# Krual-T/OutfitX

Hardware: AMD Instinct MI355X
Metric: outfits/sec CP forward (8-item sets, 224^2, bf16) (higher is better)
Workload: dtype f16

## Files before the change

include/ofx.h:

```cpp
#ifndef OFX_H
#define OFX_H
#include <stddef.h>
#include <stdint.h>

#ifdef __cplusplus
extern "C" {
#endif

#define OFX_ABI_VERSION 6

enum { OFX_OK = 0, OFX_EINVAL = -1, OFX_ESHAPE = -2, OFX_EHIP = -3, OFX_EWORKSPACE = -4, OFX_ESTATE = -5 };
enum ofx_dtype { OFX_F32 = 0, OFX_BF16 = 1, OFX_F16 = 2 };
enum ofx_act { OFX_ACT_NONE = 0, OFX_ACT_QUICK_GELU = 1, OFX_ACT_GELU = 2, OFX_ACT_MISH = 3, OFX_ACT_MISH_GRAD = 4 };
enum ofx_precision { OFX_PREC_BF16 = 0, OFX_PREC_F16 = 1, OFX_PREC_BF16X3 = 2, OFX_PREC_F16W2 = 3 };
enum ofx_out_kind { OFX_OUT_F32 = 0, OFX_OUT_OP = 1, OFX_OUT_SPLIT3 = 2 };

typedef struct ofx_handle ofx_handle;
typedef void* ofx_stream;

const char* ofx_last_error(void);
int ofx_abi_version(void);

typedef struct ofx_model_desc {
    int d_model, n_head, d_ffn, n_layers, max_items;
    int outfit_act;
    int outfit_precision;
    int vit_width, vit_layers, vit_heads, vit_mlp, vit_patch, vit_image, vit_act;
    int txt_width, txt_layers, txt_heads, txt_mlp, txt_vocab, txt_max_pos, txt_act, txt_eos_id;
    int proj_dim;
    int tower_precision;
    float ln_eps;
    int vit_w2_mask, txt_x3, proj_x3, vit_x3;
    int txt_w2_mask, vit_w2_qkv_layers, vit_w2_fc1_layers, vit_w2_out_layers, vit_w2_fc2_layers;
} ofx_model_desc;
enum { OFX_W2_PATCH = 1, OFX_W2_QKV = 2, OFX_W2_OUT = 4, OFX_W2_FC1 = 8, OFX_W2_FC2 = 16 };

void ofx_default_desc(ofx_model_desc* d);

ofx_handle* ofx_create(int device, const ofx_model_desc* desc);
void ofx_destroy(ofx_handle* h);

int ofx_pack_outfit_weights(ofx_handle* h, const void* const* fp32_params, int n_params, ofx_stream stream);
int ofx_pack_vision_weights(ofx_handle* h, const void* const* fp32_params, int n_params, ofx_stream stream);
int ofx_pack_text_weights(ofx_handle* h, const void* const* fp32_params, int n_params, ofx_stream stream);

enum ofx_op { OFX_OP_SET_ENCODER = 0, OFX_OP_VIT = 1, OFX_OP_TEXT = 2, OFX_OP_TOPK = 3 };
size_t ofx_workspace_bytes(ofx_handle* h, int op, int n, int len);

int ofx_set_encoder_fwd(ofx_handle* h, const float* x, const uint8_t* pad_mask, const float* prefix,
                        int prefix_stride, int B, int L, float* out_row0, void* ws, size_t ws_bytes,
                        ofx_stream stream);
int ofx_cp_head(ofx_handle* h, const float* row0, int B, float* logits, ofx_stream stream);
int ofx_cir_head(ofx_handle* h, const float* row0, int B, float* emb, void* ws, size_t ws_bytes, ofx_stream stream);
int ofx_cir_prefix(ofx_handle* h, const float* target_text_emb, int B, float* prefix_out, ofx_stream stream);

int ofx_vit_b32_fwd(ofx_handle* h, const float* pixels, int N, float* emb, int emb_ld, int emb_col,
                    int normalize, void* ws, size_t ws_bytes, ofx_stream stream);
int ofx_clip_text_fwd(ofx_handle* h, const int64_t* ids, const int64_t* attn_mask, const int* lengths_host,
                      int N, int T, float* emb, int emb_ld, int emb_col, int normalize, void* ws,
                      size_t ws_bytes, ofx_stream stream);

int ofx_fitb_argmin(const float* y_hat, const float* cand, int B, int C, int D, int64_t* idx, float* dist,
                    ofx_stream stream);
int ofx_fitb_argmin_indexed(const float* table, int ld, long long n_table, const int* cand_index, const float* y_hat, int B, int C, int D,
                            const int64_t* answer, int64_t* idx, float* dist, int* n_correct, ofx_stream stream);
int ofx_l2_topk(ofx_handle* h, const float* Q, const float* P, int nq, int np, int D, int k, int64_t index_base,
                int64_t* idx, float* dist, void* ws, size_t ws_bytes, ofx_stream stream);
size_t ofx_l2_topk_grouped_ws(int nq, int np, int max_group_rows);
int ofx_l2_topk_grouped(ofx_handle* h, const float* Q, const float* P, int nq, int np, int D, int k, const int* panels, int n_panels,
                        int max_group_rows, const int64_t* gt, int64_t* idx, float* dist, int* gt_pos, void* ws, size_t ws_bytes,
                        ofx_stream stream);
int ofx_topk_merge(const int64_t* idx_in, const float* dist_in, int parts, int nq, int k, int64_t* idx, float* dist,
                   ofx_stream stream);

size_t ofx_clip_preprocess_ws(const int* heights, const int* widths, int N, int channels, int size);
int ofx_clip_preprocess(const uint8_t* src, const long long* offsets, const int* heights, const int* widths, int N, int channels, int size,
                        const float* mean, const float* stdv, float* out, void* ws, size_t ws_bytes, ofx_stream stream);
int ofx_clip_preprocess_patches(const uint8_t* src, const long long* offsets, const int* heights, const int* widths, int N, int channels, int size,
                                int patch, const float* mean, const float* stdv, void* patches, int op_dtype, void* ws, size_t ws_bytes,
                                ofx_stream stream);
int ofx_patchify(const float* pixels, void* out, int N, int img, int patch, int op_dtype, ofx_stream stream);
size_t ofx_vit_b32_u8_ws_bytes(ofx_handle* h, const int* heights, const int* widths, int N, int channels);
int ofx_vit_b32_fwd_u8(ofx_handle* h, const uint8_t* src, const long long* offsets, const int* heights, const int* widths, int N, int channels,
                       const float* mean, const float* stdv, float* emb, int emb_ld, int emb_col, int normalize, void* ws, size_t ws_bytes,
                       ofx_stream stream);

int ofx_set_encoder_fwd_indexed(ofx_handle* h, const float* table, int ld, long long n_table, const int* item_index, const int* cu_items,
                                const float* prefix, int prefix_stride, int B, int max_len, float* out_row0, void* ws, size_t ws_bytes,
                                ofx_stream stream);

size_t ofx_cp_train_tape_bytes(ofx_handle* h, int B, int L);
size_t ofx_cp_train_ws_bytes(ofx_handle* h, int B, int L);
size_t ofx_cp_train_grad_floats(ofx_handle* h, size_t* offsets, int n_offsets);
int ofx_cp_train_fwd(ofx_handle* h, const float* x, const uint8_t* pad_mask, int B, int L, float* logits, void* tape, size_t tape_bytes,
                     void* ws, size_t ws_bytes, float dropout_p, unsigned seed, ofx_stream stream);
int ofx_cp_train_bwd(ofx_handle* h, void* tape, size_t tape_bytes, const float* dlogits, int B, int L, float* grads, size_t grad_floats,
                     void* ws, size_t ws_bytes, float dropout_p, unsigned seed, ofx_stream stream);
int ofx_cp_train_fwd_indexed(ofx_handle* h, const float* table, int ld, long long n_table, const int* item_index, const int* cu_items,
                             int B, int max_len, float* logits, void* tape, size_t tape_bytes, void* ws, size_t ws_bytes,
                             float dropout_p, unsigned seed, ofx_stream stream);
int ofx_cir_train_fwd(ofx_handle* h, const float* x, const uint8_t* pad_mask, const float* table, int ld, long long n_table,
                      const int* item_index, const int* cu_items, const float* target_text, int B, int L, float* y, void* tape,
                      size_t tape_bytes, void* ws, size_t ws_bytes, float dropout_p, unsigned seed, ofx_stream stream);
int ofx_cir_train_bwd(ofx_handle* h, void* tape, size_t tape_bytes, const float* dy, int B, int L, float* grads, size_t grad_floats,
                      void* ws, size_t ws_bytes, float dropout_p, unsigned seed, ofx_stream stream);
int ofx_cp_train_bwd_into(ofx_handle* h, void* tape, size_t tape_bytes, const float* dlogits, int B, int L, float* const* grad_ptrs,
                          int n_ptrs, int accumulate, void* ws, size_t ws_bytes, float dropout_p, unsigned seed, ofx_stream stream);
int ofx_cir_train_bwd_into(ofx_handle* h, void* tape, size_t tape_bytes, const float* dy, int B, int L, float* const* grad_ptrs,
                           int n_ptrs, int accumulate, void* ws, size_t ws_bytes, float dropout_p, unsigned seed, ofx_stream stream);
int ofx_train_arm_layer_events(ofx_handle* h, void* const* events, int n);
int ofx_dropout_mask(float dropout_p, unsigned seed, int site, int rows, int cols, float* out, ofx_stream stream);
int ofx_focal_loss(const float* logits, const float* labels, int B, float alpha, float gamma, float upstream, float* loss, float* dlogits,
                   ofx_stream stream);
int ofx_focal_loss_ex(const float* logits, const float* labels, int B, float alpha, float gamma, float upstream, int reduction, float* loss,
                      float* per_elem, float* dlogits, ofx_stream stream);
size_t ofx_set_rank_loss_ws_bytes(int B, int K, int D);
int ofx_set_rank_loss(const float* y, const float* y_hat, const float* neg, const uint8_t* neg_mask, int B, int K, int D, float margin,
                      float upstream, float* loss, float* dy_hat, float* d_pos, float* d_neg, void* ws, size_t ws_bytes, ofx_stream stream);
int ofx_set_rank_loss_indexed(const float* table, int ld, long long n_table, const int* pos_index, const int* neg_index, const float* y_hat,
                              int B, int K, int D, float margin, float upstream, float* loss, float* dy_hat, float* d_pos, float* d_neg,
                              void* ws, size_t ws_bytes, ofx_stream stream);

int ofx_cir_sample_batch(const int* outfit_cu, const int* outfit_rows, int n_outfits, int n_outfit_rows, const int* pos_cu, const int* pos_slots,
                         int n_pos_slots, const int* pool_cu, const int* pool_rows, int n_pools, int n_pool_rows, const int* row_pool,
                         const int* row_slot, int n_table, const int* outfit_ids, int B, unsigned seed, unsigned draw, int K, int max_len,
                         int* item_index, int* cu_seqlens, int* target_item_index, int* neg_items_index, ofx_stream stream);

typedef struct ofx_opt_segment { float* param; long long offset; long long numel; } ofx_opt_segment;
size_t ofx_adamw_step_ws_bytes(long long n_arena);
int ofx_adamw_step(const ofx_opt_segment* segments, int n_segments, float* grad, float* exp_avg, float* exp_avg_sq, long long n_arena,
                   float* step, double lr, double beta1, double beta2, double eps, double weight_decay, double max_norm, double grad_scale,
                   float* grad_norm, int* skipped, void* ws, size_t ws_bytes, ofx_stream stream);

void ofx_profile_enable(int on);
int ofx_profile_read(double* ms, double* flops, long long* launches);
typedef struct ofx_prof_record { int cat, M, N, K, kind, kmul; float ms; double flops; double bytes; } ofx_prof_record;
int ofx_profile_records(ofx_prof_record* out, int cap);

int ofx_tune(int knob, int value);
unsigned ofx_config_generation(void);
int ofx_profile_enabled(void);
int ofx_stream_create_low_priority(int device, ofx_stream* out);
int ofx_stream_destroy(ofx_stream stream);
// ... 76 lines not shown
```

outfitx_amd/_lib.py:

```python
from __future__ import annotations

import ctypes as C
import os

_HERE = os.path.dirname(os.path.abspath(__file__))
LIB_PATH = os.environ.get("OFX_LIB") or os.path.join(_HERE, "libofx_hip.so")

OFX_OK = 0
ABI_VERSION = 6
F32, BF16, F16 = 0, 1, 2
ACT_NONE, ACT_QUICK_GELU, ACT_GELU, ACT_MISH = 0, 1, 2, 3
PREC_BF16, PREC_F16, PREC_BF16X3 = 0, 1, 2
OUT_F32, OUT_OP, OUT_SPLIT3 = 0, 1, 2
OP_SET_ENCODER, OP_VIT, OP_TEXT, OP_TOPK = 0, 1, 2, 3
PREC_F16W2 = 3
PRECISIONS = {"bf16": PREC_BF16, "f16": PREC_F16, "fp16": PREC_F16, "bf16x3": PREC_BF16X3, "f16w2": PREC_F16W2}
W2_PATCH, W2_QKV, W2_OUT, W2_FC1, W2_FC2 = 1, 2, 4, 8, 16
TOWER_SCHEMES = {
    "bf16": (PREC_BF16, 0, 0, 0, 0), "f16": (PREC_F16, 0, 0, 0, 0), "fp16": (PREC_F16, 0, 0, 0, 0),
    "f16w2": (PREC_F16, W2_PATCH | W2_OUT | W2_FC2, 1, 1, 0),
    "bf16w2": (PREC_BF16, W2_PATCH | W2_OUT | W2_FC2, 1, 1, 0),
    "f16w2q": (PREC_F16, W2_PATCH | W2_QKV | W2_OUT | W2_FC2, 1, 1, 0),
    "f16w2f": (PREC_F16, W2_PATCH | W2_OUT | W2_FC1 | W2_FC2, 1, 1, 0),
    "f16w2x": (PREC_F16, W2_PATCH | W2_QKV | W2_OUT | W2_FC1 | W2_FC2, 1, 1, 0),
    "f16x3": (PREC_F16, W2_PATCH, 1, 1, 1), "bf16x3": (PREC_BF16, W2_PATCH, 1, 1, 1),
}
SCHEME_ALIASES = {"f16w2h": "f16w2x@qkv=0-5"}
DEFAULT_TOWER_PRECISION = "f16w2x"


def _layer_bits(spec: str) -> int:
    m = 0
    for part in spec.split(","):
        a, _, b = part.partition("-")
        for l in range(int(a), int(b or a) + 1):
            m |= 1 << l
    return m


def tower_scheme(name: str) -> dict:
    name = SCHEME_ALIASES.get(name, name)
    base, _, opts = name.partition("@")
    if base not in TOWER_SCHEMES:
        raise ValueError(f"unknown tower_precision {name!r}; one of {sorted(list(TOWER_SCHEMES) + list(SCHEME_ALIASES))} [+ '@txt=w2;qkv=<layers>;fc1=<layers>']")
    prec, mask, txt_x3, proj_x3, vit_x3 = TOWER_SCHEMES[base]
    d = {"tower_precision": prec, "vit_w2_mask": mask, "txt_x3": txt_x3, "proj_x3": proj_x3, "vit_x3": vit_x3,
         "txt_w2_mask": 0, "vit_w2_qkv_layers": 0, "vit_w2_fc1_layers": 0, "vit_w2_out_layers": 0, "vit_w2_fc2_layers": 0}
    for o in filter(None, opts.split(";")):
        k, _, v = o.partition("=")
        try:
            if k == "txt" and v == "w2":
                d["txt_x3"], d["txt_w2_mask"] = 0, W2_QKV | W2_OUT | W2_FC1 | W2_FC2
            elif k in ("qkv", "fc1", "out", "fc2"):
                bits = _layer_bits(v) if v not in ("", "none") else 0
                if bits == 0:
                    d["vit_w2_mask"] &= ~{"qkv": W2_QKV, "fc1": W2_FC1, "out": W2_OUT, "fc2": W2_FC2}[k]
                d[f"vit_w2_{k}_layers"] = bits
            else:
                raise ValueError
        except ValueError:
            raise ValueError(f"tower_precision {name!r}: bad option {o!r} (txt=w2 | qkv= / fc1= / out= / fc2=<layers>, layers like 0-5,8 or none)") from None
    return d
ACTS = {"none": ACT_NONE, "quick_gelu": ACT_QUICK_GELU, "gelu": ACT_GELU, "mish": ACT_MISH}


class OfxError(RuntimeError):
    pass


class ModelDesc(C.Structure):
    _fields_ = [(n, C.c_int) for n in (
        "d_model", "n_head", "d_ffn", "n_layers", "max_items", "outfit_act", "outfit_precision",
        "vit_width", "vit_layers", "vit_heads", "vit_mlp", "vit_patch", "vit_image", "vit_act",
        "txt_width", "txt_layers", "txt_heads", "txt_mlp", "txt_vocab", "txt_max_pos", "txt_act", "txt_eos_id",
        "proj_dim", "tower_precision")] + [("ln_eps", C.c_float)] + [(n, C.c_int) for n in ("vit_w2_mask", "txt_x3", "proj_x3", "vit_x3", "txt_w2_mask", "vit_w2_qkv_layers", "vit_w2_fc1_layers", "vit_w2_out_layers", "vit_w2_fc2_layers")]


class OptSegment(C.Structure):
    _fields_ = [("param", C.c_void_p), ("offset", C.c_longlong), ("numel", C.c_longlong)]


class ProfRecord(C.Structure):
    _fields_ = [("cat", C.c_int), ("M", C.c_int), ("N", C.c_int), ("K", C.c_int), ("kind", C.c_int), ("kmul", C.c_int), ("ms", C.c_float), ("flops", C.c_double), ("bytes", C.c_double)]


_vp, _i, _f, _sz, _i64 = C.c_void_p, C.c_int, C.c_float, C.c_size_t, C.c_int64

SIGNATURES = {
    "ofx_last_error": (C.c_char_p, []),
    "ofx_abi_version": (_i, []),
    "ofx_stream_create_low_priority": (_i, [_i, C.POINTER(_vp)]),
    "ofx_stream_destroy": (_i, [_vp]),
    "ofx_default_desc": (None, [C.POINTER(ModelDesc)]),
    "ofx_create": (_vp, [_i, C.POINTER(ModelDesc)]),
    "ofx_destroy": (None, [_vp]),
    "ofx_pack_outfit_weights": (_i, [_vp, C.POINTER(_vp), _i, _vp]),
    "ofx_pack_vision_weights": (_i, [_vp, C.POINTER(_vp), _i, _vp]),
    "ofx_pack_text_weights": (_i, [_vp, C.POINTER(_vp), _i, _vp]),
    "ofx_workspace_bytes": (_sz, [_vp, _i, _i, _i]),
    "ofx_set_encoder_fwd": (_i, [_vp, _vp, _vp, _vp, _i, _i, _i, _vp, _vp, _sz, _vp]),
    "ofx_cp_head": (_i, [_vp, _vp, _i, _vp, _vp]),
    "ofx_cir_head": (_i, [_vp, _vp, _i, _vp, _vp, _sz, _vp]),
    "ofx_cir_prefix": (_i, [_vp, _vp, _i, _vp, _vp]),
    "ofx_vit_b32_fwd": (_i, [_vp, _vp, _i, _vp, _i, _i, _i, _vp, _sz, _vp]),
    "ofx_clip_text_fwd": (_i, [_vp, _vp, _vp, C.POINTER(_i), _i, _i, _vp, _i, _i, _i, _vp, _sz, _vp]),
    "ofx_fitb_argmin": (_i, [_vp, _vp, _i, _i, _i, _vp, _vp, _vp]),
    "ofx_fitb_argmin_indexed": (_i, [_vp, _i, C.c_longlong, _vp, _vp, _i, _i, _i, _vp, _vp, _vp, _vp, _vp]),
    "ofx_l2_topk": (_i, [_vp, _vp, _vp, _i, _i, _i, _i, _i64, _vp, _vp, _vp, _sz, _vp]),
    "ofx_l2_topk_grouped_ws": (_sz, [_i, _i, _i]),
    "ofx_l2_topk_grouped": (_i, [_vp, _vp, _vp, _i, _i, _i, _i, _vp, _i, _i, _vp, _vp, _vp, _vp, _vp, _sz, _vp]),
    "ofx_topk_merge": (_i, [_vp, _vp, _i, _i, _i, _vp, _vp, _vp]),
    "ofx_clip_preprocess_ws": (_sz, [_vp, _vp, _i, _i, _i]),
    "ofx_clip_preprocess": (_i, [_vp, _vp, _vp, _vp, _i, _i, _i, _vp, _vp, _vp, _vp, _sz, _vp]),
    "ofx_clip_preprocess_patches": (_i, [_vp, _vp, _vp, _vp, _i, _i, _i, _i, _vp, _vp, _vp, _i, _vp, _sz, _vp]),
    "ofx_patchify": (_i, [_vp, _vp, _i, _i, _i, _i, _vp]),
    "ofx_vit_b32_u8_ws_bytes": (_sz, [_vp, _vp, _vp, _i, _i]),
    "ofx_vit_b32_fwd_u8": (_i, [_vp, _vp, _vp, _vp, _vp, _i, _i, _vp, _vp, _vp, _i, _i, _i, _vp, _sz, _vp]),
    "ofx_set_encoder_fwd_indexed": (_i, [_vp, _vp, _i, C.c_longlong, _vp, _vp, _vp, _i, _i, _i, _vp, _vp, _sz, _vp]),
    "ofx_cp_train_fwd_indexed": (_i, [_vp, _vp, _i, C.c_longlong, _vp, _vp, _i, _i, _vp, _vp, _sz, _vp, _sz, _f, C.c_uint, _vp]),
    "ofx_cp_train_tape_bytes": (_sz, [_vp, _i, _i]),
    "ofx_cp_train_ws_bytes": (_sz, [_vp, _i, _i]),
    "ofx_cp_train_grad_floats": (_sz, [_vp, C.POINTER(_sz), _i]),
    "ofx_cp_train_fwd": (_i, [_vp, _vp, _vp, _i, _i, _vp, _vp, _sz, _vp, _sz, _f, C.c_uint, _vp]),
    "ofx_cp_train_bwd": (_i, [_vp, _vp, _sz, _vp, _i, _i, _vp, _sz, _vp, _sz, _f, C.c_uint, _vp]),
    "ofx_cir_train_fwd": (_i, [_vp, _vp, _vp, _vp, _i, C.c_longlong, _vp, _vp, _vp, _i, _i, _vp, _vp, _sz, _vp, _sz, _f, C.c_uint, _vp]),
    "ofx_cir_train_bwd": (_i, [_vp, _vp, _sz, _vp, _i, _i, _vp, _sz, _vp, _sz, _f, C.c_uint, _vp]),
    "ofx_cp_train_bwd_into": (_i, [_vp, _vp, _sz, _vp, _i, _i, C.POINTER(_vp), _i, _i, _vp, _sz, _f, C.c_uint, _vp]),
    "ofx_cir_train_bwd_into": (_i, [_vp, _vp, _sz, _vp, _i, _i, C.POINTER(_vp), _i, _i, _vp, _sz, _f, C.c_uint, _vp]),
    "ofx_train_arm_layer_events": (_i, [_vp, C.POINTER(_vp), _i]),
    "ofx_dropout_mask": (_i, [_f, C.c_uint, _i, _i, _i, _vp, _vp]),
    "ofx_focal_loss": (_i, [_vp, _vp, _i, _f, _f, _f, _vp, _vp, _vp]),
    "ofx_focal_loss_ex": (_i, [_vp, _vp, _i, _f, _f, _f, _i, _vp, _vp, _vp, _vp]),
    "ofx_set_rank_loss_ws_bytes": (_sz, [_i, _i, _i]),
    "ofx_set_rank_loss": (_i, [_vp, _vp, _vp, _vp, _i, _i, _i, _f, _f, _vp, _vp, _vp, _vp, _vp, _sz, _vp]),
    "ofx_set_rank_loss_indexed": (_i, [_vp, _i, C.c_longlong, _vp, _vp, _vp, _i, _i, _i, _f, _f, _vp, _vp, _vp, _vp, _vp, _sz, _vp]),
    "ofx_cir_sample_batch": (_i, [_vp, _vp, _i, _i, _vp, _vp, _i, _vp, _vp, _i, _i, _vp, _vp, _i, _vp, _i, C.c_uint, C.c_uint, _i, _i, _vp, _vp, _vp, _vp, _vp]),
    "ofx_adamw_step_ws_bytes": (_sz, [C.c_longlong]),
    "ofx_adamw_step": (_i, [_vp, _i, _vp, _vp, _vp, C.c_longlong, _vp] + [C.c_double] * 7 + [_vp, _vp, _vp, _sz, _vp]),
    "ofx_profile_enable": (None, [_i]),
    "ofx_profile_read": (_i, [C.POINTER(C.c_double), C.POINTER(C.c_double), C.POINTER(C.c_longlong)]),
    "ofx_profile_records": (_i, [C.POINTER(ProfRecord), _i]),
    "ofx_tune": (_i, [_i, _i]),
    "ofx_config_generation": (C.c_uint, []),
    "ofx_profile_enabled": (_i, []),
    "ofx_gemm": (_i, [_vp, _vp, _vp, _vp, _vp, _i, _i, _i, _i, _i, _i, _i, _i, _i, _vp]),
    "ofx_gemm_w2": (_i, [_vp, _vp, _vp, _vp, _vp, _i, _i, _i, _i, _i, _i, _i, _i, _i, _vp]),
    "ofx_gemm_x3": (_i, [_vp, _vp, _vp, _vp, _vp, _i, _i, _i, _i, _i, _i, _i, _i, _i, _vp]),
    "ofx_pack_lo8": (_i, [_vp, _vp, _vp, _i, _i, _vp]),
    "ofx_gemm_w2f8": (_i, [_vp, _vp, _vp, _vp, _vp, _vp, _vp, _i, _i, _i, _i, _i, _i, _i, _i, _vp]),
    "ofx_gemm_w2f8_fold": (_i, [_vp, _vp, _vp, _vp, _vp, _vp, _vp, _vp, _i, _i, _i, _i, _i, _i, _vp]),
    "ofx_gemm_tn_ws": (_sz, [_i, _i, _i]),
    "ofx_gemm_tn": (_i, [_vp, _i, _vp, _i, _vp, _i, _i, _i, _i, _vp, _vp, _sz, _i, _vp]),
    "ofx_gemm_splitk_ws": (_sz, [_i, _i, _i]),
    "ofx_gemm_splitk": (_i, [_vp, _vp, _vp, _vp, _vp, _i, _i, _i, _i, _i, _i, _i, _i, _i, _vp, _sz, _vp]),
    "ofx_gemm_train": (_i, [_vp, _vp, _vp, _vp, _vp, _vp, _i, _vp, _i, _i, _i, _i, _i, _i, _i, _f, C.c_uint, _i, _i, _vp, _sz, _vp]),
    "ofx_gemm_tn_into": (_i, [_vp, _i, _vp, _i, _vp, _i, _i, _i, _i, _vp, _i, _i, _i, _vp, _sz, _i, _vp]),
    "ofx_transpose_cast": (_i, [_vp, _vp, _i, _i, _i, _vp, _i, _i, _vp]),
    "ofx_layernorm_bwd_ws": (_sz, [_i]),
    "ofx_layernorm_bwd": (_i, [_vp] * 11 + [_i, _vp, _i, _f, C.c_uint, _i, _i, _i, _vp, _sz, _vp]),
    "ofx_colsum_ws": (_sz, [_i]),
    "ofx_colsum": (_i, [_vp, _i, _i, _vp, _vp, _vp, _vp, _vp, _i, _i, _i, _i, _vp, _i, _i, _vp, _sz, _vp]),
    "ofx_head_bwd": (_i, [_vp, _vp, _vp, _vp, _vp, _vp, _i, _i, _f, C.c_uint, _i, _i, _i, _i, _vp]),
    "ofx_gemm_fold_producer": (_i, [_vp] * 9 + [_i] * 8 + [_vp]),
    "ofx_gemm_fold": (_i, [_vp, _vp, _vp, _vp, _vp, _i, _vp, _i, _i, _i, _i, _i, _i, _i, _i, _vp]),
    "ofx_stats_finalize": (_i, [_vp, _i, _i, _f, _vp, _i, _vp]),
    "ofx_row_stats_cast": (_i, [_vp, _vp, _vp, _vp, _i, _i, _f, _i, _vp]),
    "ofx_fold_pack": (_i, [_vp] * 7 + [_i, _i, _i, _i, _vp]),
    "ofx_vit_embed_ln": (_i, [_vp] * 9 + [_i, _i, _i, _f, _i, _vp]),
    "ofx_gather_hilo": (_i, [_vp, _vp, _vp, _vp, _i, _i, _i, _vp]),
    "ofx_layernorm": (_i, [_vp, _vp, _vp, _vp, _vp, _i, _i, _i, _i, _i, _f, _vp]),
    "ofx_attention": (_i, [_vp, _vp, _vp, _i, _i, _i, _i, _i, _i, _i, _i, _i, _f, _i, _vp]),
    "ofx_attention_ex": (_i, [_vp, _vp, _vp, _i, _i, _i, _i, _i, _i, _i, _i, _i, _i, _i, _f, _i, _vp]),
    "ofx_set_attention_slabs": (_i, [_vp, _sz, _i, _vp, _vp, _vp, _i, _i, _i, _i, _i, _i, _i, _f, _i, _vp]),
    "ofx_splitk_reduce_ln": (_i, [_vp, _sz, _i, _vp, _vp, _i, _vp, _i, _vp, _vp, _vp, _i, _i, _f, _i, _vp, _i, _i, _vp]),
    "ofx_fused_qkv_attention": (_i, [_vp, _vp, _vp, _vp, _vp, _vp, _i, _i, _i, _i, _i, _i, _f, _i, _vp]),
    "ofx_fused_qkv_attention_w2": (_i, [_vp, _vp, _vp, _vp, _vp, _vp, _i, _i, _i, _i, _i, _i, _f, _i, _vp]),
    "ofx_set_attention": (_i, [_vp, _vp, _vp, _i, _i, _i, _i, _i, _i, _i, _f, _i, _vp]),
    "ofx_attention_varlen": (_i, [_vp, _vp, _vp, _i, _i, _i, _i, _i, _i, _i, _i, _f, _f, C.c_uint, _i, _i, _vp]),
    "ofx_set_attention_op": (_i, [_vp, _vp, _vp, _i, _i, _i, _i, _i, _i, _i, _f, _f, C.c_uint, _i, _i, _vp]),
    "ofx_set_attention_bwd": (_i, [_vp, _vp, _vp, _vp, _i, _i, _i, _i, _i, _f, _f, C.c_uint, _i, _i, _i, _vp]),
    "ofx_attention_f32": (_i, [_vp, _vp, _vp, _i, _i, _i, _i, _i, _i, _i, _i, _f, _i, _vp]),
    "ofx_convert": (_i, [_vp, _vp, _i, _i, _i, _i, _vp]),
}

_lib = None


def load() -> C.CDLL:
# ... 31 lines not shown
```

outfitx_amd/csrc/api.hip:

```cpp
#include <stdarg.h>
#include <string.h>

#include <algorithm>
#include <vector>
#include <mutex>
#include <cstring>

#include "ofx_weights.h"

static thread_local char g_err[512] = "";
void ofx_set_error(const char* fmt, ...) {
    va_list ap;
    va_start(ap, fmt);
    vsnprintf(g_err, sizeof(g_err), fmt, ap);
    va_end(ap);
}
extern "C" const char* ofx_last_error(void) { return g_err; }
extern "C" int ofx_abi_version(void) { return OFX_ABI_VERSION; }
extern "C" int ofx_stream_create_low_priority(int device, ofx_stream* out) {
    OFX_REQUIRE(out, OFX_EINVAL, "stream_create_low_priority: NULL argument");
    int prev = 0, least = 0, greatest = 0;
    OFX_HIP(hipGetDevice(&prev));
    OFX_HIP(hipSetDevice(device));
    hipStream_t s = nullptr;
// ... 470 lines not shown
    return ofx_launch_cp_head(row0, h->cp_w, h->cp_b, logits, B, h->d.d_model, (hipStream_t)stream);
}

extern "C" int ofx_cir_head(ofx_handle* h, const float* row0, int B, float* emb, void* ws, size_t ws_bytes, ofx_stream stream) {
    OFX_REQUIRE(h && h->out_ready, OFX_ESTATE, "cir_head: outfit weights not packed");
    OFX_REQUIRE(row0 && emb && B > 0 && ws, OFX_EINVAL, "cir_head: bad argument");
    const int D = h->d.d_model, km = a_kmul(h->ot_form);
    OFX_REQUIRE(ws_bytes >= (size_t)B * km * D * 2, OFX_EWORKSPACE, "cir_head: workspace too small");
    hipStream_t s = (hipStream_t)stream;
    TRY(ofx_launch_pack_rows(row0, ws, B, B, D, D, D, km == 3 ? 1 : 0, h->ot_dtype, s));
    GemmArgs g{};
    use_cir_head(g, *h);
    g.A = ws; g.C = emb; g.M = B; g.N = D; g.ldc = D; g.out_kind = OFX_OUT_F32;
    return ofx_launch_gemm(g, h->ot_dtype, s);
}

extern "C" int ofx_cir_prefix(ofx_handle* h, const float* txt, int B, float* out, ofx_stream stream) {
    OFX_REQUIRE(h && h->out_ready, OFX_ESTATE, "cir_prefix: outfit weights not packed");
    OFX_REQUIRE(txt && out && B > 0, OFX_EINVAL, "cir_prefix: bad argument");
    return ofx_launch_cir_prefix(h->tgt_img_emb, txt, out, B, h->d.d_model, (hipStream_t)stream);
}

int g_fuse_qkv = 1;
int g_x3_vit_f32_attn = 0;
int g_prune_q = 1;

static int clip_layer(const ClipLayer& L, const ClipWs& w, int rows, int nseq, int S, int W, int MLP, int heads, int act,
                      float eps, int causal, const int64_t* key_mask, int mask_ld, int dt, const int* pool_idx, hipStream_t s, bool pool_first) {
    const bool fused = (g_fuse_qkv & (L.qkv.form == W_SPLIT ? 2 : 1)) && !pool_idx && !causal && !key_mask && S >= 33 && S <= 64 && (256 / S - 1) * S + 64 - 256 <= 16;
    if (fused) {
        TRY(ofx_launch_fused_qkv_attn(w.XB, L.qkv.w, L.qkv.bias, w.S, L.qkv.col_sum, w.H, nseq, S, W, heads, W, W, 0.125f, dt, s, L.qkv.form == W_SPLIT));
    } else {
        GemmArgs g1{}; g1.A = w.XB; g1.C = w.QKV; g1.row_stat = w.S; g1.M = rows; g1.N = 3 * W;
        g1.ldc = 3 * W; g1.act = OFX_ACT_NONE; g1.out_kind = OFX_OUT_OP;
        use_gemm(g1, L.qkv, W);
        const bool prune = pool_idx && pool_first && g_prune_q;
        if (prune) {
            GemmArgs kv = g1;
            kv.W = (const char*)g1.W + (size_t)W * g1.K * 2; kv.bias = g1.bias + W; kv.col_sum = g1.col_sum + W; kv.C = (char*)w.QKV + (size_t)W * 2; kv.N = 2 * W;
            if (g1.W8) { kv.W8 = (const char*)g1.W8 + (size_t)W * W; kv.w8_scale = (const char*)g1.w8_scale + W; }
            TRY(ofx_launch_gemm(kv, dt, s));
            GemmArgs q = g1;
            q.M = nseq; q.N = W; q.lda = S * W; q.ldc = S * 3 * W; q.stat_ld = S;
            TRY(ofx_launch_gemm(q, dt, s));
        } else
            TRY(ofx_launch_gemm(g1, dt, s));
        AttnArgs at{w.QKV, w.H, key_mask, nseq, S, heads, 3 * W, W, W, 2 * W, mask_ld, causal, 0.125f};
        at.only_row0 = prune ? 1 : 0;
        TRY(ofx_launch_attention_mfma(at, dt, s));
    }
    char* H = w.H; char* U = w.U; int M = rows;
    if (pool_idx) {
        TRY(ofx_launch_gather_rows(w.H, pool_idx, w.HP, nseq, W * 2, W * 2, s));
        TRY(ofx_launch_gather_hilo(w.XB, w.XLO, pool_idx, w.XP, nseq, W, dt, s));
        H = w.HP; U = w.UP; M = nseq;
    }
    auto to_stream = [&](GemmArgs& g) {
        g.M = M; g.N = W; g.ldc = W; g.ldr = W; g.act = OFX_ACT_NONE;
        if (pool_idx) { g.C = w.XP; g.resid = w.XP; g.out_kind = OFX_OUT_F32; g.slab = w.slab; g.slab_bytes = w.slab_bytes; }
        else { g.C = w.XB; g.xb_out = w.XB; g.xlo = w.XLO; g.stat_part = w.P; g.out_kind = OFX_OUT_OP; }
    };
    GemmArgs g2{}; g2.A = H;
    use_gemm(g2, L.o, W); to_stream(g2);
    TRY(ofx_launch_gemm(g2, dt, s));
    GemmArgs g3{}; g3.C = U; g3.M = M; g3.N = MLP; g3.ldc = MLP; g3.act = act; g3.out_kind = OFX_OUT_OP;
    if (pool_idx) {
        LnArgs ln2{w.XP, nullptr, L.g2, L.be2, H, M, W, W, OFX_OUT_OP, eps};
        TRY(ofx_launch_layernorm(ln2, dt, s));
        g3.A = H; g3.slab = w.slab; g3.slab_bytes = w.slab_bytes;
    } else {
        TRY(ofx_launch_stats_finalize(w.P, W / 64, W, eps, w.S, M, s));
        g3.A = w.XB; g3.row_stat = w.S;
    }
    use_gemm(g3, L.fc1, W);
    TRY(ofx_launch_gemm(g3, dt, s));
    GemmArgs g4{}; g4.A = U;
    use_gemm(g4, L.fc2, MLP); to_stream(g4);
    TRY(ofx_launch_gemm(g4, dt, s));
    if (!pool_idx) TRY(ofx_launch_stats_finalize(w.P, W / 64, W, eps, w.S, M, s));
    return OFX_OK;
}

static int clip_layer_x3(const ClipLayer& L, const ClipWs& w, int rows, int nseq, int S, int W, int MLP, int heads, int act,
                         float eps, int causal, const int64_t* key_mask, int mask_ld, int dt, const int* pool_idx, hipStream_t s, bool mfma_attn = false) {
    LnArgs ln{w.X, nullptr, L.g1, L.be1, w.H, rows, W, 3 * W, OFX_OUT_SPLIT3, eps};
    TRY(ofx_launch_layernorm(ln, dt, s));
    GemmArgs g1{}; g1.A = w.H; g1.C = w.QKV; g1.M = rows; g1.N = 3 * W;
    use_gemm(g1, L.qkv, W);
    const bool f32_attn = S <= 64 && !mfma_attn;
    g1.ldc = 3 * W; g1.act = OFX_ACT_NONE; g1.out_kind = f32_attn ? OFX_OUT_F32 : OFX_OUT_OP;
    TRY(ofx_launch_gemm(g1, dt, s));
    if (f32_attn) {
        SetAttnArgs sa{w.QKV, w.H, nullptr, nseq, heads, W, 3 * W, OFX_OUT_SPLIT3, S, 0, 0.125f};
        sa.fixed_len = S; sa.causal = causal; sa.key_mask = key_mask; sa.mask_ld = mask_ld;
        TRY(ofx_launch_set_attention(sa, dt, s));
    } else {
        AttnArgs at{w.QKV, w.H, key_mask, nseq, S, heads, 3 * W, 3 * W, W, 2 * W, mask_ld, causal, 0.125f};
        at.split3_w = W;
        TRY(ofx_launch_attention_mfma(at, dt, s));
    }
    float* X = w.X; char* H = w.H; char* U = w.U; int M = rows;
    if (pool_idx) {
        TRY(ofx_launch_gather_rows(w.H, pool_idx, w.HP, nseq, 3 * W * 2, 3 * W * 2, s));
        TRY(ofx_launch_gather_rows(w.X, pool_idx, w.XP, nseq, W * 4, W * 4, s));
        X = w.XP; H = w.HP; U = w.UP; M = nseq;
    }
    GemmArgs g2{}; g2.A = H; g2.C = X; g2.resid = X; g2.M = M; g2.N = W; g2.ldc = W; g2.ldr = W; g2.act = OFX_ACT_NONE; g2.out_kind = OFX_OUT_F32;
    use_gemm(g2, L.o, W);
    if (pool_idx) { g2.slab = w.slab; g2.slab_bytes = w.slab_bytes; }
    TRY(ofx_launch_gemm(g2, dt, s));
    LnArgs ln2{X, nullptr, L.g2, L.be2, H, M, W, 3 * W, OFX_OUT_SPLIT3, eps};
    TRY(ofx_launch_layernorm(ln2, dt, s));
    GemmArgs g3{}; g3.A = H; g3.C = U; g3.M = M; g3.N = MLP; g3.ldc = 3 * MLP; g3.act = act; g3.out_kind = OFX_OUT_SPLIT3;
    use_gemm(g3, L.fc1, W);
    if (pool_idx) { g3.slab = w.slab; g3.slab_bytes = w.slab_bytes; }
    TRY(ofx_launch_gemm(g3, dt, s));
    GemmArgs g4{}; g4.A = U; g4.C = X; g4.resid = X; g4.M = M; g4.N = W; g4.ldc = W; g4.ldr = W; g4.act = OFX_ACT_NONE; g4.out_kind = OFX_OUT_F32;
    use_gemm(g4, L.fc2, MLP);
    if (pool_idx) { g4.slab = w.slab; g4.slab_bytes = w.slab_bytes; }
    return ofx_launch_gemm(g4, dt, s);
}

static int clip_layers(const std::vector<ClipLayer>& Ls, const ClipWs& w, int rows, int nseq, int S, int W, int MLP,
                       int heads, int act, float eps, int causal, const int64_t* key_mask, int mask_ld, int dt,
                       const int* pool_idx, hipStream_t s, bool pool_first, bool x3) {
    if (x3) {
        for (size_t l = 0; l < Ls.size(); ++l)
            TRY(clip_layer_x3(Ls[l], w, rows, nseq, S, W, MLP, heads, act, eps, causal, key_mask, mask_ld, dt, l + 1 == Ls.size() ? pool_idx : nullptr, s, !causal && !key_mask && !g_x3_vit_f32_attn));
        return OFX_OK;
    }
    for (size_t l = 0; l < Ls.size(); ++l)
        TRY(clip_layer(Ls[l], w, rows, nseq, S, W, MLP, heads, act, eps, causal, key_mask, mask_ld, dt,
                       l + 1 == Ls.size() ? pool_idx : nullptr, s, pool_first));
    return OFX_OK;
}

struct RawImages {
    const uint8_t* src; const long long* offsets; const int* heights; const int* widths; int channels; const float* mean; const float* stdv;
    void* ws; size_t ws_bytes;
};

static int vit_core(ofx_handle* h, const float* pixels, const RawImages* raw, int N, float* emb, int emb_ld, int emb_col,
                    int normalize, void* ws, size_t ws_bytes, ofx_stream stream) {
    OFX_REQUIRE(h && h->vis_ready, OFX_ESTATE, "vit_b32_fwd: vision weights not packed");
    OFX_REQUIRE((pixels || raw) && emb && ws && N > 0, OFX_EINVAL, "vit_b32_fwd: bad argument");
    const ofx_model_desc& d = h->d;
    OFX_REQUIRE(emb_ld >= emb_col + d.proj_dim && emb_ld % 4 == 0 && emb_col % 4 == 0, OFX_ESHAPE, "vit_b32_fwd: bad emb_ld/emb_col");
    hipStream_t s = (hipStream_t)stream;
    const int g = d.vit_image / d.vit_patch, S = g * g + 1, W = d.vit_width, KP = 3 * d.vit_patch * d.vit_patch, dt = h->tw_dtype;
    int chunk = std::min(N, VIT_CHUNK_MAX);
    while (chunk > 1 && vit_bytes(h, chunk, nullptr, nullptr, ~(size_t)0) > ws_bytes) chunk = (chunk + 1) / 2;
    OFX_REQUIRE(vit_bytes(h, chunk, nullptr, nullptr, ~(size_t)0) <= ws_bytes, OFX_EWORKSPACE, "vit_b32_fwd: workspace %zu bytes cannot hold one image", ws_bytes);
    const size_t px_per_img = (size_t)3 * d.vit_image * d.vit_image;
    for (int n0 = 0; n0 < N; n0 += chunk) {
        const int n = std::min(chunk, N - n0);
        ClipWs w;
        vit_bytes(h, n, &w, ws, ws_bytes);
        const int rows = n * S;
        if (raw)
            TRY(ofx_preprocess_to(raw->src, raw->offsets + n0, raw->heights + n0, raw->widths + n0, n, raw->channels, d.vit_image, raw->mean, raw->stdv,
                                  nullptr, w.U, d.vit_patch, dt, raw->ws, raw->ws_bytes, s));
        else
            TRY(ofx_launch_patchify(pixels + (size_t)n0 * px_per_img, w.U, n, d.vit_image, d.vit_patch, dt, s));
        GemmArgs gp{}; gp.A = w.U; gp.C = w.QKV; gp.M = n * g * g; gp.N = W; gp.ldc = W;
        gp.act = OFX_ACT_NONE; gp.out_kind = OFX_OUT_F32;
        use_gemm(gp, h->v_patch, KP);
        TRY(ofx_launch_gemm(gp, dt, s));
        TRY(ofx_launch_vit_embed_ln((const float*)w.QKV, h->v_cls, h->v_pos, h->v_pre_g, h->v_pre_b, w.X, n, S, W, d.ln_eps, s, w.XB, w.S, dt, w.XLO));
        TRY(ofx_launch_iota_rows(w.idx, n, S, s));
        TRY(clip_layers(h->vl, w, rows, n, S, W, d.vit_mlp, d.vit_heads, d.vit_act, d.ln_eps, 0, nullptr, 0, dt, w.idx, s, true, h->vit_x3 != 0));
        const int pk = h->proj_x3 ? 3 : 1;
        LnArgs ln{w.XP, nullptr, h->v_post_g, h->v_post_b, w.PL, n, W, pk * W, pk == 3 ? OFX_OUT_SPLIT3 : OFX_OUT_OP, d.ln_eps};
        TRY(ofx_launch_layernorm(ln, dt, s));
        GemmArgs gj{}; gj.A = w.PL; gj.C = w.E; gj.M = n; gj.N = d.proj_dim; gj.ldc = d.proj_dim;
        use_gemm(gj, h->v_proj, W);
        gj.act = OFX_ACT_NONE; gj.out_kind = OFX_OUT_F32; gj.slab = w.slab; gj.slab_bytes = w.slab_bytes;
        TRY(ofx_launch_gemm(gj, dt, s));
        TRY(ofx_launch_l2norm_store(w.E, emb + (size_t)n0 * emb_ld, n, d.proj_dim, emb_ld, emb_col, normalize, s));
    }
    return OFX_OK;
}

extern "C" int ofx_vit_b32_fwd(ofx_handle* h, const float* pixels, int N, float* emb, int emb_ld, int emb_col,
                               int normalize, void* ws, size_t ws_bytes, ofx_stream stream) {
    OFX_REQUIRE(pixels, OFX_EINVAL, "vit_b32_fwd: pixels is NULL");
    return vit_core(h, pixels, nullptr, N, emb, emb_ld, emb_col, normalize, ws, ws_bytes, stream);
}

extern "C" size_t ofx_vit_b32_u8_ws_bytes(ofx_handle* h, const int* heights, const int* widths, int N, int channels) {
    if (!h || N <= 0) return 0;
    const size_t pre = ofx_clip_preprocess_ws(heights, widths, N, channels, h->d.vit_image);
    return pre ? align_up(pre, 256) + vit_bytes(h, std::min(N, VIT_CHUNK_MAX), nullptr, nullptr, ~(size_t)0) : 0;
}

extern "C" int ofx_vit_b32_fwd_u8(ofx_handle* h, const uint8_t* src, const long long* offsets, const int* heights, const int* widths, int N, int channels,
                                  const float* mean, const float* stdv, float* emb, int emb_ld, int emb_col, int normalize, void* ws, size_t ws_bytes,
                                  ofx_stream stream) {
    OFX_REQUIRE(h && src && offsets && heights && widths && mean && stdv && N > 0, OFX_EINVAL, "vit_b32_fwd_u8: bad argument");
    const size_t pre = align_up(ofx_clip_preprocess_ws(heights, widths, N, channels, h->d.vit_image), 256);
    OFX_REQUIRE(pre > 0 && pre < ws_bytes, OFX_EWORKSPACE, "vit_b32_fwd_u8: workspace %zu bytes, the preprocessor alone needs %zu", ws_bytes, pre);
    RawImages raw{src, offsets, heights, widths, channels, mean, stdv, ws, pre};
    return vit_core(h, nullptr, &raw, N, emb, emb_ld, emb_col, normalize, (char*)ws + pre, ws_bytes - pre, stream);
}

extern "C" int ofx_clip_text_fwd(ofx_handle* h, const int64_t* ids, const int64_t* attn_mask, const int* lengths_host,
                                 int N, int T, float* emb, int emb_ld, int emb_col, int normalize, void* ws,
                                 size_t ws_bytes, ofx_stream stream) {
    OFX_REQUIRE(h && h->txt_ready, OFX_ESTATE, "clip_text_fwd: text weights not packed");
    OFX_REQUIRE(ids && emb && ws && N > 0 && T > 0, OFX_EINVAL, "clip_text_fwd: bad argument");
    const ofx_model_desc& d = h->d;
    OFX_REQUIRE(T <= d.txt_max_pos, OFX_ESHAPE, "clip_text_fwd: T=%d exceeds max_position_embeddings=%d", T, d.txt_max_pos);
    OFX_REQUIRE(emb_ld >= emb_col + d.proj_dim && emb_ld % 4 == 0 && emb_col % 4 == 0, OFX_ESHAPE, "clip_text_fwd: bad emb_ld/emb_col");
    int Tc = T;
    if (lengths_host) {
        Tc = 1;
        for (int i = 0; i < N; ++i) Tc = std::max(Tc, std::min(lengths_host[i], T));
    }
    OFX_REQUIRE(Tc <= 64, OFX_ESHAPE, "clip_text_fwd: %d tokens per text exceed the 64-token attention tile", Tc);
    hipStream_t s = (hipStream_t)stream;
    ClipWs w;
    const size_t need = txt_bytes(h, N, Tc, &w, ws, ws_bytes);
    OFX_REQUIRE(need <= ws_bytes, OFX_EWORKSPACE, "clip_text_fwd: workspace %zu < %zu bytes", ws_bytes, need);
    const int W = d.txt_width, dt = h->tw_dtype, rows = N * Tc;
    TRY(ofx_launch_text_embed(ids, h->t_tok, h->t_pos, w.X, N, T, Tc, W, d.txt_vocab, s));
    TRY(ofx_launch_text_eos_index(ids, w.idx, N, T, Tc, d.txt_eos_id, s));
    const bool x3 = h->txt_x3 != 0, x3p = x3 || h->proj_x3;
    const int pk = x3p ? 3 : 1;
    if (!x3) TRY(ofx_launch_row_stats_cast(w.X, w.XB, w.XLO, w.S, rows, W, d.ln_eps, dt, s));
    TRY(clip_layers(h->tl, w, rows, N, Tc, W, d.txt_mlp, d.txt_heads, d.txt_act, d.ln_eps, 1, attn_mask, T, dt, w.idx, s, false, x3));
    LnArgs ln{w.XP, nullptr, h->t_fin_g, h->t_fin_b, w.PL, N, W, pk * W, x3p ? OFX_OUT_SPLIT3 : OFX_OUT_OP, d.ln_eps};
    TRY(ofx_launch_layernorm(ln, dt, s));
    GemmArgs gj{}; gj.A = w.PL; gj.C = w.E; gj.M = N; gj.N = d.proj_dim; gj.ldc = d.proj_dim;
    use_gemm(gj, h->t_proj, W);
    gj.act = OFX_ACT_NONE; gj.out_kind = OFX_OUT_F32; gj.slab = w.slab; gj.slab_bytes = w.slab_bytes;
    TRY(ofx_launch_gemm(gj, dt, s));
    return ofx_launch_l2norm_store(w.E, emb, N, d.proj_dim, emb_ld, emb_col, normalize, s);
}

extern "C" int ofx_fitb_argmin(const float* y, const float* cand, int B, int C, int D, int64_t* idx, float* dist, ofx_stream stream) {
    OFX_REQUIRE(y && cand && idx && B > 0 && C > 0 && D > 0 && D % 4 == 0, OFX_EINVAL, "fitb_argmin: bad argument");
    return ofx_launch_fitb(y, cand, B, C, D, idx, dist, (hipStream_t)stream);
}
extern "C" int ofx_fitb_argmin_indexed(const float* table, int ld, long long n_table, const int* cand_index, const float* y_hat, int B, int C, int D,
                                       const int64_t* answer, int64_t* idx, float* dist, int* n_correct, ofx_stream stream) {
    OFX_REQUIRE(table && cand_index && y_hat && idx, OFX_EINVAL, "fitb_argmin_indexed: NULL argument");
    OFX_REQUIRE((answer != nullptr) == (n_correct != nullptr), OFX_EINVAL, "fitb_argmin_indexed: answer and n_correct go together");
    OFX_REQUIRE((((uintptr_t)table | (uintptr_t)y_hat) & 15) == 0, OFX_EINVAL, "fitb_argmin_indexed: table and y_hat must be 16-byte aligned");
    OFX_REQUIRE(B >= 1 && C >= 1 && D >= 4 && D % 4 == 0, OFX_ESHAPE, "fitb_argmin_indexed: B = %d, C = %d, D = %d; needs B >= 1, C >= 1, D %% 4 == 0, D >= 4",
                B, C, D);
    OFX_REQUIRE(ld >= D && ld % 4 == 0 && n_table >= 1 && n_table <= INT_MAX, OFX_ESHAPE,
                "fitb_argmin_indexed: ld = %d, n_table = %lld; needs ld >= D = %d, ld %% 4 == 0, 1 <= n_table <= INT_MAX", ld, n_table, D);
    return ofx_launch_fitb_indexed(table, ld, (int)n_table, cand_index, y_hat, B, C, D, answer, idx, dist, n_correct, (hipStream_t)stream);
}
extern "C" int ofx_l2_topk(ofx_handle*, const float* Q, const float* P, int nq, int np, int D, int k, int64_t index_base,
                           int64_t* idx, float* dist, void* ws, size_t ws_bytes, ofx_stream stream) {
    return ofx_launch_l2_topk(Q, P, nq, np, D, k, index_base, idx, dist, ws, ws_bytes, (hipStream_t)stream);
}
extern "C" int ofx_l2_topk_grouped(ofx_handle*, const float* Q, const float* P, int nq, int np, int D, int k, const int* panels, int n_panels,
                                   int max_group_rows, const int64_t* gt, int64_t* idx, float* dist, int* gt_pos, void* ws, size_t ws_bytes, ofx_stream stream) {
    return ofx_launch_l2_topk_grouped(Q, P, nq, np, D, k, panels, n_panels, max_group_rows, gt, idx, dist, gt_pos, ws, ws_bytes, (hipStream_t)stream);
}
extern "C" int ofx_topk_merge(const int64_t* idx_in, const float* dist_in, int parts, int nq, int k, int64_t* idx, float* dist, ofx_stream stream) {
    return ofx_launch_topk_merge(idx_in, dist_in, parts, nq, k, idx, dist, (hipStream_t)stream);
}

namespace {
struct TapeLayer { float* Xin; float* st1; char* H1; char* QKV; char* O; float* Xmid; float* st2; char* H2; float* Upre; char* A; };
struct Tape { int* cu; float* row0; float* prefix; char* row0b; char* pO; float* pX; std::vector<TapeLayer> L; size_t bytes; };
size_t carve_tape(const ofx_handle* h, Bump& b, int B, int Lq, Tape* t) {
    const size_t M = (size_t)B * (Lq + 1), D = h->d.d_model, Fp = h->ot_ffn_pad, Mp = align_up(M, 64);
    Tape tp;
    tp.cu = b.take<int>(B + 1);
    tp.row0 = b.take<float>((size_t)B * D);
    tp.prefix = b.take<float>((size_t)B * D);
    tp.row0b = b.take<char>(align_up((size_t)B, 64) * D * 2);
    tp.pO = b.take<char>(align_up((size_t)B, 64) * D * 2);
    tp.pX = b.take<float>((size_t)B * D);
    tp.L.resize(h->d.n_layers);
    for (TapeLayer& l : tp.L) {
        l.Xin = b.take<float>(M * D); l.st1 = b.take<float>(M * 2); l.H1 = b.take<char>(Mp * D * 2); l.QKV = b.take<char>(M * 3 * D * 2);
        l.O = b.take<char>(Mp * D * 2); l.Xmid = b.take<float>(M * D); l.st2 = b.take<float>(M * 2); l.H2 = b.take<char>(Mp * D * 2);
        l.Upre = b.take<float>(M * Fp); l.A = b.take<char>(Mp * Fp * 2);
    }
    tp.bytes = align_up(b.off, 256);
    if (t) *t = tp;
    return tp.bytes;
}
struct BwdWs { float *dXa, *dXb_f, *dH, *dO, *part, *d_row0; char *gXb, *dU, *gQb, *dyb; int* rowmap; char* slab; size_t slab_bytes; };
size_t carve_bwd(const ofx_handle* h, Bump& b, int B, int Lq, BwdWs* w) {
    const size_t M = (size_t)B * (Lq + 1), D = h->d.d_model, Fp = h->ot_ffn_pad, Mp = align_up(M, 64);
    BwdWs t;
    t.dXa = b.take<float>(M * D); t.dXb_f = b.take<float>(M * D); t.dH = b.take<float>(M * D); t.dO = b.take<float>(M * D);
    t.part = b.take<float>(std::max(ofx_ln_bwd_part_floats((int)D), ofx_colsum_part_floats((int)(3 * D))));
    t.gXb = b.take<char>(Mp * D * 2); t.dU = b.take<char>(Mp * Fp * 2); t.gQb = b.take<char>(Mp * 3 * D * 2);
    t.d_row0 = b.take<float>((size_t)B * D); t.dyb = b.take<char>(align_up((size_t)B, 64) * D * 2);
    t.rowmap = b.take<int>(M);
    t.slab_bytes = 0;
    const int m = (int)M, Di = (int)D, Fi = (int)Fp;
    for (auto s : {ofx_gemm_tn_slab_bytes(Di, Di, B), ofx_gemm_splitk_bytes(B, Di, Di), ofx_gemm_tn_slab_bytes(Di, Fi, B), ofx_gemm_tn_slab_bytes(Fi, Di, B),
                   ofx_gemm_splitk_bytes(B, Fi, Di), ofx_gemm_splitk_bytes(B, Di, Fi),
                   ofx_gemm_tn_slab_bytes(Di, Fi, m), ofx_gemm_tn_slab_bytes(Fi, Di, m), ofx_gemm_tn_slab_bytes(Di, Di, m), ofx_gemm_tn_slab_bytes(3 * Di, Di, m),
                   ofx_gemm_splitk_bytes(m, Fi, Di), ofx_gemm_splitk_bytes(m, Di, Fi), ofx_gemm_splitk_bytes(m, Di, Di), ofx_gemm_splitk_bytes(m, Di, 3 * Di)})
        t.slab_bytes = std::max(t.slab_bytes, s);
    t.slab = b.take<char>(t.slab_bytes);
    if (w) *w = t;
    return align_up(b.off, 256);
}
void grad_offsets(const ofx_handle* h, std::vector<size_t>& off, size_t* total) {
    const size_t D = h->d.d_model, Fp = h->ot_ffn_pad;
    size_t o = 0;
    auto add = [&](size_t n) { off.push_back(o); o += (n + 63) / 64 * 64; };
    add(D); add(D / 2); add(D); add(1); add(D * D);
    for (int l = 0; l < h->d.n_layers; ++l) { add(3 * D * D); add(3 * D); add(D * D); add(D); add(Fp * D); add(Fp); add(D * Fp); add(D); add(D); add(D); add(D); add(D); }
    *total = o;
}
}

extern "C" size_t ofx_cp_train_tape_bytes(ofx_handle* h, int B, int L) { Bump b(nullptr, ~(size_t)0); return h ? carve_tape(h, b, B, L, nullptr) : 0; }
extern "C" size_t ofx_cp_train_ws_bytes(ofx_handle* h, int B, int L) {
// ... 236 lines not shown
}

static bool rank_loss_shape_ok(int B, int K, int D) { return B >= 1 && K >= 0 && D >= 4 && D <= 4096 && D % 4 == 0; }
extern "C" size_t ofx_set_rank_loss_ws_bytes(int B, int K, int D) { return rank_loss_shape_ok(B, K, D) ? ofx_set_rank_loss_ws(B, K) : 0; }
extern "C" int ofx_set_rank_loss(const float* y, const float* y_hat, const float* neg, const uint8_t* neg_mask, int B, int K, int D, float margin,
                                 float upstream, float* loss, float* dy_hat, float* d_pos, float* d_neg, void* ws, size_t ws_bytes, ofx_stream stream) {
    OFX_REQUIRE(rank_loss_shape_ok(B, K, D), OFX_ESHAPE, "set_rank_loss: B = %d, K = %d, D = %d; needs B >= 1, K >= 0, D %% 4 == 0, 4 <= D <= 4096", B, K, D);
    OFX_REQUIRE(y && y_hat && loss && ws && (neg || K == 0), OFX_EINVAL, "set_rank_loss: NULL argument");
    OFX_REQUIRE((((uintptr_t)y | (uintptr_t)y_hat | (uintptr_t)neg | (uintptr_t)dy_hat | (uintptr_t)ws) & 15) == 0, OFX_EINVAL,
                "set_rank_loss: y, y_hat, neg, dy_hat and ws must be 16-byte aligned");
    OFX_REQUIRE(ws_bytes >= ofx_set_rank_loss_ws(B, K), OFX_EWORKSPACE, "set_rank_loss: workspace %zu < %zu bytes", ws_bytes, ofx_set_rank_loss_ws(B, K));
    return ofx_launch_set_rank_loss(y, y_hat, neg, neg_mask, B, K, D, margin, upstream, loss, dy_hat, d_pos, d_neg, ws, (hipStream_t)stream);
}

extern "C" int ofx_set_rank_loss_indexed(const float* table, int ld, long long n_table, const int* pos_index, const int* neg_index, const float* y_hat,
                                         int B, int K, int D, float margin, float upstream, float* loss, float* dy_hat, float* d_pos, float* d_neg,
                                         void* ws, size_t ws_bytes, ofx_stream stream) {
    OFX_REQUIRE(rank_loss_shape_ok(B, K, D), OFX_ESHAPE,
                "set_rank_loss_indexed: B = %d, K = %d, D = %d; needs B >= 1, K >= 0, D %% 4 == 0, 4 <= D <= 4096", B, K, D);
    OFX_REQUIRE(ld >= D && ld % 4 == 0 && n_table >= 1 && n_table <= INT_MAX, OFX_ESHAPE,
                "set_rank_loss_indexed: ld = %d, n_table = %lld; needs ld >= D = %d, ld %% 4 == 0, 1 <= n_table <= INT_MAX", ld, n_table, D);
    OFX_REQUIRE(table && pos_index && y_hat && loss && ws && (neg_index || K == 0), OFX_EINVAL, "set_rank_loss_indexed: NULL argument");
    OFX_REQUIRE((((uintptr_t)table | (uintptr_t)y_hat | (uintptr_t)dy_hat | (uintptr_t)ws) & 15) == 0 &&
                    (((uintptr_t)pos_index | (uintptr_t)neg_index) & 3) == 0,
                OFX_EINVAL, "set_rank_loss_indexed: table, y_hat, dy_hat and ws must be 16-byte aligned, the index arrays 4-byte aligned");
    OFX_REQUIRE(ws_bytes >= ofx_set_rank_loss_ws(B, K), OFX_EWORKSPACE, "set_rank_loss_indexed: workspace %zu < %zu bytes", ws_bytes,
                ofx_set_rank_loss_ws(B, K));
    return ofx_launch_set_rank_loss_indexed(table, ld, (int)n_table, pos_index, neg_index, y_hat, B, K, D, margin, upstream, loss, dy_hat, d_pos, d_neg, ws,
                                            (hipStream_t)stream);
}

extern "C" int ofx_cir_sample_batch(const int* outfit_cu, const int* outfit_rows, int n_outfits, int n_outfit_rows, const int* pos_cu, const int* pos_slots,
                                    int n_pos_slots, const int* pool_cu, const int* pool_rows, int n_pools, int n_pool_rows, const int* row_pool,
                                    const int* row_slot, int n_table, const int* outfit_ids, int B, unsigned seed, unsigned draw, int K, int max_len,
                                    int* item_index, int* cu_seqlens, int* target_item_index, int* neg_items_index, ofx_stream stream) {
    OFX_REQUIRE(B >= 1, OFX_EINVAL, "cir_sample_batch: B = %d; needs B >= 1", B);
    OFX_REQUIRE(K >= 0 && K <= 64 && max_len >= 1 && max_len <= 31, OFX_ESHAPE, "cir_sample_batch: K = %d, max_len = %d; needs 0 <= K <= 64, 1 <= max_len <= 31",
                K, max_len);
    OFX_REQUIRE(n_outfits >= 1 && n_table >= 1 && n_outfit_rows >= 0 && n_pos_slots >= 0 && n_pools >= 0 && n_pool_rows >= 0, OFX_ESHAPE,
                "cir_sample_batch: n_outfits = %d, n_table = %d (both >= 1), n_outfit_rows = %d, n_pos_slots = %d, n_pools = %d, n_pool_rows = %d (all >= 0)",
                n_outfits, n_table, n_outfit_rows, n_pos_slots, n_pools, n_pool_rows);
    OFX_REQUIRE((long long)B * std::max(K, max_len) <= INT_MAX, OFX_ESHAPE, "cir_sample_batch: B * max(K, max_len) = %lld exceeds INT_MAX",
                (long long)B * std::max(K, max_len));
    const void* ptrs[] = {outfit_cu, outfit_rows, pos_cu, pos_slots, pool_cu, pool_rows, row_pool, row_slot, outfit_ids, item_index, cu_seqlens, target_item_index};
    uintptr_t bits = (uintptr_t)neg_items_index;
    for (const void* p : ptrs) {
        OFX_REQUIRE(p, OFX_EINVAL, "cir_sample_batch: NULL argument");
        bits |= (uintptr_t)p;
    }
    OFX_REQUIRE(neg_items_index || K == 0, OFX_EINVAL, "cir_sample_batch: NULL neg_items_index with K = %d", K);
    OFX_REQUIRE((bits & 15) == 0, OFX_EINVAL, "cir_sample_batch: every array must be 16-byte aligned");
    CirSampleArgs a{outfit_cu, outfit_rows, pos_cu, pos_slots, pool_cu, pool_rows, row_pool, row_slot, outfit_ids,
                    n_outfits, n_outfit_rows, n_pos_slots, n_pools, n_pool_rows, n_table, B, K, max_len, seed, draw,
                    item_index, cu_seqlens, target_item_index, neg_items_index};
    return ofx_launch_cir_sample_batch(a, (hipStream_t)stream);
}

static bool adamw_shape_ok(long long n_arena) { return n_arena > 0 && n_arena % 64 == 0; }
extern "C" size_t ofx_adamw_step_ws_bytes(long long n_arena) { return adamw_shape_ok(n_arena) ? ofx_adamw_step_ws(n_arena) : 0; }
extern "C" int ofx_adamw_step(const ofx_opt_segment* segments, int n_segments, float* grad, float* exp_avg, float* exp_avg_sq, long long n_arena,
                              float* step, double lr, double beta1, double beta2, double eps, double weight_decay, double max_norm, double grad_scale,
                              float* grad_norm, int* skipped, void* ws, size_t ws_bytes, ofx_stream stream) {
    OFX_REQUIRE(segments && grad && exp_avg && exp_avg_sq && step && grad_norm && skipped && ws, OFX_EINVAL, "adamw_step: NULL argument");
    OFX_REQUIRE(n_segments >= 1 && n_segments <= 1024, OFX_ESHAPE, "adamw_step: n_segments = %d; needs 1 <= n_segments <= 1024", n_segments);
    OFX_REQUIRE(adamw_shape_ok(n_arena), OFX_ESHAPE, "adamw_step: n_arena = %lld; needs a positive multiple of 64", n_arena);
    OFX_REQUIRE((((uintptr_t)grad | (uintptr_t)exp_avg | (uintptr_t)exp_avg_sq | (uintptr_t)ws) & 15) == 0 && ((uintptr_t)segments & 7) == 0, OFX_EINVAL,
                "adamw_step: grad, exp_avg, exp_avg_sq and ws must be 16-byte aligned, segments 8-byte aligned");
    OFX_REQUIRE(ws_bytes >= ofx_adamw_step_ws(n_arena), OFX_EWORKSPACE, "adamw_step: workspace %zu < %zu bytes", ws_bytes, ofx_adamw_step_ws(n_arena));
    return ofx_launch_adamw_step(segments, n_segments, grad, exp_avg, exp_avg_sq, n_arena, step, lr, beta1, beta2, eps, weight_decay, max_norm,
                                 grad_scale, grad_norm, skipped, ws, (hipStream_t)stream);
}

extern "C" int ofx_tune(int knob, int value) {
    ++g_config_generation;
    switch (knob) {
        case 2: case 5: case 11: case 15: case 16: case 18: return ofx_gemm_tune(knob, value);
        case 6: if (value != 2) { ofx_set_error("ofx_tune(6): %d is not 2 (the towers' LayerNorms are always folded)", value); return OFX_EINVAL; } return OFX_OK;
        case 7: g_train_mfma_attn = value; return OFX_OK;
        case 8: g_prune_q = value; return OFX_OK;
        case 9: g_fuse_qkv = value; return OFX_OK;
        case 10: g_set_fuse = value; return OFX_OK;
        case 17: g_topk_filter = value != 0; return OFX_OK;
        case 20: g_x3_vit_f32_attn = value != 0; return OFX_OK;
        default: ofx_set_error("ofx_tune: unknown knob %d", knob); return OFX_EINVAL;
    }
}

static GemmArgs op_gemm(const void* A, const void* W, void* C, const float* bias, const float* resid, int M, int N, int K, int lda, int ldc, int ldr,
                        int act, int out_kind) {
    GemmArgs g{}; g.A = A; g.W = W; g.C = C; g.bias = bias; g.resid = resid; g.M = M; g.N = N; g.K = K; g.lda = lda; g.ldc = ldc;
    g.ldr = ldr; g.act = act; g.out_kind = out_kind;
    return g;
}
extern "C" int ofx_gemm(const void* A, const void* W, void* C, const float* bias, const float* resid, int M, int N, int K,
                        int lda, int ldc, int ldr, int act, int out_kind, int op_dtype, ofx_stream stream) {
    return ofx_launch_gemm(op_gemm(A, W, C, bias, resid, M, N, K, lda, ldc, ldr, act, out_kind), op_dtype, (hipStream_t)stream);
}
extern "C" int ofx_gemm_w2(const void* A, const void* W2, void* C, const float* bias, const float* resid, int M, int N, int K,
                           int lda, int ldc, int ldr, int act, int out_kind, int op_dtype, ofx_stream stream) {
    GemmArgs g = op_gemm(A, W2, C, bias, resid, M, N, 2 * K, lda, ldc, ldr, act, out_kind); g.a_wrap = K;
    return ofx_launch_gemm(g, op_dtype, (hipStream_t)stream);
}
extern "C" int ofx_gemm_x3(const void* A3, const void* W3, void* C, const float* bias, const float* resid, int M, int N, int K,
                           int lda, int ldc, int ldr, int act, int out_kind, int op_dtype, ofx_stream stream) {
    GemmArgs g = op_gemm(A3, W3, C, bias, resid, M, N, 3 * K, lda, ldc, ldr, act, out_kind); g.k_mult = 3;
    return ofx_launch_gemm(g, op_dtype, (hipStream_t)stream);
}
extern "C" int ofx_pack_lo8(const void* W2, void* W8, void* scale8, int N, int K, ofx_stream stream) {
    return ofx_launch_pack_lo8(W2, W8, scale8, N, K, (hipStream_t)stream);
}
extern "C" int ofx_gemm_w2f8(const void* A, const void* W2, const void* W8, const void* scale8, void* C, const float* bias, const float* resid, int M, int N, int K,
                             int lda, int ldc, int ldr, int act, int out_kind, ofx_stream stream) {
    GemmArgs g = op_gemm(A, W2, C, bias, resid, M, N, 2 * K, lda, ldc, ldr, act, out_kind); g.a_wrap = K; g.W8 = W8; g.w8_scale = scale8;
    return ofx_launch_gemm(g, OFX_F16, (hipStream_t)stream);
}
extern "C" int ofx_gemm_w2f8_fold(const void* A, const void* W2, const void* W8, const void* scale8, void* C, const float* bias, const float* row_stat, const float* col_sum,
                                  int M, int N, int K, int lda, int ldc, int act, ofx_stream stream) {
    OFX_REQUIRE(row_stat && col_sum, OFX_EINVAL, "gemm_w2f8_fold: row_stat and col_sum are required");
    GemmArgs g = op_gemm(A, W2, C, bias, nullptr, M, N, 2 * K, lda, ldc, 0, act, OFX_OUT_OP); g.a_wrap = K; g.W8 = W8; g.w8_scale = scale8;
    g.row_stat = row_stat; g.col_sum = col_sum; g.stat_ld = 1;
    return ofx_launch_gemm(g, OFX_F16, (hipStream_t)stream);
}
extern "C" size_t ofx_gemm_splitk_ws(int M, int N, int K) { return ofx_gemm_splitk_bytes(M, N, K); }
extern "C" int ofx_gemm_splitk(const void* A, const void* W, void* C, const float* bias, const float* resid, int M, int N, int K,
                               int lda, int ldc, int ldr, int act, int out_kind, int op_dtype, void* slab, size_t slab_bytes, ofx_stream stream) {
    GemmArgs g = op_gemm(A, W, C, bias, resid, M, N, K, lda, ldc, ldr, act, out_kind); g.slab = slab; g.slab_bytes = slab_bytes;
    return ofx_launch_gemm(g, op_dtype, (hipStream_t)stream);
}
extern "C" size_t ofx_gemm_tn_ws(int M, int N, int K) { return ofx_gemm_tn_slab_bytes(M, N, K); }
extern "C" int ofx_gemm_tn(const void* A, int lda, const void* B, int ldb, float* C, int ldc, int M, int N, int K, const int* k_dev,
                           void* slab, size_t slab_bytes, int op_dtype, ofx_stream stream) {
    return ofx_launch_gemm_tn(A, lda, B, ldb, C, ldc, M, N, K, k_dev, slab, slab_bytes, op_dtype, (hipStream_t)stream);
}
static bool op_dtype_ok(int op_dtype) { return op_dtype == OFX_BF16 || op_dtype == OFX_F16; }
static bool drop_p_ok(float p) { return p >= 0.f && p < 1.f; }
static bool aligned_to(size_t mask, std::initializer_list<const void*> ptrs) {
    for (const void* p : ptrs) if ((uintptr_t)p & mask) return false;
    return true;
}
extern "C" int ofx_gemm_train(const void* A, const void* W, void* C, const float* bias, const float* resid, float* aux_out, int M, const int* m_dev,
                              int N, int K, int lda, int ldc, int ldr, int act, int out_kind, float dropout_p, unsigned seed, int site, int op_dtype,
                              void* slab, size_t slab_bytes, ofx_stream stream) {
    OFX_REQUIRE(A && W && C && drop_p_ok(dropout_p) && (act != OFX_ACT_MISH_GRAD || resid), OFX_EINVAL, "gemm_train: bad argument");
    OFX_REQUIRE(aligned_to(15, {bias, resid, aux_out, slab}) && aligned_to(3, {m_dev}), OFX_EINVAL,
                "gemm_train: bias, resid, aux_out and slab must be 16-byte aligned");
    GemmArgs g = op_gemm(A, W, C, bias, resid, M, N, K, lda, ldc, ldr, act, out_kind); g.slab = slab; g.slab_bytes = slab_bytes;
    g.aux_out = aux_out; g.m_dev = m_dev; g.drop = make_drop(dropout_p, seed, (unsigned)site);
    return ofx_launch_gemm(g, op_dtype, (hipStream_t)stream);
}
extern "C" int ofx_gemm_tn_into(const void* A, int lda, const void* B, int ldb, float* C, int ldc, int M, int N, int K, const int* k_dev,
                                int m_valid, int n_valid, int accumulate, void* slab, size_t slab_bytes, int op_dtype, ofx_stream stream) {
    OFX_REQUIRE(A && B && C && m_valid >= 0 && n_valid >= 0, OFX_EINVAL, "gemm_tn_into: bad argument");
    OFX_REQUIRE(aligned_to(15, {slab}) && aligned_to(3, {k_dev}), OFX_EINVAL, "gemm_tn_into: slab must be 16-byte aligned");
    return ofx_launch_gemm_tn(A, lda, B, ldb, C, ldc, M, N, K, k_dev, slab, slab_bytes, op_dtype, (hipStream_t)stream, m_valid, n_valid, accumulate ? 1 : 0);
}
extern "C" int ofx_transpose_cast(const float* src, void* dst, int R, int C, int ldd, void* row_dst, int ld_row, int op_dtype, ofx_stream stream) {
    OFX_REQUIRE(src && dst && op_dtype_ok(op_dtype), OFX_EINVAL, "transpose_cast: bad argument");
    OFX_REQUIRE(aligned_to(3, {src}) && aligned_to(1, {dst, row_dst}), OFX_EINVAL, "transpose_cast: misaligned pointer");
    OFX_REQUIRE(R > 0 && C > 0, OFX_ESHAPE, "transpose_cast: R=%d C=%d", R, C);
    return ofx_launch_transpose_cast(src, dst, R, C, ldd, op_dtype, (hipStream_t)stream, row_dst, ld_row);
}
static bool ln_bwd_d_ok(int D) { return D == 512 || D == 768 || D == 1024; }
extern "C" size_t ofx_layernorm_bwd_ws(int D) { return ln_bwd_d_ok(D) ? ofx_ln_bwd_part_floats(D) * sizeof(float) : 0; }
extern "C" int ofx_layernorm_bwd(const float* dy, const float* x, const float* stats, const float* gamma, const float* add, const int* add_map,
                                 float* dx, void* dx_op, float* dgamma, float* dbeta, float* dcols, int M, const int* m_dev, int D, float dropout_p,
                                 unsigned seed, int site, int accumulate, int op_dtype, void* ws, size_t ws_bytes, ofx_stream stream) {
// ... 199 lines not shown
```

outfitx_amd/csrc/attention.hip:

```cpp
#include "attn_wave.h"

namespace {

struct AttnK {
    const char* qkv;
    char* out;
    const int64_t* key_mask;
    int nseq, S, n_head, ld, ldo, k_off, v_off, mask_ld, causal;
    float scale;
    const int* cu;
    int only_row0;
    DropArgs drop;
    int split3_w;
};

template <typename T, int NT>
__global__ __launch_bounds__(256, 3) void attention_mfma_kernel(AttnK a) {
    typedef typename OpT<T>::v8 v8;
    constexpr int KS = attn_ksteps(NT), VROWS = 32 * KS, VT = VROWS * ATTN_V_ROW;
    __shared__ __attribute__((aligned(16))) char smem[4 * VT];
    const int lane = threadIdx.x & 63, wave = threadIdx.x >> 6;
    const int npairs = a.nseq * a.n_head;
    const int pair_raw = blockIdx.x * 4 + wave;
    const bool live = pair_raw < npairs;
    const int pair = live ? pair_raw : npairs - 1;
    const int seq = pair / a.n_head, head = pair % a.n_head;
    const int row_first = a.cu ? a.cu[seq] : seq * a.S;
    const int S = a.cu ? min(a.cu[seq + 1] - row_first, 16 * NT) : a.S;
    const T* base = (const T*)a.qkv + (size_t)row_first * a.ld + head * 64;
    const int r16 = lane & 15, q4 = lane >> 4;

    OFX_LDS char* vl = (OFX_LDS char*)smem + wave * VT;
#pragma unroll
    for (int it = 0; it < VROWS / 8; ++it) {
        const int key = it * 8 + (lane >> 3);
        v8 val;
#pragma unroll
        for (int e = 0; e < 8; ++e) val[e] = (T)0.0f;
        if (key < S) val = *(const v8*)(base + (size_t)key * a.ld + a.v_off + (lane & 7) * 8);
        *(OFX_LDS v8*)(vl + key * ATTN_V_ROW + (lane & 7) * 16) = val;
    }

    v8 kf[NT][2], qf[NT][2];
#pragma unroll
    for (int t = 0; t < NT; ++t) {
        int row = 16 * t + r16;
        row = row < S ? row : S - 1;
        const T* rp = base + (size_t)row * a.ld + q4 * 8;
#pragma unroll
        for (int ks = 0; ks < 2; ++ks) {
            kf[t][ks] = *(const v8*)(rp + a.k_off + ks * 32);
            qf[t][ks] = *(const v8*)(rp + ks * 32);
        }
    }

    float neg[NT][4];
#pragma unroll
    for (int t = 0; t < NT; ++t)
#pragma unroll
        for (int r = 0; r < 4; ++r) {
            const int key = 16 * t + 4 * q4 + r;
            bool dead = key >= S;
            if (!dead && a.key_mask) dead = a.key_mask[(size_t)seq * a.mask_ld + key] == 0;
            neg[t][r] = dead ? -INFINITY : 0.f;
        }

    const int nu = a.only_row0 ? 1 : NT;
    f32x4 st[NT][NT];
    attn_scores<T, NT>(st, kf, qf, neg, nu);
    if (a.causal) {
#pragma unroll
        for (int t = 0; t < NT; ++t)
#pragma unroll
            for (int u = 0; u < NT; ++u)
#pragma unroll
                for (int r = 0; r < 4; ++r)
                    if (16 * t + 4 * q4 + r > 16 * u + r16) st[t][u][r] = -INFINITY;
    }
    v8 pf[NT][KS];
    attn_softmax_p<T, NT, true>(pf, st, a.scale, nu, a.drop, pair);
    attn_pv_store<T, NT>(vl, pf, nu, live, (T*)a.out, row_first, a.ldo, head * 64, a.only_row0 ? 1 : S, a.split3_w);
}

struct SetK {
    const void* qkv;
    char* out;
    const int* cu;
    int nseq, n_head, D, ldo, out_kind, only_row0;
    float scale;
    DropArgs drop;
    int fixed_S, causal, mask_ld;
    const int64_t* key_mask;
    int splits; size_t plane; const float* bias;
};

template <typename T, int SMAX, typename TI = float, int HD = 64>
__global__ __launch_bounds__(64) void set_attention_kernel(SetK a) {
    static_assert(HD == 64 || HD == 96, "set_attention: heads of 64 or 96 columns");
    constexpr int STR = HD == 64 ? 68 : 100;
    constexpr int C4 = HD / 4, C8 = HD / 8;
    constexpr bool WIDE = HD > 64;
    __shared__ __attribute__((aligned(16))) float qs[SMAX * STR];
    __shared__ __attribute__((aligned(16))) float ks[SMAX * STR];
    __shared__ __attribute__((aligned(16))) float sc[SMAX * (SMAX + 4)];
    const int lane = threadIdx.x;
    const int b = blockIdx.x / a.n_head, h = blockIdx.x % a.n_head;
    const int r0 = a.cu ? a.cu[b] : b * a.fixed_S;
    int S = a.cu ? a.cu[b + 1] - r0 : a.fixed_S;
    S = S < SMAX ? S : SMAX;
    const int nq = a.only_row0 ? 1 : S;
    const int D = a.D;
    const bool two = WIDE && lane < HD - 64;
    float vreg[SMAX];
    float vreg2[WIDE ? SMAX : 1];
    if (a.splits > 1) {
        constexpr int VS = SMAX <= 32 ? SMAX : 1;
        __shared__ __attribute__((aligned(16))) float vs[VS * STR];
        auto slab_row = [&](int j, int c4) {
            const float* bp = a.bias + h * HD + c4;
            const f32x4 bq = *(const f32x4*)bp, bk = *(const f32x4*)(bp + D), bv = *(const f32x4*)(bp + 2 * D);
            const float* rp = (const float*)a.qkv + (size_t)(r0 + j) * 3 * D + h * HD + c4;
            f32x4 q = {0.f, 0.f, 0.f, 0.f}, kk = *(const f32x4*)(rp + D), vv = *(const f32x4*)(rp + 2 * D);
            if (j < nq) q = *(const f32x4*)rp;
            for (int sl = 1; sl < a.splits; ++sl) {
                const float* sp = rp + sl * a.plane;
                if (j < nq) q += *(const f32x4*)sp;
                kk += *(const f32x4*)(sp + D); vv += *(const f32x4*)(sp + 2 * D);
            }
            if (j < nq) *(f32x4*)(qs + j * STR + c4) = q + bq;
            *(f32x4*)(ks + j * STR + c4) = kk + bk;
            *(f32x4*)(vs + (j % VS) * STR + c4) = vv + bv;
        };
        if constexpr (!WIDE) {
            const int c4 = (lane & 15) * 4, rsub = lane >> 4;
            for (int j0 = 0; j0 < S; j0 += 4) {
                const int j = j0 + rsub;
                if (j < S) slab_row(j, c4);
            }
        } else {
            for (int f = lane; f < S * C4; f += 64) slab_row(f / C4, (f % C4) * 4);
        }
        __syncthreads();
#pragma unroll
        for (int j = 0; j < SMAX; ++j) vreg[j] = j < S ? vs[(j % VS) * STR + lane] : 0.f;
        if constexpr (WIDE) {
#pragma unroll
            for (int j = 0; j < SMAX; ++j) vreg2[j] = (j < S && two) ? vs[(j % VS) * STR + 64 + lane] : 0.f;
        }
    } else if (sizeof(TI) == 4) {
        auto f32_row = [&](int j, int c4) {
            const float* rp = (const float*)a.qkv + (size_t)(r0 + j) * 3 * D + h * HD + c4;
            if (j < nq) *(f32x4*)(qs + j * STR + c4) = *(const f32x4*)rp;
            *(f32x4*)(ks + j * STR + c4) = *(const f32x4*)(rp + D);
        };
        if constexpr (!WIDE) {
            const int c4 = (lane & 15) * 4, rsub = lane >> 4;
            for (int j0 = 0; j0 < S; j0 += 4) {
                const int j = j0 + rsub;
                if (j < S) f32_row(j, c4);
            }
        } else {
            for (int f = lane; f < S * C4; f += 64) f32_row(f / C4, (f % C4) * 4);
        }
#pragma unroll
        for (int j = 0; j < SMAX; ++j) vreg[j] = j < S ? ((const float*)a.qkv)[(size_t)(r0 + j) * 3 * D + 2 * D + h * HD + lane] : 0.f;
        if constexpr (WIDE) {
#pragma unroll
            for (int j = 0; j < SMAX; ++j) vreg2[j] = (j < S && two) ? ((const float*)a.qkv)[(size_t)(r0 + j) * 3 * D + 2 * D + h * HD + 64 + lane] : 0.f;
        }
    } else {
#pragma unroll
        for (int j = 0; j < SMAX; ++j) {
            vreg[j] = 0.f;
            if constexpr (WIDE) vreg2[j] = 0.f;
            if (j < S) {
                const TI* rp = (const TI*)a.qkv + (size_t)(r0 + j) * 3 * D + h * HD + lane;
                if (j < nq) qs[j * STR + lane] = (float)rp[0];
                ks[j * STR + lane] = (float)rp[D];
                vreg[j] = (float)rp[2 * D];
                if constexpr (WIDE) {
                    if (two) {
                        if (j < nq) qs[j * STR + 64 + lane] = (float)rp[64];
                        ks[j * STR + 64 + lane] = (float)rp[D + 64];
                        vreg2[j] = (float)rp[2 * D + 64];
                    }
                }
            }
        }
    }
    __syncthreads();
    for (int p = lane; p < nq * S; p += 64) {
        const int i = p / S, j = p % S;
        const f32x4* qp = (const f32x4*)(qs + i * STR);
        const f32x4* kp = (const f32x4*)(ks + j * STR);
        float d = 0.f;
#pragma unroll
        for (int c = 0; c < C4; ++c) {
            const f32x4 x = qp[c], y = kp[c];
            d += x[0] * y[0] + x[1] * y[1] + x[2] * y[2] + x[3] * y[3];
        }
        bool dead = a.causal && j > i;
        if (!dead && a.key_mask) dead = a.key_mask[(size_t)b * a.mask_ld + j] == 0;
        sc[i * (SMAX + 4) + j] = dead ? -INFINITY : d * a.scale;
    }
    __syncthreads();
    if (lane < nq) {
        float* row = sc + lane * (SMAX + 4);
        float m = -INFINITY;
        for (int j = 0; j < S; ++j) m = fmaxf(m, row[j]);
        if (m == -INFINITY) m = 0.f;
        float sum = 0.f;
        for (int j = 0; j < S; ++j) { const float e = expf(row[j] - m); row[j] = e; sum += e; }
        const float inv = sum > 0.f ? 1.0f / sum : 0.f;
        if (a.drop.thresh) for (int j = 0; j < S; ++j) row[j] *= inv * drop_mul(a.drop, blockIdx.x, lane * 32 + j);
        else for (int j = 0; j < S; ++j) row[j] *= inv;
    }
    __syncthreads();
    if (a.out_kind == 0) {
        for (int i = 0; i < nq; ++i) {
            const float* row = sc + i * (SMAX + 4);
            float acc = 0.f;
#pragma unroll
            for (int j = 0; j < SMAX; ++j) acc += (j < S ? row[j] : 0.f) * vreg[j];
            ((float*)a.out)[(size_t)(r0 + i) * a.ldo + h * HD + lane] = acc;
            if constexpr (WIDE) {
                float acc2 = 0.f;
#pragma unroll
                for (int j = 0; j < SMAX; ++j) acc2 += (j < S ? row[j] : 0.f) * vreg2[j];
                if (two) ((float*)a.out)[(size_t)(r0 + i) * a.ldo + h * HD + 64 + lane] = acc2;
            }
        }
        return;
    }
    for (int i = 0; i < nq; ++i) {
        const float* row = sc + i * (SMAX + 4);
        float acc = 0.f;
#pragma unroll
        for (int j = 0; j < SMAX; ++j) acc += (j < S ? row[j] : 0.f) * vreg[j];
        qs[i * STR + lane] = acc;
        if constexpr (WIDE) {
            float acc2 = 0.f;
#pragma unroll
            for (int j = 0; j < SMAX; ++j) acc2 += (j < S ? row[j] : 0.f) * vreg2[j];
            if (two) qs[i * STR + 64 + lane] = acc2;
        }
    }
    __syncthreads();
    auto store_row = [&](int i, int c8) {
        const f32x4 x0 = *(const f32x4*)(qs + i * STR + c8), x1 = *(const f32x4*)(qs + i * STR + c8 + 4);
        store8<T>(a.out, (size_t)(r0 + i) * a.ldo + h * HD + c8, x0, x1, a.out_kind, D);
    };
    if constexpr (!WIDE) {
        const int c8 = (lane & 7) * 8, r8 = lane >> 3;
        for (int i0 = 0; i0 < nq; i0 += 8) {
            const int i = i0 + r8;
            if (i < nq) store_row(i, c8);
        }
    } else {
        for (int f = lane; f < nq * C8; f += 64) store_row(f / C8, (f % C8) * 8);
    }
}


struct AttnBwdK {
    const char* qkv;
    const float* d_o;
    char* dqkv;
    const int* cu;
    int nseq, n_head, D, only_row0;
    float scale;
    DropArgs drop;
};

__device__ __forceinline__ float drop_dp(float dp, float mk) {
#pragma clang fp contract(off)
    return dp * mk;
}

template <typename T, int NT>
__global__ __launch_bounds__(256) void set_attention_bwd_mfma_kernel(AttnBwdK a) {
    typedef typename OpT<T>::v8 v8;
    typedef typename OpT<T>::v4 v4;
    constexpr int KS = attn_ksteps(NT), VROWS = 32 * KS, VT = VROWS * ATTN_V_ROW;
    __shared__ __attribute__((aligned(16))) char smem[4 * 3 * VT];
    const int lane = threadIdx.x & 63, wave = threadIdx.x >> 6;
    const int npairs = a.nseq * a.n_head;
    const int pair_raw = blockIdx.x * 4 + wave;
    const bool live = pair_raw < npairs;
    const int pair = live ? pair_raw : npairs - 1;
    const int seq = pair / a.n_head, head = pair % a.n_head;
    const int D = a.D, ld = 3 * D;
    const int row_first = a.cu[seq];
    const int S = min(a.cu[seq + 1] - row_first, 16 * NT);
    const T* base = (const T*)a.qkv + (size_t)row_first * ld + head * 64;
    const int r16 = lane & 15, q4 = lane >> 4;
    const int n_go = a.only_row0 ? 1 : S;

    OFX_LDS char* kl = (OFX_LDS char*)smem + wave * 3 * VT;
    OFX_LDS char* ql = kl + VT;
    OFX_LDS char* gl = ql + VT;
#pragma unroll
    for (int it = 0; it < VROWS / 8; ++it) {
        const int row = it * 8 + (lane >> 3), c8 = (lane & 7) * 8;
        v8 kv, qv, gv;
#pragma unroll
        for (int e = 0; e < 8; ++e) { kv[e] = (T)0.0f; qv[e] = (T)0.0f; gv[e] = (T)0.0f; }
        if (row < S) {
            kv = *(const v8*)(base + (size_t)row * ld + D + c8);
            qv = *(const v8*)(base + (size_t)row * ld + c8);
        }
        if (row < n_go) {
            const float* gp = a.d_o + (size_t)(a.only_row0 ? seq : row_first + row) * D + head * 64 + c8;
            const f32x4 g0 = *(const f32x4*)gp, g1 = *(const f32x4*)(gp + 4);
#pragma unroll
            for (int e = 0; e < 4; ++e) { gv[e] = (T)g0[e]; gv[4 + e] = (T)g1[e]; }
        }
        *(OFX_LDS v8*)(kl + row * ATTN_V_ROW + (lane & 7) * 16) = kv;
        *(OFX_LDS v8*)(ql + row * ATTN_V_ROW + (lane & 7) * 16) = qv;
        *(OFX_LDS v8*)(gl + row * ATTN_V_ROW + (lane & 7) * 16) = gv;
    }

    v8 kf[NT][2], qf[NT][2], vf[NT][2], gf[NT][2];
#pragma unroll
    for (int t = 0; t < NT; ++t) {
        const int rowu = 16 * t + r16;
        const int row = rowu < S ? rowu : S - 1;
        const T* rp = base + (size_t)row * ld + q4 * 8;
#pragma unroll
        for (int ks = 0; ks < 2; ++ks) {
            qf[t][ks] = *(const v8*)(rp + ks * 32);
            kf[t][ks] = *(const v8*)(rp + D + ks * 32);
            vf[t][ks] = *(const v8*)(rp + 2 * D + ks * 32);
            v8 g;
#pragma unroll
            for (int e = 0; e < 8; ++e) g[e] = (T)0.0f;
            if (rowu < n_go) {
                const float* gp = a.d_o + (size_t)(a.only_row0 ? seq : row_first + rowu) * D + head * 64 + q4 * 8 + ks * 32;
                const f32x4 g0 = *(const f32x4*)gp, g1 = *(const f32x4*)(gp + 4);
#pragma unroll
                for (int e = 0; e < 4; ++e) { g[e] = (T)g0[e]; g[4 + e] = (T)g1[e]; }
            }
            gf[t][ks] = g;
// ... 75 lines not shown
#pragma unroll
            for (int r = 0; r < 4; ++r) {
                const int query = 16 * u + 4 * q4 + r, key = 16 * t + r16;
                const float mk = a.drop.thresh ? drop_mul(a.drop, pair, query * 32 + key) : 1.0f;
                const float p = key < S ? exp2f(sN[u][t][r] * sc - mq[r]) * iq[r] : 0.f;
                const float dp = drop_dp(pN[u][t][r], mk);
                sN[u][t][r] = p * mk;
                pN[u][t][r] = p * (dp - dq[r]) * a.scale;
            }
    }
#pragma unroll
    for (int t = 0; t < NT; ++t)
#pragma unroll
        for (int ks = 0; ks < KS; ++ks)
#pragma unroll
            for (int j = 0; j < 8; ++j) {
                const int u = 2 * ks + (j >> 2);
                dsN[t][ks][j] = u < NT ? (T)pN[u % NT][t][j & 3] : (T)0.0f;
                pdN[t][ks][j] = u < NT ? (T)sN[u % NT][t][j & 3] : (T)0.0f;
            }

    T* obase = (T*)a.dqkv + (size_t)row_first * ld + head * 64;
    auto product = [&](OFX_LDS char* img, v8 (&bop)[NT][KS], int col_off, int n_rows_out) {
#pragma unroll
        for (int nd = 0; nd < 4; ++nd) {
            v8 af[KS];
#pragma unroll
            for (int ks = 0; ks < KS; ++ks) af[ks] = attn_tr_frag<T>(img, 32 * ks, 16 * nd + 4 * (r16 & 3));
#pragma unroll
            for (int u = 0; u < NT; ++u) {
                f32x4 c = {0.f, 0.f, 0.f, 0.f};
#pragma unroll
                for (int ks = 0; ks < KS; ++ks) c = OpT<T>::mfma16(af[ks], bop[u][ks], c);
                const int orow = 16 * u + r16;
                if (live && orow < n_rows_out) {
                    v4 o;
#pragma unroll
                    for (int r = 0; r < 4; ++r) o[r] = (T)c[r];
                    *(v4*)(obase + (size_t)orow * ld + col_off + 16 * nd + 4 * q4) = o;
                }
            }
        }
    };
    product(kl, dsT, 0, S);
    product(ql, dsN, D, S);
    product(gl, pdN, 2 * D, S);
}

}

int ofx_launch_attention_mfma(const AttnArgs& g, int op_dtype, hipStream_t s) {
    OFX_REQUIRE(g.seq_len >= 1 && g.seq_len <= 64, OFX_ESHAPE, "attention: seq_len=%d must be in [1,64]", g.seq_len);
    OFX_REQUIRE(g.nseq > 0 && g.n_head > 0, OFX_ESHAPE, "attention: nseq=%d n_head=%d", g.nseq, g.n_head);
    OFX_REQUIRE(g.seq_len <= 32 || !g.drop.thresh, OFX_ESHAPE, "attention: dropout columns are keyed query * 32 + key");
    OFX_REQUIRE(g.ld % 8 == 0 && g.ldo % 4 == 0 && g.k_off % 8 == 0 && g.v_off % 8 == 0, OFX_ESHAPE, "attention: strides must keep 16-byte alignment");
    OFX_REQUIRE((uintptr_t)g.qkv % 16 == 0 && (uintptr_t)g.out % 8 == 0, OFX_EINVAL, "attention: misaligned pointers");
    AttnK k;
    k.qkv = (const char*)g.qkv; k.out = (char*)g.out; k.key_mask = g.key_mask; k.nseq = g.nseq; k.S = g.seq_len;
    k.n_head = g.n_head; k.ld = g.ld; k.ldo = g.ldo; k.k_off = g.k_off; k.v_off = g.v_off; k.mask_ld = g.mask_ld;
    k.causal = g.causal; k.scale = g.scale; k.cu = g.cu_seqlens; k.only_row0 = g.only_row0; k.drop = g.drop; k.split3_w = g.split3_w;
    OFX_REQUIRE(g.split3_w == 0 || (g.split3_w % 8 == 0 && g.ldo >= 3 * g.split3_w), OFX_ESHAPE, "attention: split3 output needs ldo >= 3 W");
    const int grid = (g.nseq * g.n_head + 3) / 4;
    ProfScope prof(PROF_ATTN, s);
#define AT(T, N) hipLaunchKernelGGL((attention_mfma_kernel<T, N>), dim3(grid), dim3(256), 0, s, k)
    const int nt = g.seq_len <= 16 ? 1 : g.seq_len <= 32 ? 2 : 4;
    if (op_dtype == OFX_F16) { if (nt == 1) AT(f16_t, 1); else if (nt == 2) AT(f16_t, 2); else AT(f16_t, 4); }
    else { if (nt == 1) AT(bf16_t, 1); else if (nt == 2) AT(bf16_t, 2); else AT(bf16_t, 4); }
#undef AT
    OFX_LAUNCH_CHECK();
    return OFX_OK;
}

int ofx_launch_set_attention(const SetAttnArgs& g, int op_dtype, hipStream_t s) {
    OFX_REQUIRE(g.n_head > 0 && (g.D == g.n_head * 64 || g.D == g.n_head * 96), OFX_ESHAPE, "set_attention: head_dim must be 64 or 96 (D=%d heads=%d)", g.D, g.n_head);
    const bool wide = g.D == g.n_head * 96;
    OFX_REQUIRE(g.max_len >= 1 && g.max_len <= 64, OFX_ESHAPE, "set_attention: %d rows per sequence exceed 64", g.max_len);
    OFX_REQUIRE(g.max_len <= 32 || !g.drop.thresh, OFX_ESHAPE, "set_attention: dropout columns are keyed query * 32 + key");
    OFX_REQUIRE(g.ldo >= (g.out_kind == 2 ? 3 * g.D : g.D) && (g.out_kind == 0 || g.ldo % 8 == 0), OFX_ESHAPE, "set_attention: bad ldo=%d (operand-type rows leave as 16-byte stores)", g.ldo);
    OFX_REQUIRE(g.cu_seqlens || (g.fixed_len >= 1 && g.fixed_len <= g.max_len), OFX_EINVAL, "set_attention: needs cu_seqlens or a fixed length <= max_len");
    SetK k;
    k.qkv = g.qkv; k.out = (char*)g.out; k.cu = g.cu_seqlens; k.nseq = g.nseq; k.n_head = g.n_head; k.D = g.D; k.ldo = g.ldo;
    k.out_kind = g.out_kind; k.only_row0 = g.only_row0; k.scale = g.scale; k.drop = g.drop;
    k.fixed_S = g.fixed_len; k.causal = g.causal; k.mask_ld = g.mask_ld; k.key_mask = g.key_mask;
    OFX_REQUIRE(g.splits <= 1 || (!g.qkv_op && g.bias && g.plane > 0 && g.max_len <= 32), OFX_EINVAL, "set_attention: slab input needs fp32 q|k|v, the bias, the slab stride and sets of <= 32 rows");
    k.splits = g.splits > 1 ? g.splits : 1; k.plane = g.plane; k.bias = g.bias;
    const int grid = g.nseq * g.n_head;
    ProfScope prof(PROF_ATTN, s);
#define SA(T, N) do { if (wide) { if (g.qkv_op) hipLaunchKernelGGL((set_attention_kernel<T, N, T, 96>), dim3(grid), dim3(64), 0, s, k); \
                                      else hipLaunchKernelGGL((set_attention_kernel<T, N, float, 96>), dim3(grid), dim3(64), 0, s, k); } \
                      else if (g.qkv_op) hipLaunchKernelGGL((set_attention_kernel<T, N, T>), dim3(grid), dim3(64), 0, s, k); \
                      else hipLaunchKernelGGL((set_attention_kernel<T, N, float>), dim3(grid), dim3(64), 0, s, k); } while (0)
    if (op_dtype == OFX_F16) { if (g.max_len <= 8) SA(f16_t, 8); else if (g.max_len <= 20) SA(f16_t, 20); else if (g.max_len <= 32) SA(f16_t, 32); else SA(f16_t, 64); }
    else { if (g.max_len <= 8) SA(bf16_t, 8); else if (g.max_len <= 20) SA(bf16_t, 20); else if (g.max_len <= 32) SA(bf16_t, 32); else SA(bf16_t, 64); }
#undef SA
    OFX_LAUNCH_CHECK();
    return OFX_OK;
}

int ofx_launch_set_attention_bwd_mfma(const void* qkv, const float* d_o, void* dqkv, const int* cu, int nseq, int n_head, int D, int max_len,
                                      float scale, int op_dtype, const DropArgs& drop, int only_row0, hipStream_t s) {
    OFX_REQUIRE(D == n_head * 64 && max_len >= 1 && max_len <= 32, OFX_ESHAPE, "set_attention_bwd_mfma: bad shape");
    AttnBwdK k{(const char*)qkv, d_o, (char*)dqkv, cu, nseq, n_head, D, only_row0, scale, drop};
    const int grid = (nseq * n_head + 3) / 4;
    ProfScope prof(PROF_ATTN, s);
#define AB(T, N) hipLaunchKernelGGL((set_attention_bwd_mfma_kernel<T, N>), dim3(grid), dim3(256), 0, s, k)
    if (op_dtype == OFX_F16) { if (max_len <= 16) AB(f16_t, 1); else AB(f16_t, 2); }
    else { if (max_len <= 16) AB(bf16_t, 1); else AB(bf16_t, 2); }
#undef AB
    OFX_LAUNCH_CHECK();
    return OFX_OK;
}
```

outfitx_amd/csrc/norm_act.hip:

```cpp
#include <algorithm>
#include "ofx_common.h"

namespace {

template <typename T, int NCH>
__global__ __launch_bounds__(256) void layernorm_kernel(LnArgs a, const int* rows_dev) {
    const int lane = threadIdx.x & 63, w = threadIdx.x >> 6;
    const int rows = rows_dev ? *rows_dev : a.rows;
    const int D = NCH * 256;
    for (int r = blockIdx.x * 4 + w; r < rows; r += gridDim.x * 4) {
        const int src = a.row_idx ? a.row_idx[r] : r;
        const f32x4* xp = (const f32x4*)(a.x + (size_t)src * D);
        f32x4 v[NCH];
        float s = 0.f;
#pragma unroll
        for (int c = 0; c < NCH; ++c) {
            v[c] = xp[lane + 64 * c];
            s += v[c][0] + v[c][1] + v[c][2] + v[c][3];
        }
        const float mu = wave_sum(s) * (1.0f / D);
        float q = 0.f;
#pragma unroll
        for (int c = 0; c < NCH; ++c) {
            v[c] -= mu;
// ... 122 lines not shown
    else
        hipLaunchKernelGGL(pack_rows_kernel<bf16_t>, dim3(grid), dim3(256), 0, s, src, (bf16_t*)dst, rows_src, rows_dst, K_src, K_dst, ld_src, mode);
    OFX_LAUNCH_CHECK();
    return OFX_OK;
}

namespace {
template <typename T>
__global__ __launch_bounds__(256) void patchify_kernel(const float* px, T* out, int N, int img, int patch) {
    const int g = img / patch;
    const int per_img = 3 * img * img / 8;
    const size_t total = (size_t)N * per_img;
    const int kdim = 3 * patch * patch;
    for (size_t i = blockIdx.x * (size_t)blockDim.x + threadIdx.x; i < total; i += (size_t)gridDim.x * blockDim.x) {
        const int n = (int)(i / per_img);
        int e = (int)(i % per_img) * 8;
        const int c = e / (img * img); e -= c * img * img;
        const int y = e / img, x = e % img;
        const float* sp = px + (size_t)n * 3 * img * img + (size_t)c * img * img + (size_t)y * img + x;
        const f32x4 a = *(const f32x4*)sp, b = *(const f32x4*)(sp + 4);
        const int py = y / patch, ky = y % patch, pxi = x / patch, kx = x % patch;
        typename OpT<T>::v8 v;
#pragma unroll
        for (int k = 0; k < 4; ++k) { v[k] = (T)a[k]; v[4 + k] = (T)b[k]; }
        *(typename OpT<T>::v8*)(out + ((size_t)n * g * g + py * g + pxi) * kdim + c * patch * patch + ky * patch + kx) = v;
    }
}

template <int NCH, typename T>
__global__ __launch_bounds__(256) void vit_embed_ln_kernel(const float* patch_out, const float* cls, const float* pos,
                                                          const float* gamma, const float* beta, float* x, int N, int S,
                                                          float eps, T* xb, float* stat, T* xlo) {
    typedef typename OpT<T>::v4 v4;
    const int lane = threadIdx.x & 63, w = threadIdx.x >> 6;
    const int D = NCH * 256, rows = N * S;
    for (int r = blockIdx.x * 4 + w; r < rows; r += gridDim.x * 4) {
        const int n = r / S, t = r % S;
        const f32x4* sp = (const f32x4*)(t == 0 ? cls : patch_out + ((size_t)n * (S - 1) + t - 1) * D);
        const f32x4* pp = (const f32x4*)(pos + (size_t)t * D);
        f32x4 v[NCH];
        float s = 0.f;
#pragma unroll
        for (int c = 0; c < NCH; ++c) {
            v[c] = sp[lane + 64 * c] + pp[lane + 64 * c];
            s += v[c][0] + v[c][1] + v[c][2] + v[c][3];
        }
        const float mu = wave_sum(s) * (1.0f / D);
        float q = 0.f;
#pragma unroll
        for (int c = 0; c < NCH; ++c) {
            v[c] -= mu;
            q += v[c][0] * v[c][0] + v[c][1] * v[c][1] + v[c][2] * v[c][2] + v[c][3] * v[c][3];
        }
        const float rstd = rsqrtf(wave_sum(q) * (1.0f / D) + eps);
        float so = 0.f;
#pragma unroll
        for (int c = 0; c < NCH; ++c) {
            const int col = (lane + 64 * c) * 4;
            v[c] = v[c] * rstd * *(const f32x4*)(gamma + col) + *(const f32x4*)(beta + col);
            if (x) *(f32x4*)(x + (size_t)r * D + col) = v[c];
            so += (v[c][0] + v[c][1]) + (v[c][2] + v[c][3]);
        }
        if (xb) {
            const float mo = wave_sum(so) * (1.0f / D);
            float qo = 0.f;
#pragma unroll
            for (int c = 0; c < NCH; ++c) {
                const int col = (lane + 64 * c) * 4;
                v4 o;
#pragma unroll
                for (int e = 0; e < 4; ++e) { const float dlt = v[c][e] - mo; qo += dlt * dlt; o[e] = (T)v[c][e]; }
                *(v4*)(xb + (size_t)r * D + col) = o;
                v4 l;
#pragma unroll
                for (int e = 0; e < 4; ++e) l[e] = (T)(v[c][e] - (float)o[e]);
                *(v4*)(xlo + (size_t)r * D + col) = l;
            }
            qo = wave_sum(qo);
            if (lane == 0) { stat[2 * (size_t)r] = mo; stat[2 * (size_t)r + 1] = rsqrtf(qo * (1.0f / D) + eps); }
        }
    }
}

__global__ __launch_bounds__(256) void text_embed_kernel(const int64_t* ids, const float* tok, const float* pos, float* x,
                                                        int N, int T, int Tc, int D, int vocab) {
    const int lane = threadIdx.x & 63, w = threadIdx.x >> 6;
    const int rows = N * Tc;
    for (int r = blockIdx.x * 4 + w; r < rows; r += gridDim.x * 4) {
        const int i = r / Tc, t = r % Tc;
        long long id = ids[(size_t)i * T + t];
        id = id < 0 ? 0 : (id >= vocab ? vocab - 1 : id);
        const f32x4* tp = (const f32x4*)(tok + (size_t)id * D);
        const f32x4* pp = (const f32x4*)(pos + (size_t)t * D);
        for (int c = lane; c < D / 4; c += 64) *(f32x4*)(x + (size_t)r * D + c * 4) = tp[c] + pp[c];
    }
}

__global__ void text_eos_index_kernel(const int64_t* ids, int* row_idx, int N, int T, int Tc, int eos_id) {
    const int i = blockIdx.x * blockDim.x + threadIdx.x;
    if (i >= N) return;
    const int64_t* p = ids + (size_t)i * T;
    int pos = 0;
    if (eos_id == 2) {
        long long best = p[0];
        for (int t = 1; t < T; ++t) if (p[t] > best) { best = p[t]; pos = t; }
    } else {
        for (int t = 0; t < T; ++t) if (p[t] == eos_id) { pos = t; break; }
    }
    row_idx[i] = i * Tc + (pos < Tc ? pos : Tc - 1);
}

__global__ void iota_rows_kernel(int* idx, int n, int stride) {
    const int i = blockIdx.x * blockDim.x + threadIdx.x;
    if (i < n) idx[i] = i * stride;
}

__global__ __launch_bounds__(256) void l2norm_store_kernel(const float* src, float* dst, int rows, int D, int ld, int col,
                                                          int normalize) {
    const int lane = threadIdx.x & 63, w = threadIdx.x >> 6;
    for (int r = blockIdx.x * 4 + w; r < rows; r += gridDim.x * 4) {
        const f32x4* sp = (const f32x4*)(src + (size_t)r * D);
        float q = 0.f;
        for (int c = lane; c < D / 4; c += 64) { f32x4 v = sp[c]; q += v[0] * v[0] + v[1] * v[1] + v[2] * v[2] + v[3] * v[3]; }
        const float inv = normalize ? 1.0f / fmaxf(sqrtf(wave_sum(q)), 1e-12f) : 1.0f;
        for (int c = lane; c < D / 4; c += 64) *(f32x4*)(dst + (size_t)r * ld + col + c * 4) = sp[c] * inv;
    }
}

__global__ __launch_bounds__(1024) void set_offsets_kernel(const uint8_t* mask, int* cu, int B, int L) {
    __shared__ int part[1024];
    const int t = threadIdx.x, per = (B + 1023) / 1024;
    int cnt = 0;
    for (int b = t * per; b < min(B, (t + 1) * per); ++b) {
        int c = 1;
        for (int l = 0; l < L; ++l) c += mask[(size_t)b * L + l] == 0;
        cnt += c;
    }
    part[t] = cnt;
    __syncthreads();
    for (int o = 1; o < 1024; o <<= 1) {
        int v = t >= o ? part[t - o] : 0;
        __syncthreads();
        part[t] += v;
        __syncthreads();
    }
    int run = t ? part[t - 1] : 0;
    for (int b = t * per; b < min(B, (t + 1) * per); ++b) {
        cu[b] = run;
        int c = 1;
        for (int l = 0; l < L; ++l) c += mask[(size_t)b * L + l] == 0;
        run += c;
    }
    if (t == 1023) cu[B] = part[1023];
}

__global__ __launch_bounds__(256) void set_build_kernel(const float* x, const uint8_t* mask, const float* prefix,
                                                       int prefix_stride, const int* cu, float* X, int B, int L, int D) {
    const int lane = threadIdx.x & 63, w = threadIdx.x >> 6;
    const int slots = B * (L + 1);
    for (int s = blockIdx.x * 4 + w; s < slots; s += gridDim.x * 4) {
        const int b = s / (L + 1), l = s % (L + 1) - 1;
        const float* src;
        int dst;
        if (l < 0) {
            src = prefix + (size_t)b * prefix_stride;
            dst = cu[b];
        } else {
            if (mask[(size_t)b * L + l]) continue;
            int k = 0;
            for (int j = 0; j < l; ++j) k += mask[(size_t)b * L + j] == 0;
            src = x + ((size_t)b * L + l) * D;
            dst = cu[b] + 1 + k;
        }
        for (int c = lane; c < D / 4; c += 64) *(f32x4*)(X + (size_t)dst * D + c * 4) = *(const f32x4*)(src + c * 4);
    }
}

__global__ __launch_bounds__(256) void set_build_indexed_kernel(const float* table, int ld, long long n_table, const int* idx, const int* cu_items,
                                                               const float* prefix, int prefix_stride, int* cu_rows, float* X, int B, int D) {
    const int lane = threadIdx.x & 63, w = threadIdx.x >> 6;
    for (int b = blockIdx.x * 4 + w; b < B; b += gridDim.x * 4) {
        const int i0 = cu_items[b], n = cu_items[b + 1] - i0, r0 = i0 + b;
        if (lane == 0) { cu_rows[b] = r0; if (b == B - 1) cu_rows[B] = cu_items[B] + B; }
        const float* pp = prefix + (size_t)b * prefix_stride;
        for (int c = lane; c < D / 4; c += 64) *(f32x4*)(X + (size_t)r0 * D + c * 4) = *(const f32x4*)(pp + c * 4);
        for (int j = 0; j < n; ++j) {
            long long t = idx[i0 + j];
            t = t < 0 ? 0 : (t >= n_table ? n_table - 1 : t);
            const float* src = table + (size_t)t * ld;
            for (int c = lane; c < D / 4; c += 64) *(f32x4*)(X + (size_t)(r0 + 1 + j) * D + c * 4) = *(const f32x4*)(src + c * 4);
        }
    }
// ... 64 lines not shown
    if (r >= rows) return;
    const float* p = part + (size_t)r * slots * 2;
    float s = 0.f, q = 0.f;
    for (int k = 0; k < slots; ++k) { s += p[2 * k]; q += p[2 * k + 1]; }
    const float mu = s / W;
    const float var = fmaxf(q / W - mu * mu, 0.f);
    stat[2 * (size_t)r] = mu;
    stat[2 * (size_t)r + 1] = rsqrtf(var + eps);
}
template <typename T>
__global__ __launch_bounds__(256) void fold_pack_kernel(const float* Wsrc, const float* gamma, const float* beta, const float* bias, T* Wf,
                                                       float* col_sum, float* bias_f, int N, int K, int split) {
    const int lane = threadIdx.x & 63, w = threadIdx.x >> 6;
    const int ld = split ? 2 * K : K;
    for (int n = blockIdx.x * 4 + w; n < N; n += gridDim.x * 4) {
        float cs = 0.f, bb = 0.f;
        for (int k = lane; k < K; k += 64) {
            const float wv = Wsrc[(size_t)n * K + k];
            float wg = wv * gamma[k];
            asm volatile("" : "+v"(wg));
            const T r = (T)wg;
            Wf[(size_t)n * ld + k] = r;
            cs += (float)r;
            if (split) {
                const T lo = (T)(wg - (float)r);
                Wf[(size_t)n * ld + K + k] = lo;
                cs += (float)lo;
            }
            bb += beta[k] * wv;
        }
        cs = wave_sum(cs); bb = wave_sum(bb);
        if (lane == 0) { col_sum[n] = cs; bias_f[n] = bias[n] + bb; }
    }
}

struct MultiCopyEntry { const float* src; float* dst; long long n; };
struct MultiCopyTable { MultiCopyEntry e[128]; };
__global__ __launch_bounds__(256) void multi_copy_kernel(const MultiCopyTable table) {
    const MultiCopyEntry e = table.e[blockIdx.x];
    for (long long i = (long long)blockIdx.y * 256 + threadIdx.x; i < e.n; i += (long long)gridDim.y * 256) e.dst[i] = e.src[i];
}

__global__ __launch_bounds__(256) void cp_head_kernel(const float* row0, const float* w, const float* bias, float* logits, int B, int D) {
    const int lane = threadIdx.x & 63, wv = threadIdx.x >> 6;
    for (int b = blockIdx.x * 4 + wv; b < B; b += gridDim.x * 4) {
        float s = 0.f;
        for (int c = lane; c < D / 4; c += 64) {
            const f32x4 a = *(const f32x4*)(row0 + (size_t)b * D + c * 4), k = *(const f32x4*)(w + c * 4);
            s += a[0] * k[0] + a[1] * k[1] + a[2] * k[2] + a[3] * k[3];
        }
        s = wave_sum(s);
        if (lane == 0) logits[b] = s + bias[0];
    }
}
}

static inline int rows_grid(int rows) { int g = (rows + 3) / 4; return g > 8192 ? 8192 : (g < 1 ? 1 : g); }

int ofx_launch_patchify(const float* px, void* out, int N, int img, int patch, int op_dtype, hipStream_t s) {
    OFX_REQUIRE(img % patch == 0 && img % 8 == 0 && patch % 8 == 0, OFX_ESHAPE, "patchify: img=%d patch=%d", img, patch);
    size_t total = (size_t)N * 3 * img * img / 8;
    int grid = (int)((total + 255) / 256);
    if (grid > 32768) grid = 32768;
    ProfScope prof(PROF_OTHER, s);
    if (op_dtype == OFX_F16) hipLaunchKernelGGL(patchify_kernel<f16_t>, dim3(grid), dim3(256), 0, s, px, (f16_t*)out, N, img, patch);
    else hipLaunchKernelGGL(patchify_kernel<bf16_t>, dim3(grid), dim3(256), 0, s, px, (bf16_t*)out, N, img, patch);
    OFX_LAUNCH_CHECK();
    return OFX_OK;
}
int ofx_launch_vit_embed_ln(const float* patch_out, const float* cls, const float* pos, const float* g, const float* b,
                            float* x, int N, int S, int D, float eps, hipStream_t s, void* xb, float* stat, int op_dtype, void* xlo) {
    OFX_REQUIRE(D == 768 || D == 512 || D == 1024, OFX_ESHAPE, "vit_embed_ln: D=%d", D);
    OFX_REQUIRE(x ? !xb && !stat && !xlo : xb && stat && xlo, OFX_EINVAL, "vit_embed_ln: writes either x or the (xb, xlo) stream + stat");
    const int grid = rows_grid(N * S);
    ProfScope prof(PROF_NORM, s);
#define VEL(NCH, T) hipLaunchKernelGGL((vit_embed_ln_kernel<NCH, T>), dim3(grid), dim3(256), 0, s, patch_out, cls, pos, g, b, x, N, S, eps, (T*)xb, stat, (T*)xlo)
    if (op_dtype == OFX_F16) { if (D == 768) VEL(3, f16_t); else if (D == 512) VEL(2, f16_t); else VEL(4, f16_t); }
    else { if (D == 768) VEL(3, bf16_t); else if (D == 512) VEL(2, bf16_t); else VEL(4, bf16_t); }
#undef VEL
    OFX_LAUNCH_CHECK();
    return OFX_OK;
}
int ofx_launch_text_embed(const int64_t* ids, const float* tok, const float* pos, float* x, int N, int T, int Tc, int D,
                          int vocab, hipStream_t s) {
    hipLaunchKernelGGL(text_embed_kernel, dim3(rows_grid(N * Tc)), dim3(256), 0, s, ids, tok, pos, x, N, T, Tc, D, vocab);
    OFX_LAUNCH_CHECK();
    return OFX_OK;
}
int ofx_launch_text_eos_index(const int64_t* ids, int* row_idx, int N, int T, int Tc, int eos_id, hipStream_t s) {
    hipLaunchKernelGGL(text_eos_index_kernel, dim3((N + 255) / 256), dim3(256), 0, s, ids, row_idx, N, T, Tc, eos_id);
    OFX_LAUNCH_CHECK();
    return OFX_OK;
}
int ofx_launch_iota_rows(int* idx, int n, int stride, hipStream_t s) {
    hipLaunchKernelGGL(iota_rows_kernel, dim3((n + 255) / 256), dim3(256), 0, s, idx, n, stride);
    OFX_LAUNCH_CHECK();
    return OFX_OK;
}
int ofx_launch_l2norm_store(const float* src, float* dst, int rows, int D, int ld, int col, int normalize, hipStream_t s) {
    OFX_REQUIRE(D % 4 == 0 && ld % 4 == 0 && col % 4 == 0, OFX_ESHAPE, "l2norm_store: D/ld/col must be multiples of 4");
    hipLaunchKernelGGL(l2norm_store_kernel, dim3(rows_grid(rows)), dim3(256), 0, s, src, dst, rows, D, ld, col, normalize);
    OFX_LAUNCH_CHECK();
    return OFX_OK;
}
int ofx_launch_set_build(const float* x, const uint8_t* mask, const float* prefix, int prefix_stride, int* cu, float* X,
                         int B, int L, int D, hipStream_t s) {
    OFX_REQUIRE(B > 0 && B <= 65536 * 16 && L >= 0 && D % 4 == 0, OFX_ESHAPE, "set_build: B=%d L=%d D=%d", B, L, D);
    hipLaunchKernelGGL(set_offsets_kernel, dim3(1), dim3(1024), 0, s, mask, cu, B, L);
    hipLaunchKernelGGL(set_build_kernel, dim3(rows_grid(B * (L + 1))), dim3(256), 0, s, x, mask, prefix, prefix_stride, cu, X, B, L, D);
    OFX_LAUNCH_CHECK();
    return OFX_OK;
}
int ofx_launch_set_build_indexed(const float* table, int ld, long long n_table, const int* idx, const int* cu_items, const float* prefix,
                                 int prefix_stride, int* cu_rows, float* X, int B, int D, hipStream_t s) {
    OFX_REQUIRE(B > 0 && D % 4 == 0 && ld % 4 == 0 && ld >= D && n_table > 0, OFX_ESHAPE, "set_build_indexed: B=%d D=%d ld=%d", B, D, ld);
    ProfScope prof(PROF_OTHER, s);
    hipLaunchKernelGGL(set_build_indexed_kernel, dim3(rows_grid(B)), dim3(256), 0, s, table, ld, n_table, idx, cu_items, prefix, prefix_stride, cu_rows, X, B, D);
    OFX_LAUNCH_CHECK();
    return OFX_OK;
}
int ofx_launch_gather_rows(const void* src, const int* idx, void* dst, int rows, int row_bytes, int src_ld_bytes, hipStream_t s) {
    OFX_REQUIRE(row_bytes % 16 == 0 && src_ld_bytes % 16 == 0, OFX_ESHAPE, "gather_rows: row bytes must be multiples of 16");
    ProfScope prof(PROF_OTHER, s);
    hipLaunchKernelGGL(gather_rows_kernel, dim3(rows_grid(rows)), dim3(256), 0, s, (const char*)src, idx, (char*)dst, rows, row_bytes, src_ld_bytes);
    OFX_LAUNCH_CHECK();
    return OFX_OK;
}
int ofx_launch_gather_hilo(const void* hi, const void* lo, const int* idx, float* dst, int rows, int W, int op_dtype, hipStream_t s) {
    OFX_REQUIRE(W % 4 == 0 && rows > 0, OFX_ESHAPE, "gather_hilo: rows=%d W=%d", rows, W);
    if (op_dtype == OFX_F16) hipLaunchKernelGGL(gather_hilo_kernel<f16_t>, dim3(rows_grid(rows)), dim3(256), 0, s, (const f16_t*)hi, (const f16_t*)lo, idx, dst, rows, W);
    else hipLaunchKernelGGL(gather_hilo_kernel<bf16_t>, dim3(rows_grid(rows)), dim3(256), 0, s, (const bf16_t*)hi, (const bf16_t*)lo, idx, dst, rows, W);
    OFX_LAUNCH_CHECK();
    return OFX_OK;
}
int ofx_launch_row_stats_cast(const float* X, void* Xb, void* Xlo, float* stat, int rows, int W, float eps, int op_dtype, hipStream_t s) {
    OFX_REQUIRE(W % 4 == 0 && rows > 0, OFX_ESHAPE, "row_stats_cast: rows=%d W=%d", rows, W);
    OFX_REQUIRE(Xb && Xlo && stat, OFX_EINVAL, "row_stats_cast: the (hi, lo) pair and the statistics are all written");
    ProfScope prof(PROF_NORM, s);
    if (op_dtype == OFX_F16) hipLaunchKernelGGL(row_stats_cast_kernel<f16_t>, dim3(rows_grid(rows)), dim3(256), 0, s, X, (f16_t*)Xb, stat, rows, W, eps, (f16_t*)Xlo);
    else hipLaunchKernelGGL(row_stats_cast_kernel<bf16_t>, dim3(rows_grid(rows)), dim3(256), 0, s, X, (bf16_t*)Xb, stat, rows, W, eps, (bf16_t*)Xlo);
    OFX_LAUNCH_CHECK();
    return OFX_OK;
}
int ofx_launch_stats_finalize(const float* part, int slots, int W, float eps, float* stat, int rows, hipStream_t s) {
    ProfScope prof(PROF_NORM, s);
    hipLaunchKernelGGL(stats_finalize_kernel, dim3((rows + 255) / 256), dim3(256), 0, s, part, slots, W, eps, stat, rows);
    OFX_LAUNCH_CHECK();
    return OFX_OK;
}
int ofx_launch_fold_pack(const float* Wsrc, const float* gamma, const float* beta, const float* bias, void* Wf, float* col_sum, float* bias_f,
                         int N, int K, int op_dtype, hipStream_t s, int split) {
    if (op_dtype == OFX_F16) hipLaunchKernelGGL(fold_pack_kernel<f16_t>, dim3(rows_grid(N)), dim3(256), 0, s, Wsrc, gamma, beta, bias, (f16_t*)Wf, col_sum, bias_f, N, K, split);
    else hipLaunchKernelGGL(fold_pack_kernel<bf16_t>, dim3(rows_grid(N)), dim3(256), 0, s, Wsrc, gamma, beta, bias, (bf16_t*)Wf, col_sum, bias_f, N, K, split);
    OFX_LAUNCH_CHECK();
    return OFX_OK;
}
int ofx_launch_multi_copy(const void* table_host, int n, hipStream_t s) {
    const MultiCopyEntry* src = (const MultiCopyEntry*)table_host;
    for (int i0 = 0; i0 < n; i0 += 128) {
        MultiCopyTable t;
        const int m = n - i0 < 128 ? n - i0 : 128;
        for (int i = 0; i < m; ++i) t.e[i] = src[i0 + i];
        hipLaunchKernelGGL(multi_copy_kernel, dim3(m, 64), dim3(256), 0, s, t);
    }
    OFX_LAUNCH_CHECK();
    return OFX_OK;
}
namespace {
__global__ __launch_bounds__(256) void fill_f32_kernel(float* p, size_t n, float v) {
    for (size_t i = blockIdx.x * (size_t)256 + threadIdx.x; i < n; i += (size_t)gridDim.x * 256) p[i] = v;
}
}
int ofx_launch_fill_f32(float* p, size_t n, float v, hipStream_t s) {
// ... 16 lines not shown
```

outfitx_amd/csrc/ofx_common.h:

```cpp
#pragma once
#include <hip/hip_runtime.h>
#include <hip/hip_ext.h>
#include <mutex>
#include <stdint.h>
#include <stdio.h>

#include "../../include/ofx.h"
#include "gemm_plan.h"

typedef __bf16 bf16_t;
typedef _Float16 f16_t;
typedef __bf16 bf16x8 __attribute__((ext_vector_type(8)));
typedef __bf16 bf16x4 __attribute__((ext_vector_type(4)));
typedef _Float16 f16x8 __attribute__((ext_vector_type(8)));
typedef _Float16 f16x4 __attribute__((ext_vector_type(4)));
typedef float f32x4 __attribute__((ext_vector_type(4)));
typedef float f32x2 __attribute__((ext_vector_type(2)));
typedef float f32x16 __attribute__((ext_vector_type(16)));
typedef short s16x4 __attribute__((ext_vector_type(4)));
typedef short s16x8 __attribute__((ext_vector_type(8)));

#define OFX_LDS __attribute__((address_space(3)))
#define OFX_GLB __attribute__((address_space(1)))

// ... 202 lines not shown
    return h;
}
__host__ __device__ __forceinline__ float drop_mul(const DropArgs& d, unsigned row, unsigned col) {
    unsigned h = ofx_fmix32(d.seed + d.site * 0x9E3779B9u + row * 0x632BE5ABu);
    h = ofx_fmix32(h ^ (col * 0x9E3779B1u + 0x7F4A7C15u));
    return h >= d.thresh ? d.scale : 0.0f;
}
__host__ __device__ __forceinline__ unsigned ofx_draw_u32(unsigned seed, unsigned draw, unsigned stream, unsigned b, unsigned i) {
    unsigned h = ofx_fmix32(seed + 0x6A09E667u);
    h = ofx_fmix32(h ^ draw);
    h = ofx_fmix32(h + stream * 0x9E3779B9u + 0x7F4A7C15u);
    h = ofx_fmix32(h ^ (b * 0x632BE5ABu));
    return ofx_fmix32(h + i * 0x9E3779B1u);
}
__host__ __device__ __forceinline__ unsigned ofx_draw_below(unsigned u, unsigned n) { return (unsigned)(((unsigned long long)u * n) >> 32); }
inline DropArgs make_drop(float p, unsigned seed, unsigned site) {
    DropArgs d;
    if (p > 0.f) { d.seed = seed; d.site = site; d.thresh = (unsigned)((double)p * 4294967296.0); d.scale = 1.0f / (1.0f - p); }
    return d;
}

struct GemmArgs {
    const void* A;
    const void* W;
    void* C;
    const float* bias;
    const float* resid;
    const int* m_dev = nullptr;
    float* aux_out = nullptr;
    void* slab = nullptr;
    size_t slab_bytes = 0;
    int M, N, K, lda, ldc, ldr;
    int act;
    int out_kind;
    DropArgs drop;
    void* xb_out = nullptr;
    float* stat_part = nullptr;
    const float* row_stat = nullptr;
    int stat_ld = 1;
    void* xlo = nullptr;
    const float* col_sum = nullptr;
    int a_wrap = 0;
    const void* W8 = nullptr; const void* w8_scale = nullptr;
    int k_mult = 1;
    int* defer_splits = nullptr;
    const float* ln_gamma = nullptr; const float* ln_beta = nullptr; void* ln_out = nullptr; int ln_ld = 0, ln_kind = 0; float ln_eps = 0.f;
    bool* ln_done = nullptr;
};
int ofx_launch_gemm(const GemmArgs& g, int op_dtype , hipStream_t s);
size_t ofx_gemm_splitk_bytes(int M, int N, int K);
int ofx_gemm_tune(int knob, int value);

struct LnArgs {
    const float* x;
    const int* row_idx;
    const float* gamma;
    const float* beta;
    void* y;
    int rows, D, ldy;
    int out_kind;
    float eps;
    float* stats = nullptr;
};
size_t ofx_gemm_tn_slab_bytes(int M, int N, int K);
int ofx_launch_gemm_tn(const void* A, int lda, const void* B, int ldb, float* C, int ldc, int M, int N, int K, const int* k_dev,
                       void* slab, size_t slab_bytes, int op_dtype, hipStream_t s, int m_valid = 0, int n_valid = 0, int accumulate = 0);
int ofx_launch_layernorm(const LnArgs& a, int op_dtype, hipStream_t s);
struct SplitKLnArgs {
    const float* slab; size_t plane; int splits;
    const float* bias; const float* resid; int ldr;
    float* x; int ldx;
    const float* gamma; const float* beta; void* y; int ldy, out_kind; float eps;
    int rows, D; const int* m_dev;
};
int ofx_launch_splitk_reduce_ln(const SplitKLnArgs& a, int op_dtype, hipStream_t s, bool in_gemm_scope = false);
int ofx_launch_layernorm_dev(const LnArgs& a, const int* rows_dev, int op_dtype, hipStream_t s);
int ofx_launch_pack_lo8(const void* w2_rows, void* dst8, void* scale8, int N, int K, hipStream_t s);
int ofx_launch_pack_rows(const float* src, void* dst, int rows_src, int rows_dst, int K_src, int K_dst, int ld_src,
                         int mode, int op_dtype, hipStream_t s);
int ofx_launch_patchify(const float* px, void* out, int N, int img, int patch, int op_dtype, hipStream_t s);
int ofx_launch_vit_embed_ln(const float* patch_out, const float* cls, const float* pos, const float* g, const float* b,
                            float* x, int N, int S, int D, float eps, hipStream_t s, void* xb, float* stat, int op_dtype, void* xlo);
int ofx_launch_text_embed(const int64_t* ids, const float* tok, const float* pos, float* x, int N, int T, int Tc, int D,
                          int vocab, hipStream_t s);
int ofx_launch_text_eos_index(const int64_t* ids, int* row_idx, int N, int T, int Tc, int eos_id, hipStream_t s);
int ofx_launch_iota_rows(int* idx, int n, int stride, hipStream_t s);
int ofx_launch_l2norm_store(const float* src, float* dst, int rows, int D, int ld, int col, int normalize, hipStream_t s);
int ofx_launch_set_build(const float* x, const uint8_t* mask, const float* prefix, int prefix_stride, int* cu, float* X,
                         int B, int L, int D, hipStream_t s);
int ofx_launch_gather_rows(const void* src, const int* idx, void* dst, int rows, int row_bytes, int src_ld_bytes, hipStream_t s);
int ofx_launch_set_build_indexed(const float* table, int ld, long long n_table, const int* idx, const int* cu_items, const float* prefix,
                                 int prefix_stride, int* cu_rows, float* X, int B, int D, hipStream_t s);
int ofx_preprocess_to(const uint8_t* src, const long long* offsets, const int* heights, const int* widths, int N, int channels, int size,
                      const float* mean, const float* stdv, float* out, void* patches, int patch, int op_dtype, void* ws, size_t ws_bytes, hipStream_t stream);
int ofx_launch_row_stats_cast(const float* X, void* Xb, void* Xlo, float* stat, int rows, int W, float eps, int op_dtype, hipStream_t s);
int ofx_launch_gather_hilo(const void* hi, const void* lo, const int* idx, float* dst, int rows, int W, int op_dtype, hipStream_t s);
int ofx_launch_stats_finalize(const float* part, int slots, int W, float eps, float* stat, int rows, hipStream_t s);
int ofx_launch_fold_pack(const float* Wsrc, const float* gamma, const float* beta, const float* bias, void* Wf, float* col_sum, float* bias_f,
                         int N, int K, int op_dtype, hipStream_t s, int split = 0);
int ofx_launch_cir_prefix(const float* img_emb, const float* txt, float* out, int B, int D, hipStream_t s);
int ofx_launch_cp_head(const float* row0, const float* w, const float* bias, float* logits, int B, int D, hipStream_t s);

struct CirSampleArgs {
    const int *outfit_cu, *outfit_rows, *pos_cu, *pos_slots, *pool_cu, *pool_rows, *row_pool, *row_slot, *outfit_ids;
    int n_outfits, n_outfit_rows, n_pos_slots, n_pools, n_pool_rows, n_table, B, K, max_len;
    unsigned seed, draw;
    int *item_index, *cu_seqlens, *target_item_index, *neg_items_index;
};
int ofx_launch_cir_sample_batch(const CirSampleArgs& a, hipStream_t s);

struct AttnArgs {
    const void* qkv;
    void* out;
    const int64_t* key_mask;
    int nseq, seq_len, n_head, ld, ldo, k_off, v_off, mask_ld;
    int causal;
    float scale;
    const int* cu_seqlens = nullptr;
    int only_row0 = 0;
    DropArgs drop;
    int split3_w = 0;
};
int ofx_launch_attention_mfma(const AttnArgs& a, int op_dtype, hipStream_t s);

struct SetAttnArgs {
    const void* qkv;
    void* out;
    const int* cu_seqlens;
    int nseq, n_head, D, ldo, out_kind;
    int max_len;
    int only_row0;
    float scale;
    DropArgs drop;
    int qkv_op = 0;
    int fixed_len = 0, causal = 0, mask_ld = 0;
    const int64_t* key_mask = nullptr;
    int splits = 1; size_t plane = 0; const float* bias = nullptr;
};
int ofx_launch_set_attention(const SetAttnArgs& a, int op_dtype, hipStream_t s);
int ofx_launch_fused_qkv_attn(const void* X, const void* Wqkv, const float* bias, const float* row_stat, const float* col_sum, void* out,
                              int n_img, int S, int Wm, int heads, int ldx, int ldo, float scale, int op_dtype, hipStream_t s, bool w2 = false);

int ofx_launch_multi_copy(const void* table_host, int n, hipStream_t s);
int ofx_launch_fill_f32(float* p, size_t n, float v, hipStream_t s);
int ofx_launch_transpose_cast(const float* src, void* dst, int R, int C, int ldd, int op_dtype, hipStream_t s, void* row_dst = nullptr, int ld_row = 0);
size_t ofx_colsum_part_floats(int C);
int ofx_launch_colsum(const void* x, int x_kind, int ld, const int* gather, const float* row_scale, float* out0, float* out1, float* out2, int seg,
                      float* part, int C, const int* m_dev, int M, int op_dtype, hipStream_t s, int valid = 0, int accumulate = 0);
size_t ofx_ln_bwd_part_floats(int D);
int ofx_launch_row_map(const int* cu, int* map, int B, int M, hipStream_t s);
int ofx_launch_ln_bwd(const float* dy, const float* x, const float* stats, const float* gamma, const float* add, const int* add_map, float* dx_out, void* dx_op,
                      float* dgamma, float* dbeta, float* dcols, float* part, int D, const int* m_dev, int M, int op_dtype, const DropArgs& drop, hipStream_t s,
                      int accumulate = 0);
int ofx_launch_set_attention_bwd(const void* qkv, const float* d_o, void* dqkv, const int* cu, int nseq, int n_head, int D, int max_len,
                                 float scale, int op_dtype, const DropArgs& drop, int only_row0, hipStream_t s);
int ofx_launch_set_attention_bwd_mfma(const void* qkv, const float* d_o, void* dqkv, const int* cu, int nseq, int n_head, int D, int max_len,
                                      float scale, int op_dtype, const DropArgs& drop, int only_row0, hipStream_t s);
int ofx_launch_drop_rows(float* x, int rows, int cols, const DropArgs& d, hipStream_t s);
int ofx_launch_focal_loss(const float* logits, const float* labels, int B, float alpha, float gamma, float upstream, float* loss, float* dlogits, hipStream_t s,
                          int reduction = 1, float* per_elem = nullptr);
size_t ofx_set_rank_loss_ws(int B, int K);
int ofx_launch_set_rank_loss(const float* y, const float* y_hat, const float* neg, const uint8_t* mask, int B, int K, int D, float margin, float upstream,
                             float* loss, float* dy_hat, float* d_pos, float* d_neg, void* ws, hipStream_t s);
int ofx_launch_set_rank_loss_indexed(const float* table, int ld, int n_table, const int* pos_index, const int* neg_index, const float* y_hat, int B, int K,
                                     int D, float margin, float upstream, float* loss, float* dy_hat, float* d_pos, float* d_neg, void* ws, hipStream_t s);
size_t ofx_adamw_step_ws(long long n_arena);
int ofx_launch_adamw_step(const ofx_opt_segment* segments, int n_segments, float* grad, float* exp_avg, float* exp_avg_sq, long long n_arena,
                          float* step, double lr, double beta1, double beta2, double eps, double weight_decay, double max_norm, double grad_scale,
                          float* grad_norm, int* skipped, void* ws, hipStream_t s);
int ofx_launch_cp_head_bwd(const float* dlogits, const float* w_or_rows, const int* cu, float* dX, void* dXb, float* db, int B, int D, int op_dtype,
                           const DropArgs& head, const DropArgs& below, hipStream_t s, int accumulate = 0);
int ofx_launch_fitb(const float* y, const float* cand, int B, int C, int D, int64_t* idx, float* dist, hipStream_t s);
int ofx_launch_fitb_indexed(const float* table, int ld, int n_table, const int* cand_index, const float* y, int B, int C, int D, const int64_t* answer,
                            int64_t* idx, float* dist, int* n_correct, hipStream_t s);
int ofx_launch_l2_topk(const float* Q, const float* P, int nq, int np, int D, int k, int64_t index_base, int64_t* idx,
                       float* dist, void* ws, size_t ws_bytes, hipStream_t s);
size_t ofx_l2_topk_ws(int nq, int np);
int ofx_launch_l2_topk_grouped(const float* Q, const float* P, int nq, int np, int D, int k, const int* panels, int n_panels, int max_group_rows,
                               const int64_t* gt, int64_t* idx, float* dist, int* gt_pos, void* ws, size_t ws_bytes, hipStream_t s);
int ofx_launch_topk_merge(const int64_t* idx_in, const float* dist_in, int parts, int nq, int k, int64_t* idx, float* dist,
                          hipStream_t s);

extern int g_topk_filter;
```

outfitx_amd/encoders.py:

```python
from __future__ import annotations

import ctypes as C
import itertools
import warnings
from types import SimpleNamespace
from typing import Any, Dict, List, Optional, Sequence, Tuple, Union

import numpy as np
import torch
from PIL import Image
from torch import nn

from . import _lib as L
from .configs import ItemEncoderConfig
from .engine import Engine

CLIP_MEAN = (0.48145466, 0.4578275, 0.40821073)
CLIP_STD = (0.26862954, 0.26130258, 0.27577711)


def freeze_model(model: nn.Module) -> None:
    for p in model.parameters():
        p.requires_grad = False


def flatten_seq_to_one_dim(sequences: List[List[Any]]) -> List[Any]:
    return list(itertools.chain(*sequences))


def aggregate_embeddings(image_embeddings=None, text_embeddings=None, aggregation_method: str = "concat"):
    embeds = [e for e in (image_embeddings, text_embeddings) if e is not None]
    if not embeds:
        raise ValueError("At least one of image_embeds or text_embeds must be provided.")
    if aggregation_method == "concat":
        return torch.cat(embeds, dim=-1)
    if aggregation_method == "mean":
        return torch.mean(torch.stack(embeds), dim=-2)
    raise ValueError(f"Unsupported aggregation method: {aggregation_method}. Use 'concat' or 'mean'.")


class _ClipAttentionParams(nn.Module):
    def __init__(self, width):
        super().__init__()
        self.k_proj = nn.Linear(width, width)
        self.v_proj = nn.Linear(width, width)
        self.q_proj = nn.Linear(width, width)
        self.out_proj = nn.Linear(width, width)


class _ClipMlpParams(nn.Module):
    def __init__(self, width, mlp):
        super().__init__()
        self.fc1 = nn.Linear(width, mlp)
        self.fc2 = nn.Linear(mlp, width)


class _ClipLayerParams(nn.Module):
    def __init__(self, width, mlp, eps):
        super().__init__()
        self.self_attn = _ClipAttentionParams(width)
        self.layer_norm1 = nn.LayerNorm(width, eps=eps)
        self.mlp = _ClipMlpParams(width, mlp)
        self.layer_norm2 = nn.LayerNorm(width, eps=eps)


class _ClipEncoderParams(nn.Module):
    def __init__(self, width, mlp, n_layers, eps):
        super().__init__()
        self.layers = nn.ModuleList([_ClipLayerParams(width, mlp, eps) for _ in range(n_layers)])


def _layer_tensors(layer: _ClipLayerParams) -> List[torch.Tensor]:
    a, m = layer.self_attn, layer.mlp
    return [a.k_proj.weight, a.k_proj.bias, a.v_proj.weight, a.v_proj.bias, a.q_proj.weight, a.q_proj.bias,
            a.out_proj.weight, a.out_proj.bias, layer.layer_norm1.weight, layer.layer_norm1.bias,
            m.fc1.weight, m.fc1.bias, m.fc2.weight, m.fc2.bias, layer.layer_norm2.weight, layer.layer_norm2.bias]


class _VisionEmbeddingParams(nn.Module):
    def __init__(self, width, patch, image):
        super().__init__()
        self.class_embedding = nn.Parameter(torch.randn(width))
        self.patch_embedding = nn.Conv2d(3, width, kernel_size=patch, stride=patch, bias=False)
        self.position_embedding = nn.Embedding((image // patch) ** 2 + 1, width)


class _VisionTransformerParams(nn.Module):
    def __init__(self, c):
        super().__init__()
        self.embeddings = _VisionEmbeddingParams(c.hidden_size, c.patch_size, c.image_size)
        self.pre_layrnorm = nn.LayerNorm(c.hidden_size, eps=c.layer_norm_eps)
        self.encoder = _ClipEncoderParams(c.hidden_size, c.intermediate_size, c.num_hidden_layers, c.layer_norm_eps)
        self.post_layernorm = nn.LayerNorm(c.hidden_size, eps=c.layer_norm_eps)


class ClipVisionParams(nn.Module):

    def __init__(self, **over):
# ... 179 lines not shown
                    eng.vit(px[a:b], out[a:b], col, normalize)
            for i in range(self.vit_streams):
                cur.wait_stream(pool[i])
        elif arrs is None:
            eng.vit(px, out, col, normalize)
        elif self.fused_preprocess:
            eng.vit_u8(arrs, CLIP_MEAN, CLIP_STD, out, col, normalize)
        else:
            eng.vit(eng.clip_preprocess(arrs, self.model.config.image_size, CLIP_MEAN, CLIP_STD), out, col, normalize)

    fused_preprocess = True

    @torch.no_grad()
    def encode_into(self, images, out: torch.Tensor, col: int, normalize: bool) -> int:
        px, arrs, b = self._pixels(images)
        self._run(px, arrs, out, col, normalize)
        return b

    @torch.no_grad()
    def forward(self, images, normalize: bool = True, *args, **kwargs) -> torch.Tensor:
        px, arrs, b = self._pixels(images)
        n = px.shape[0] if arrs is None else len(arrs)
        out = torch.empty(n, self.d_embed, dtype=torch.float32, device=self.device)
        self._run(px, arrs, out, 0, normalize)
        return out.view(b, -1, self.d_embed)


class CLIPTextEncoder(_TowerBase):

    def __init__(self, model_name_or_path: str = "patrickjohncyh/fashion-clip", freeze: bool = True):
        super().__init__()
        self.model = ClipTextParams()
        self.pretrained = _try_load_pretrained(self.model, "CLIPTextModelWithProjection", model_name_or_path)
        if not self.pretrained:
            warnings.warn(f"CLIP text checkpoint '{model_name_or_path}' not available offline: random-initialised",
                          stacklevel=2)
        self.model.eval()
        if freeze:
            freeze_model(self.model)
        self._tok_name = model_name_or_path
        self.tokenizer = None
        self.dedup_texts = False
        self.cache_texts = False
        self._cache_rows: dict = {}
        self._cache_table: Optional[torch.Tensor] = None
        self._cache_state = None
        self.cache_tower_rows = 0

    def _desc(self) -> L.ModelDesc:
        d, c = L.default_desc(), self.model.config
        d.txt_width, d.txt_layers, d.txt_heads, d.txt_mlp = c.hidden_size, c.num_hidden_layers, c.num_attention_heads, c.intermediate_size
        d.txt_vocab, d.txt_max_pos, d.proj_dim, d.ln_eps = c.vocab_size, c.max_position_embeddings, c.projection_dim, c.layer_norm_eps
        d.txt_act, d.txt_eos_id = L.ACTS[c.hidden_act], c.eos_token_id
        return d

    @property
    def d_embed(self) -> int:
        return self.model.config.projection_dim

    def _tokenize(self, texts: List[str], tokenizer_kargs: Optional[dict]):
        if self.tokenizer is None:
            try:
                from transformers import CLIPTokenizer
                self.tokenizer = CLIPTokenizer.from_pretrained(self._tok_name)
            except Exception as e:
                raise RuntimeError("CLIP tokenizer files are not available; pass pre-tokenised "
                                   "{'input_ids','attention_mask'} tensors instead of strings") from e
        kw = tokenizer_kargs if tokenizer_kargs is not None else {"max_length": 64, "padding": "max_length", "truncation": True}
        kw["return_tensors"] = "pt"
        enc = self.tokenizer(text=texts, **kw)
        return enc["input_ids"], enc["attention_mask"]

    def _ids(self, texts, tokenizer_kargs=None):
        if isinstance(texts, dict):
            ids = texts["input_ids"]
            b, l = ids.size(0), ids.size(1)
            att = texts.get("attention_mask")
            return ids.reshape(b * l, -1), None if att is None else att.reshape(b * l, -1), b
        if len(set(len(seq) for seq in texts)) != 1:
            raise ValueError("All sequences in texts should have the same length.")
        ids, att = self._tokenize(flatten_seq_to_one_dim(texts), tokenizer_kargs)
        return ids, att, len(texts)

    def _lengths(self, ids: torch.Tensor):
        if ids.device.type != "cpu":
            return None
        eos = self.model.config.eos_token_id
        pos = ids.argmax(-1) if eos == 2 else (ids == eos).int().argmax(-1)
        return (pos + 1).tolist()

    def _dedup(self, ids: torch.Tensor, att: Optional[torch.Tensor]):
        if not self.dedup_texts or ids.device.type != "cpu" or ids.shape[0] < 2:
            return None
        a = ids.numpy()
        key = a if att is None else a * 2 + att.numpy().astype(a.dtype)
        w = getattr(self, "_hash_w", None)
        if w is None or w.shape[0] != key.shape[1]:
            w = np.random.default_rng(0x5EED).integers(1, 2 ** 62, key.shape[1], dtype=np.int64) | 1
            self._hash_w = w
        h = (key.astype(np.int64) * w).sum(1)
        _, first, inv = np.unique(h, return_index=True, return_inverse=True)
        if first.shape[0] == key.shape[0] or not np.array_equal(key[first][inv], key):
            return None
        first_t = torch.from_numpy(first)
        uniq_ids = ids.index_select(0, first_t)
        uniq_att = None if att is None else att.index_select(0, first_t)
        return uniq_ids.contiguous(), (None if uniq_att is None else uniq_att.contiguous()), torch.from_numpy(inv.astype(np.int64))

    def _cache_plan(self, ids: torch.Tensor, att: Optional[torch.Tensor]):
        a = ids.numpy()
        key = a if att is None else a * 2 + att.numpy().astype(a.dtype)
        rows = np.empty(a.shape[0], np.int64)
        slot0 = len(self._cache_rows)
        miss, new_keys, pending = [], [], {}
        for i in range(a.shape[0]):
            k = key[i].tobytes()
            r = self._cache_rows.get(k)
            if r is None:
                r = pending.get(k)
                if r is None:
                    r = pending[k] = slot0 + len(miss)
                    miss.append(i)
                    new_keys.append(k)
            rows[i] = r
        return rows, miss, new_keys, slot0

    @torch.no_grad()
    def prepare(self, texts, tokenizer_kargs=None):
        ids, att, b = self._ids(texts, tokenizer_kargs)
        inverse = None
        if self.cache_texts and ids.device.type == "cpu":
            state = tuple(p._version for p in self.model.parameters())
            if state != self._cache_state:
                self._cache_rows, self._cache_table, self._cache_state = {}, None, state
            rows, miss, new_keys, slot0 = self._cache_plan(ids, att)
            plan = {"rows": torch.from_numpy(rows).to(self.device, non_blocking=True), "slot0": slot0, "n_new": len(miss), "new_keys": new_keys}
            if miss:
                sel = torch.as_tensor(miss, dtype=torch.long)
                m_ids = ids.index_select(0, sel).contiguous()
                m_att = None if att is None else att.index_select(0, sel).contiguous()
                plan["lengths"] = self._lengths(m_ids)
                plan["ids"], plan["att"] = self._engine("text").stage_tokens(m_ids, m_att)
            return None, None, None, b, plan
        dd = self._dedup(ids, att)
        if dd is not None:
            ids, att, inverse = dd
            inverse = inverse.to(self.device, non_blocking=True)
        lengths = self._lengths(ids)
        ids_d, att_d = self._engine("text").stage_tokens(ids, att)
        return ids_d, att_d, lengths, b, inverse

    def _run(self, ids, att, lengths, inverse, out: torch.Tensor, col: int, normalize: bool) -> None:
        eng = self._engine("text")
        if isinstance(inverse, dict):
            plan, d = inverse, self.d_embed
            if self._cache_table is not None and getattr(self, "_cache_norm", normalize) != normalize:
                raise ValueError("cache_texts: the cache was filled with normalize=%s; clear it (set cache_texts again) before changing the flag" % (not normalize))
            self._cache_norm = normalize
            if plan["slot0"] != len(self._cache_rows):
                raise RuntimeError("cache_texts: this prepared batch is stale (another batch was prepared and run, or the cache was cleared, since prepare()); prepare it again")
            need = plan["slot0"] + plan["n_new"]
            if self._cache_table is None or self._cache_table.shape[0] < need:
                grown = torch.empty(max(need, 256, 2 * (0 if self._cache_table is None else self._cache_table.shape[0])), d, dtype=torch.float32, device=self.device)
                if self._cache_table is not None:
                    grown[:self._cache_table.shape[0]] = self._cache_table
                self._cache_table = grown
            if plan["n_new"]:
                eng.text(plan["ids"], plan["att"], self._cache_table[plan["slot0"]:need], 0, normalize, plan["lengths"])
                for j, k in enumerate(plan["new_keys"]):
                    self._cache_rows[k] = plan["slot0"] + j
                self.cache_tower_rows += plan["n_new"]
            out[:, col:col + d] = self._cache_table.index_select(0, plan["rows"])
            return
        if inverse is None:
            eng.text(ids, att, out, col, normalize, lengths)
            return
        uniq = torch.empty(ids.shape[0], self.d_embed, dtype=torch.float32, device=self.device)
        eng.text(ids, att, uniq, 0, normalize, lengths)
        out[:, col:col + self.d_embed] = uniq.index_select(0, inverse)

    @torch.no_grad()
    def encode_into(self, texts, out: torch.Tensor, col: int, normalize: bool, tokenizer_kargs=None, prepared=None) -> int:
        ids, att, lengths, b, inverse = prepared if prepared is not None else self.prepare(texts, tokenizer_kargs)
        self._run(ids, att, lengths, inverse, out, col, normalize)
        return b

    @torch.no_grad()
    def forward(self, texts, normalize: bool = True, *args, **kwargs) -> torch.Tensor:
        ids, att, lengths, b, inverse = self.prepare(texts, kwargs.get("tokenizer_kargs"))
        n = inverse["rows"].shape[0] if isinstance(inverse, dict) else (ids.shape[0] if inverse is None else inverse.shape[0])
        out = torch.empty(n, self.d_embed, dtype=torch.float32, device=self.device)
        self._run(ids, att, lengths, inverse, out, 0, normalize)
        return out.view(b, -1, self.d_embed)


class ItemEncoder(nn.Module):

    def __init__(self, cfg: ItemEncoderConfig):
        super().__init__()
        self.cfg = cfg
        if cfg.type != "clip":
            raise NotImplementedError(
                f"ItemEncoderConfig(type='{cfg.type}') is outside the MI355X scoring path; build the model with "
                "OutfitXConfig(item_encoder=ItemEncoderConfig(type='clip')), or - for precomputed embeddings only - OutfitX(cfg, item_towers=False)")
        self.image_enc = CLIPImageEncoder(model_name_or_path=cfg.clip_model_name)
        self.text_enc = CLIPTextEncoder(model_name_or_path=cfg.clip_model_name)
        self.overlap_towers = True
        self.side_stream_priority = "normal"
        self._streams: Dict[Any, Any] = {}

    def _side_stream(self, dev):
        key = (dev, self.side_stream_priority)
        s = self._streams.get(key)
        if s is None:
            if self.side_stream_priority == "low":
                raw = C.c_void_p()
                L.check(L.load().ofx_stream_create_low_priority(dev.index if dev.index is not None else torch.cuda.current_device(), C.byref(raw)),
                        "ofx_stream_create_low_priority")
                s = torch.cuda.ExternalStream(raw.value, device=dev)
            else:
                s = torch.cuda.Stream(device=dev)
            self._streams[key] = s
        return s

    def __getstate__(self):
        s = self.__dict__.copy()
        s["_streams"] = {}
        return s

    @property
    def d_embed(self) -> int:
# ... 72 lines not shown
```

outfitx_amd/engine.py:

```python
from __future__ import annotations

import ctypes as C
from typing import Dict, List, NamedTuple, Optional, Sequence

import torch

from . import _lib as L


def _ptr(t: Optional[torch.Tensor]) -> Optional[int]:
    return None if t is None else t.data_ptr()


def _stream(device: torch.device) -> int:
    return torch.cuda.current_stream(device).cuda_stream


def _f32c(t: torch.Tensor, device) -> torch.Tensor:
    if t.device != device or t.dtype != torch.float32 or not t.is_contiguous():
        t = t.to(device=device, dtype=torch.float32).contiguous()
    return t


class SetInput(NamedTuple):
    B: int
    L: int
    staged: tuple
    args: tuple

    @property
    def indexed(self) -> bool:
        return self.args[0] is None


class Engine:

    def __init__(self, device: torch.device, desc: Optional[L.ModelDesc] = None,
                 precision: str = "bf16x3", tower_precision: str = L.DEFAULT_TOWER_PRECISION):
        self.lib = L.load()
        if device.type != "cuda":
            raise L.OfxError(f"outfitx_amd runs on an MI355X HIP device only (got {device}); there is no CPU path")
        self.device = torch.device("cuda", device.index if device.index is not None else torch.cuda.current_device())
        d = desc if desc is not None else L.default_desc()
        d.outfit_precision = L.PRECISIONS[precision]
        for k, v in L.tower_scheme(tower_precision).items():
            setattr(d, k, v)
        self.desc = d
        self.h = self.lib.ofx_create(self.device.index, C.byref(d))
        if not self.h:
            raise L.OfxError("ofx_create failed: " + self.lib.ofx_last_error().decode())
        self._ws: Dict[int, torch.Tensor] = {}
        self._keep: List[torch.Tensor] = []
        self.signature = {"outfit": None, "vision": None, "text": None}

    def __del__(self):
        try:
            if getattr(self, "h", None):
                self.lib.ofx_destroy(self.h)
                self.h = None
        except Exception:
            pass

    def _pack(self, fn, tensors: Sequence[torch.Tensor], what: str):
        ts = [_f32c(t.detach(), self.device) for t in tensors]
        arr = (C.c_void_p * len(ts))(*[t.data_ptr() for t in ts])
        with torch.cuda.device(self.device):
            L.check(fn(self.h, arr, len(ts), _stream(self.device)), f"ofx_pack_{what}_weights")
        self._keep = [t for t in ts]

    def pack_outfit(self, tensors): self._pack(self.lib.ofx_pack_outfit_weights, tensors, "outfit")
    def pack_vision(self, tensors): self._pack(self.lib.ofx_pack_vision_weights, tensors, "vision")
    def pack_text(self, tensors): self._pack(self.lib.ofx_pack_text_weights, tensors, "text")

    def workspace(self, nbytes: int) -> torch.Tensor:
        key = _stream(self.device)
        ws = self._ws.get(key)
        if ws is None or ws.numel() < nbytes:
            ws = torch.empty(int(nbytes * 1.05) + 4096, dtype=torch.uint8, device=self.device)
            self._ws[key] = ws
        return ws

    def ws_bytes(self, op: int, n: int, length: int) -> int:
        return int(self.lib.ofx_workspace_bytes(self.h, op, n, length))

    @staticmethod
    def cir_sample_batch(split: Dict[str, torch.Tensor], pools: Dict[str, torch.Tensor], outfit_ids: torch.Tensor, seed: int, draw: int, K: int,
                         max_len: int, n_pool_rows: Optional[int] = None):
        lib = L.load()
        dev = split["outfit_cu"].device
        if dev.type != "cuda":
            raise L.OfxError("cir_sample_batch needs HIP tensors; there is no CPU path")
        ts = [split[k] for k in ("outfit_cu", "outfit_rows", "pos_cu", "pos_slots")] + [pools[k] for k in ("pool_cu", "pool_rows", "row_pool", "row_slot")]
        for t in ts:
            if t.device != dev or t.dtype != torch.int32 or not t.is_contiguous():
                raise ValueError(f"cir_sample_batch: every table must be a contiguous int32 tensor on {dev}")
        ocu, orows, pcu, pslots, gcu, grows, rpool, rslot = ts
        if rpool.numel() != rslot.numel() or pcu.numel() != ocu.numel():
            raise ValueError("cir_sample_batch: row_pool / row_slot or outfit_cu / pos_cu differ in length")
        ids = outfit_ids if isinstance(outfit_ids, torch.Tensor) else torch.as_tensor(outfit_ids)
        ids = ids.reshape(-1).to(device=dev, dtype=torch.int32).contiguous()
        if ids.data_ptr() % 16:
            ids = ids.clone()
        B, K, max_len = ids.numel(), int(K), int(max_len)
        item_index = torch.empty(max(B * max_len, 1), dtype=torch.int32, device=dev)
# ... 123 lines not shown
            L.check(getattr(self.lib, name)(self.h, _ptr(tape), tape.numel(), _ptr(d), B, Lq, *sink, _ptr(ws), ws.numel(),
                                            float(dropout_p), int(seed) & 0xFFFFFFFF, _stream(self.device)), name)
        return g

    def arm_layer_events(self, events) -> None:
        arr = (C.c_void_p * len(events))(*[int(e.cuda_event) for e in events])
        L.check(self.lib.ofx_train_arm_layer_events(self.h, arr, len(events)), "ofx_train_arm_layer_events")

    def vit(self, pixels: torch.Tensor, out: torch.Tensor, col: int, normalize: bool) -> None:
        px = _f32c(pixels, self.device)
        N = px.shape[0]
        nb = self.ws_bytes(L.OP_VIT, N, 0)
        ws = self.workspace(nb)
        with torch.cuda.device(self.device):
            L.check(self.lib.ofx_vit_b32_fwd(self.h, _ptr(px), N, _ptr(out), out.stride(0), col, int(normalize),
                                             _ptr(ws), ws.numel(), _stream(self.device)), "ofx_vit_b32_fwd")

    def _stage_images(self, images: Sequence):
        import numpy as np
        arrs = []
        for a in images:
            a = np.asarray(a)
            if a.dtype != np.uint8 or a.ndim not in (2, 3) or (a.ndim == 3 and a.shape[2] != 3):
                raise ValueError(f"clip_preprocess takes uint8 [H,W,3] or [H,W] images, got {a.dtype} {a.shape}")
            arrs.append(np.repeat(a[:, :, None], 3, 2) if a.ndim == 2 else a)
        N = len(arrs)
        hs = np.asarray([a.shape[0] for a in arrs], np.int32); ws_ = np.asarray([a.shape[1] for a in arrs], np.int32)
        nbytes = hs.astype(np.int64) * ws_ * 3
        offs = np.zeros(N, np.int64); offs[1:] = np.cumsum((nbytes[:-1] + 15) // 16 * 16)
        total = int(offs[-1] + nbytes[-1])
        stage = getattr(self, "_px_stage", None)
        if stage is None or stage.numel() < total + 4:
            stage = torch.empty(int(total * 1.25) + 4096, dtype=torch.uint8).pin_memory()
            self._px_stage = stage
        elif getattr(self, "_px_event", None) is not None:
            self._px_event.synchronize()
        buf = stage.numpy()
        for a, o, n in zip(arrs, offs, nbytes):
            buf[o:o + n] = a.reshape(-1)
        src = stage[:total + 4].to(self.device, non_blocking=True)
        self._px_event = torch.cuda.Event()
        self._px_event.record(torch.cuda.current_stream(self.device))
        self._keep_px = src
        return src, offs, hs, ws_

    def clip_preprocess(self, images: Sequence, size: int, mean: Sequence[float], std: Sequence[float]) -> torch.Tensor:
        src, offs, hs, ws_ = self._stage_images(images)
        N = len(hs)
        out = torch.empty(N, 3, size, size, dtype=torch.float32, device=self.device)
        I = C.POINTER(C.c_int); LL = C.POINTER(C.c_longlong)
        nb = int(self.lib.ofx_clip_preprocess_ws(hs.ctypes.data_as(I), ws_.ctypes.data_as(I), N, 3, size))
        ws = self.workspace(nb)
        m = (C.c_float * 3)(*mean); sd = (C.c_float * 3)(*std)
        with torch.cuda.device(self.device):
            L.check(self.lib.ofx_clip_preprocess(_ptr(src), offs.ctypes.data_as(LL), hs.ctypes.data_as(I), ws_.ctypes.data_as(I), N, 3, size,
                                                 m, sd, _ptr(out), _ptr(ws), ws.numel(), _stream(self.device)), "ofx_clip_preprocess")
        return out

    def vit_u8(self, images: Sequence, mean: Sequence[float], std: Sequence[float], out: torch.Tensor, col: int, normalize: bool) -> None:
        src, offs, hs, ws_ = self._stage_images(images)
        N = len(hs)
        I = C.POINTER(C.c_int); LL = C.POINTER(C.c_longlong)
        nb = int(self.lib.ofx_vit_b32_u8_ws_bytes(self.h, hs.ctypes.data_as(I), ws_.ctypes.data_as(I), N, 3))
        if nb == 0:
            raise ValueError("ofx_vit_b32_u8_ws_bytes: bad image geometry")
        ws = self.workspace(nb)
        m = (C.c_float * 3)(*mean); sd = (C.c_float * 3)(*std)
        with torch.cuda.device(self.device):
            L.check(self.lib.ofx_vit_b32_fwd_u8(self.h, _ptr(src), offs.ctypes.data_as(LL), hs.ctypes.data_as(I), ws_.ctypes.data_as(I), N, 3,
                                                m, sd, _ptr(out), out.stride(0), col, int(normalize), _ptr(ws), ws.numel(),
                                                _stream(self.device)), "ofx_vit_b32_fwd_u8")

    def stage_tokens(self, ids: torch.Tensor, att: Optional[torch.Tensor]):
        def mv(t):
            if t is None:
                return None
            if t.device == self.device and t.dtype == torch.int64 and t.is_contiguous():
                return t
            return t.to(device=self.device, dtype=torch.int64, non_blocking=t.device.type == "cpu" and t.is_pinned()).contiguous()
        return mv(ids), mv(att)

    def text(self, ids: torch.Tensor, att: Optional[torch.Tensor], out: torch.Tensor, col: int, normalize: bool,
             lengths: Optional[Sequence[int]] = None) -> None:
        ids_d, att_d = self.stage_tokens(ids, att)
        N, T = ids_d.shape
        Tc = T if lengths is None else max(1, min(T, max(int(v) for v in lengths)))
        arr = None if lengths is None else (C.c_int * N)(*[int(v) for v in lengths])
        nb = self.ws_bytes(L.OP_TEXT, N, Tc)
        ws = self.workspace(nb)
        with torch.cuda.device(self.device):
            L.check(self.lib.ofx_clip_text_fwd(self.h, _ptr(ids_d), _ptr(att_d), arr, N, T, _ptr(out), out.stride(0), col,
                                               int(normalize), _ptr(ws), ws.numel(), _stream(self.device)), "ofx_clip_text_fwd")
        self._keep_ids = (ids_d, att_d)

    def l2_topk(self, Q: torch.Tensor, P: torch.Tensor, k: int, index_base: int = 0):
        Q = _f32c(Q, self.device); P = _f32c(P, self.device)
        nq, D = Q.shape
        npool = P.shape[0]
        idx = torch.empty(nq, k, dtype=torch.int64, device=self.device)
        dist = torch.empty(nq, k, dtype=torch.float32, device=self.device)
        ws = self.workspace(self.ws_bytes(L.OP_TOPK, nq, npool))
        with torch.cuda.device(self.device):
            L.check(self.lib.ofx_l2_topk(self.h, _ptr(Q), _ptr(P), nq, npool, D, k, index_base, _ptr(idx), _ptr(dist),
                                         _ptr(ws), ws.numel(), _stream(self.device)), "ofx_l2_topk")
        return idx, dist

    def l2_topk_grouped(self, Q: torch.Tensor, group_of_query, P: torch.Tensor, pool_offsets, k: int, gt=None, max_ws_bytes: int = 1 << 30):
        Q = _f32c(Q, self.device); P = _f32c(P, self.device)
        nq, D = Q.shape
        npool = P.shape[0]
        grp = torch.as_tensor(group_of_query, device="cpu").to(torch.int64).reshape(-1)
        off = torch.as_tensor(pool_offsets, device="cpu").to(torch.int64).reshape(-1)
        G = off.numel() - 1
        if G < 1 or int(off[0]) != 0 or int(off[-1]) != npool or bool((off[1:] < off[:-1]).any()):
            raise ValueError("pool_offsets must start at 0, be non-decreasing and end at len(P)")
        if grp.numel() != nq:
            raise ValueError(f"group_of_query has {grp.numel()} entries for {nq} queries")
        if nq and (int(grp.min()) < 0 or int(grp.max()) >= G):
            raise ValueError(f"group_of_query must lie in [0, {G})")
        q_lo, q_hi = off[grp], off[grp + 1]
        if bool((q_hi == q_lo).any()):
            raise ValueError("a query's pool is empty")
        gt_h = None
        if gt is not None:
            gt_h = torch.as_tensor(gt).to(device="cpu", dtype=torch.int64).reshape(-1)
            if gt_h.numel() != nq:
                raise ValueError(f"gt has {gt_h.numel()} entries for {nq} queries")
            if bool(((gt_h >= 0) & ((gt_h < q_lo) | (gt_h >= q_hi))).any()):
                raise ValueError("a gt row lies outside its query's pool")
        idx = torch.empty(nq, k, dtype=torch.int64, device=self.device)
        dist = torch.empty(nq, k, dtype=torch.float32, device=self.device)
        gt_pos = torch.empty(nq, dtype=torch.int32, device=self.device) if gt_h is not None else None
        if nq == 0:
            return idx, dist, gt_pos
        max_rows = int((q_hi - q_lo).max())
        need = lambda n: int(self.lib.ofx_l2_topk_grouped_ws(n, npool, max_rows))
        if need(1) > max_ws_bytes:
            raise ValueError(f"max_ws_bytes={max_ws_bytes}: one query against {max_rows} rows needs {need(1)} bytes")
        lo, hi = 1, nq
        while lo < hi:
            mid = (lo + hi + 1) // 2
            lo, hi = (mid, hi) if need(mid) <= max_ws_bytes else (lo, mid - 1)
        n_chunks = -(-nq // lo)
        chunk = -(-nq // n_chunks)
        order = torch.argsort(grp, stable=True)
        table, chunk_panels = _group_panels(grp[order], off, chunk)
        table = table.to(self.device)
        order_d = order.to(self.device)
        Qs = Q.index_select(0, order_d)
        gt_s = gt_h[order].to(self.device) if gt_h is not None else None
        idx_s, dist_s = torch.empty_like(idx), torch.empty_like(dist)
        pos_s = torch.empty_like(gt_pos) if gt_pos is not None else None
        ws = self.workspace(need(chunk))
        with torch.cuda.device(self.device):
            for c0, c1, first, n_panels in chunk_panels:
                L.check(self.lib.ofx_l2_topk_grouped(self.h, _ptr(Qs[c0:c1]), _ptr(P), c1 - c0, npool, D, k, _ptr(table[first:]), n_panels, max_rows,
                                                     _ptr(gt_s[c0:c1]) if gt_s is not None else None, _ptr(idx_s[c0:c1]), _ptr(dist_s[c0:c1]),
                                                     _ptr(pos_s[c0:c1]) if pos_s is not None else None, _ptr(ws), ws.numel(), _stream(self.device)),
                        "ofx_l2_topk_grouped")
        idx[order_d] = idx_s
        dist[order_d] = dist_s
        if gt_pos is not None:
            gt_pos[order_d] = pos_s
            if bool((gt_h < 0).any()):
                gt_pos.masked_fill_(gt_h.to(self.device) < 0, -1)
        return idx, dist, gt_pos


def _group_panels(sorted_groups: torch.Tensor, offsets: torch.Tensor, chunk: int):
    nq, G = sorted_groups.numel(), offsets.numel() - 1
    cnt = torch.bincount(sorted_groups, minlength=G)
    start = torch.cumsum(cnt, 0) - cnt
    cuts = [torch.arange(s, s + n, 128) for s, n in zip(start.tolist(), cnt.tolist()) if n]
    calls = torch.arange(0, nq, chunk)
    lo = torch.unique(torch.cat(cuts + [calls]))
# ... 188 lines not shown
```

outfitx_amd/graphs.py:

```python
from __future__ import annotations

from typing import Any, Callable, Optional

import torch


class CapturedCall:

    def __init__(self, fn: Callable[[], Any], device: torch.device, warmup: int = 2, inputs: Optional[dict] = None):
        if device.type != "cuda":
            raise ValueError("CapturedCall needs a HIP device")
        self.inputs = inputs or {}
        self.device = device
        self.check: Optional[Callable[[], None]] = None
        self._graph = torch.cuda.CUDAGraph()
        cur = torch.cuda.current_stream(device)
        cap = torch.cuda.Stream(device)
        cap.wait_stream(cur)
        with torch.cuda.stream(cap), torch.no_grad():
            for _ in range(max(1, warmup)):
                fn()
        cur.wait_stream(cap)
        torch.cuda.synchronize(device)
        with torch.no_grad(), torch.cuda.graph(self._graph, stream=cap, capture_error_mode="thread_local"):
            self.output = fn()
        torch.cuda.synchronize(device)
        self.replays = 0

    def replay(self):
        if self.check is not None:
            self.check()
        self._graph.replay()
        self.replays += 1
        return self.output


def capture_cp_forward(model, outfit_mask: torch.Tensor, images: torch.Tensor, texts: dict, warmup: int = 2) -> CapturedCall:
    from .datatypes import OutfitCompatibilityPredictionTask as CP
    if model.training:
        raise ValueError("capture_cp_forward: put the model in eval() mode (the training step is not capturable: its parameters change)")
    if not isinstance(images, torch.Tensor) or images.device.type != "cuda":
        raise ValueError("capture_cp_forward: images must be a device tensor (host preprocessing cannot be captured)")
    for k, v in texts.items():
        if isinstance(v, torch.Tensor) and v.device.type == "cpu" and not v.is_pinned():
            raise ValueError(f"capture_cp_forward: texts['{k}'] lives in pageable host memory; pin it (or move it to the device) - a pageable copy is synchronous and cannot be captured")

    enc = model.item_encoder.text_enc
    if enc.dedup_texts or enc.cache_texts:
        raise ValueError("capture_cp_forward: turn text_enc.dedup_texts / cache_texts off - their row maps are computed on the host per batch and would be frozen into the graph")

    def fn():
        return model(task=CP, outfit_embedding=None, outfit_mask=outfit_mask, encoder_input_dict={"images": images, "texts": texts})

    was = getattr(model, "graph_replay", False)
    model.graph_replay = False
    try:
        cc = CapturedCall(fn, images.device, warmup, inputs={"images": images, "texts": texts, "outfit_mask": outfit_mask})
    finally:
        model.graph_replay = was
    ids = texts["input_ids"]
    if ids.device.type == "cpu":
        flat = ids.reshape(-1, ids.shape[-1])
        cc.captured_tokens = max(1, min(flat.shape[1], max(enc._lengths(flat))))

        def check():
            now = max(enc._lengths(flat))
            if now > cc.captured_tokens:
                raise ValueError(f"replay: a token row of {now} positions, but the graph was captured for {cc.captured_tokens}: capture again (a longer row would be silently truncated)")
        cc.check = check
    return cc


class ForwardReplay:

    def __init__(self, capacity: int = 2, capture_after: int = 2):
        self.capacity, self.capture_after = capacity, capture_after
        self.entries: dict = {}
        self.seen: dict = {}
        self.failed: set = set()
        self.stats = {"eager": 0, "captures": 0, "replays": 0, "capture_failures": 0}

    def clear(self) -> None:
        self.entries.clear()
        self.seen.clear()
        self.failed.clear()

    @staticmethod
    def eligible(model, outfit_mask, enc_in) -> bool:
        if not isinstance(enc_in, dict) or set(enc_in) - {"images", "texts"}:
            return False
        images, texts = enc_in.get("images"), enc_in.get("texts")
        if not (isinstance(images, torch.Tensor) and images.device.type == "cuda" and images.is_contiguous() and images.dim() == 5):
            return False
        if not (isinstance(texts, dict) and isinstance(texts.get("input_ids"), torch.Tensor) and texts["input_ids"].dim() == 3):
            return False
        att = texts.get("attention_mask")
        if att is not None and not (isinstance(att, torch.Tensor) and att.shape == texts["input_ids"].shape):
            return False
        if not (isinstance(outfit_mask, torch.Tensor) and outfit_mask.dim() == 2):
            return False
        enc = model.item_encoder
        if enc.text_enc.dedup_texts or enc.text_enc.cache_texts or enc.cfg.aggregation_method != "concat":
            return False
        return not torch.cuda.is_current_stream_capturing()

    def run(self, model, outfit_mask, enc_in, eager: Callable[[], torch.Tensor]):
        from . import _lib as L
        lib = L.load()
        if lib.ofx_profile_enabled():
            return eager()
        images, texts = enc_in["images"], enc_in["texts"]
        ids, att = texts["input_ids"], texts.get("attention_mask")
        enc = model.item_encoder
        T = ids.shape[-1]
        tokens = T
        if ids.device.type == "cpu":
            tokens = max(1, min(T, max(enc.text_enc._lengths(ids.reshape(-1, T)))))
        key = (images.data_ptr(), tuple(images.shape), images.dtype, tuple(ids.shape), att is not None, tokens, tuple(outfit_mask.shape),
               model.precision, model.tower_fed_precision, enc.image_enc.tower_precision, enc.text_enc.tower_precision, enc.overlap_towers, enc.side_stream_priority,
               enc.image_enc.vit_streams, lib.ofx_config_generation(), torch.cuda.current_stream(images.device).cuda_stream)
        sig = tuple((p.data_ptr(), p._version) for p in model.parameters())
        e = self.entries.get(key)
        if e is not None and e["sig"] != sig:
            del self.entries[key]
            e = None
        if e is None and key in self.failed:
            self.stats["eager"] += 1
            return eager()
        if e is None:
            n = self.seen.get(key, 0) + 1
            if len(self.seen) > 64:
                self.seen.clear()
            self.seen[key] = n
            if n < self.capture_after:
                self.stats["eager"] += 1
                return eager()
            out = eager()
            self.stats["eager"] += 1
            e = self._capture(model, outfit_mask, images, ids, att, tokens, sig)
            if e is None:
                if len(self.failed) < 256:
                    self.failed.add(key)
            else:
                while len(self.entries) >= self.capacity:
                    self.entries.pop(next(iter(self.entries)))
                self.entries[key] = e
            return out
        dev = images.device
        e["ids"].copy_(ids.reshape(e["ids"].shape), non_blocking=True)
        if att is not None:
            e["att"].copy_(att.reshape(e["att"].shape), non_blocking=True)
        e["mask"].copy_(outfit_mask, non_blocking=True)
        e["graph"].replay()
        self.stats["replays"] += 1
        return e["out"].clone()

    def _capture(self, model, outfit_mask, images, ids, att, tokens, sig):
        dev = images.device
        n_rows, T = ids.numel() // ids.shape[-1], ids.shape[-1]
        ids_d = torch.empty(n_rows, T, dtype=torch.int64, device=dev); ids_d.copy_(ids.reshape(n_rows, T))
        att_d = None
        if att is not None:
            att_d = torch.empty(n_rows, T, dtype=torch.int64, device=dev); att_d.copy_(att.reshape(n_rows, T))
        mask_d = outfit_mask.to(dev).clone()
        lengths = None if ids.device.type != "cpu" else [tokens] * n_rows
        prepared = (ids_d, att_d, lengths, ids.shape[0], None)

        def fn():
            return model._cp_eval(mask_d, images, prepared)

        try:
            cc = CapturedCall(fn, dev, warmup=1)
        except Exception:
            self.stats["capture_failures"] += 1
            return None
        self.stats["captures"] += 1
        return {"graph": cc, "out": cc.output, "ids": ids_d, "att": att_d, "mask": mask_d, "sig": sig}
```

Baseline: 8075.

## Compute the shared BOS row once across text sequences in causal CLIP text tower

Under causal attention, the hidden state at position 0 depends only on token 0. When every text row starts with the same unmasked token, the text tower now computes that row once instead of once per sequence, so it processes 1+N*(Tc-1) rows instead of N*Tc. The embedding, EOS-index and set-attention kernels remap row indices, and attention launches an extra block for the shared row. The host detects the shared-first condition and adds it to the graph-cache key and replay checks. The path only runs with the three-product (x3) text precision and fp32 set attention, and it adds index arithmetic plus host-side checks on the token tensors.

Result: faster. 8198 (median of 6 runs) (+1.5%).

```diff
diff --git a/include/ofx.h b/include/ofx.h
--- a/include/ofx.h
+++ b/include/ofx.h
@@ -59,6 +59,9 @@
 int ofx_clip_text_fwd(ofx_handle* h, const int64_t* ids, const int64_t* attn_mask, const int* lengths_host,
                       int N, int T, float* emb, int emb_ld, int emb_col, int normalize, void* ws,
                       size_t ws_bytes, ofx_stream stream);
+int ofx_clip_text_fwd_shared(ofx_handle* h, const int64_t* ids, const int64_t* attn_mask, const int* lengths_host,
+                             int N, int T, float* emb, int emb_ld, int emb_col, int normalize, int shared_first, void* ws,
+                             size_t ws_bytes, ofx_stream stream);
 
 int ofx_fitb_argmin(const float* y_hat, const float* cand, int B, int C, int D, int64_t* idx, float* dist,
                     ofx_stream stream);
diff --git a/outfitx_amd/_lib.py b/outfitx_amd/_lib.py
--- a/outfitx_amd/_lib.py
+++ b/outfitx_amd/_lib.py
@@ -104,6 +104,7 @@
     "ofx_cir_prefix": (_i, [_vp, _vp, _i, _vp, _vp]),
     "ofx_vit_b32_fwd": (_i, [_vp, _vp, _i, _vp, _i, _i, _i, _vp, _sz, _vp]),
     "ofx_clip_text_fwd": (_i, [_vp, _vp, _vp, C.POINTER(_i), _i, _i, _vp, _i, _i, _i, _vp, _sz, _vp]),
+    "ofx_clip_text_fwd_shared": (_i, [_vp, _vp, _vp, C.POINTER(_i), _i, _i, _vp, _i, _i, _i, _i, _vp, _sz, _vp]),
     "ofx_fitb_argmin": (_i, [_vp, _vp, _i, _i, _i, _vp, _vp, _vp]),
     "ofx_fitb_argmin_indexed": (_i, [_vp, _i, C.c_longlong, _vp, _vp, _i, _i, _i, _vp, _vp, _vp, _vp, _vp]),
     "ofx_l2_topk": (_i, [_vp, _vp, _vp, _i, _i, _i, _i, _i64, _vp, _vp, _vp, _sz, _vp]),
diff --git a/outfitx_amd/csrc/api.hip b/outfitx_amd/csrc/api.hip
--- a/outfitx_amd/csrc/api.hip
+++ b/outfitx_amd/csrc/api.hip
@@ -576,17 +576,19 @@
 }
 
 static int clip_layer_x3(const ClipLayer& L, const ClipWs& w, int rows, int nseq, int S, int W, int MLP, int heads, int act,
-                         float eps, int causal, const int64_t* key_mask, int mask_ld, int dt, const int* pool_idx, hipStream_t s, bool mfma_attn = false) {
+                         float eps, int causal, const int64_t* key_mask, int mask_ld, int dt, const int* pool_idx, hipStream_t s, bool mfma_attn = false,
+                         int shared_first = 0) {
     LnArgs ln{w.X, nullptr, L.g1, L.be1, w.H, rows, W, 3 * W, OFX_OUT_SPLIT3, eps};
     TRY(ofx_launch_layernorm(ln, dt, s));
     GemmArgs g1{}; g1.A = w.H; g1.C = w.QKV; g1.M = rows; g1.N = 3 * W;
     use_gemm(g1, L.qkv, W);
     const bool f32_attn = S <= 64 && !mfma_attn;
+    OFX_REQUIRE(!shared_first || f32_attn, OFX_EINVAL, "clip_layer_x3: a shared first row needs the fp32 set attention");
     g1.ldc = 3 * W; g1.act = OFX_ACT_NONE; g1.out_kind = f32_attn ? OFX_OUT_F32 : OFX_OUT_OP;
     TRY(ofx_launch_gemm(g1, dt, s));
     if (f32_attn) {
         SetAttnArgs sa{w.QKV, w.H, nullptr, nseq, heads, W, 3 * W, OFX_OUT_SPLIT3, S, 0, 0.125f};
-        sa.fixed_len = S; sa.causal = causal; sa.key_mask = key_mask; sa.mask_ld = mask_ld;
+        sa.fixed_len = S; sa.causal = causal; sa.key_mask = key_mask; sa.mask_ld = mask_ld; sa.shared_first = shared_first;
         TRY(ofx_launch_set_attention(sa, dt, s));
     } else {
         AttnArgs at{w.QKV, w.H, key_mask, nseq, S, heads, 3 * W, 3 * W, W, 2 * W, mask_ld, causal, 0.125f};
@@ -617,10 +619,12 @@
 
 static int clip_layers(const std::vector<ClipLayer>& Ls, const ClipWs& w, int rows, int nseq, int S, int W, int MLP,
                        int heads, int act, float eps, int causal, const int64_t* key_mask, int mask_ld, int dt,
-                       const int* pool_idx, hipStream_t s, bool pool_first, bool x3) {
+                       const int* pool_idx, hipStream_t s, bool pool_first, bool x3, int shared_first = 0) {
+    OFX_REQUIRE(!shared_first || x3, OFX_EINVAL, "clip_layers: a shared first row exists in the three-product path only");
     if (x3) {
         for (size_t l = 0; l < Ls.size(); ++l)
-            TRY(clip_layer_x3(Ls[l], w, rows, nseq, S, W, MLP, heads, act, eps, causal, key_mask, mask_ld, dt, l + 1 == Ls.size() ? pool_idx : nullptr, s, !causal && !key_mask && !g_x3_vit_f32_attn));
+            TRY(clip_layer_x3(Ls[l], w, rows, nseq, S, W, MLP, heads, act, eps, causal, key_mask, mask_ld, dt, l + 1 == Ls.size() ? pool_idx : nullptr, s, !causal && !key_mask && !g_x3_vit_f32_attn,
+                              shared_first));
         return OFX_OK;
     }
     for (size_t l = 0; l < Ls.size(); ++l)
@@ -697,9 +701,11 @@
     return vit_core(h, nullptr, &raw, N, emb, emb_ld, emb_col, normalize, (char*)ws + pre, ws_bytes - pre, stream);
 }
 
-extern "C" int ofx_clip_text_fwd(ofx_handle* h, const int64_t* ids, const int64_t* attn_mask, const int* lengths_host,
-                                 int N, int T, float* emb, int emb_ld, int emb_col, int normalize, void* ws,
-                                 size_t ws_bytes, ofx_stream stream) {
+int g_text_shared_first = 1;
+
+static int clip_text_core(ofx_handle* h, const int64_t* ids, const int64_t* attn_mask, const int* lengths_host,
+                          int N, int T, float* emb, int emb_ld, int emb_col, int normalize, int shared_first, void* ws,
+                          size_t ws_bytes, ofx_stream stream) {
     OFX_REQUIRE(h && h->txt_ready, OFX_ESTATE, "clip_text_fwd: text weights not packed");
     OFX_REQUIRE(ids && emb && ws && N > 0 && T > 0, OFX_EINVAL, "clip_text_fwd: bad argument");
     const ofx_model_desc& d = h->d;
@@ -715,13 +721,14 @@
     ClipWs w;
     const size_t need = txt_bytes(h, N, Tc, &w, ws, ws_bytes);
     OFX_REQUIRE(need <= ws_bytes, OFX_EWORKSPACE, "clip_text_fwd: workspace %zu < %zu bytes", ws_bytes, need);
-    const int W = d.txt_width, dt = h->tw_dtype, rows = N * Tc;
-    TRY(ofx_launch_text_embed(ids, h->t_tok, h->t_pos, w.X, N, T, Tc, W, d.txt_vocab, s));
-    TRY(ofx_launch_text_eos_index(ids, w.idx, N, T, Tc, d.txt_eos_id, s));
     const bool x3 = h->txt_x3 != 0, x3p = x3 || h->proj_x3;
+    const int sf = shared_first && g_text_shared_first && x3 && Tc >= 2 ? 1 : 0;
+    const int W = d.txt_width, dt = h->tw_dtype, rows = sf ? 1 + N * (Tc - 1) : N * Tc;
+    TRY(ofx_launch_text_embed(ids, h->t_tok, h->t_pos, w.X, N, T, Tc, W, d.txt_vocab, sf, s));
+    TRY(ofx_launch_text_eos_index(ids, w.idx, N, T, Tc, d.txt_eos_id, sf, s));
     const int pk = x3p ? 3 : 1;
     if (!x3) TRY(ofx_launch_row_stats_cast(w.X, w.XB, w.XLO, w.S, rows, W, d.ln_eps, dt, s));
-    TRY(clip_layers(h->tl, w, rows, N, Tc, W, d.txt_mlp, d.txt_heads, d.txt_act, d.ln_eps, 1, attn_mask, T, dt, w.idx, s, false, x3));
+    TRY(clip_layers(h->tl, w, rows, N, Tc, W, d.txt_mlp, d.txt_heads, d.txt_act, d.ln_eps, 1, attn_mask, T, dt, w.idx, s, false, x3, sf));
     LnArgs ln{w.XP, nullptr, h->t_fin_g, h->t_fin_b, w.PL, N, W, pk * W, x3p ? OFX_OUT_SPLIT3 : OFX_OUT_OP, d.ln_eps};
     TRY(ofx_launch_layernorm(ln, dt, s));
     GemmArgs gj{}; gj.A = w.PL; gj.C = w.E; gj.M = N; gj.N = d.proj_dim; gj.ldc = d.proj_dim;
@@ -729,6 +736,17 @@
     gj.act = OFX_ACT_NONE; gj.out_kind = OFX_OUT_F32; gj.slab = w.slab; gj.slab_bytes = w.slab_bytes;
     TRY(ofx_launch_gemm(gj, dt, s));
     return ofx_launch_l2norm_store(w.E, emb, N, d.proj_dim, emb_ld, emb_col, normalize, s);
+}
+
+extern "C" int ofx_clip_text_fwd(ofx_handle* h, const int64_t* ids, const int64_t* attn_mask, const int* lengths_host,
+                                 int N, int T, float* emb, int emb_ld, int emb_col, int normalize, void* ws,
+                                 size_t ws_bytes, ofx_stream stream) {
+    return clip_text_core(h, ids, attn_mask, lengths_host, N, T, emb, emb_ld, emb_col, normalize, 0, ws, ws_bytes, stream);
+}
+extern "C" int ofx_clip_text_fwd_shared(ofx_handle* h, const int64_t* ids, const int64_t* attn_mask, const int* lengths_host,
+                                        int N, int T, float* emb, int emb_ld, int emb_col, int normalize, int shared_first, void* ws,
+                                        size_t ws_bytes, ofx_stream stream) {
+    return clip_text_core(h, ids, attn_mask, lengths_host, N, T, emb, emb_ld, emb_col, normalize, shared_first, ws, ws_bytes, stream);
 }
 
 extern "C" int ofx_fitb_argmin(const float* y, const float* cand, int B, int C, int D, int64_t* idx, float* dist, ofx_stream stream) {
@@ -1131,6 +1149,7 @@
         case 10: g_set_fuse = value; return OFX_OK;
         case 17: g_topk_filter = value != 0; return OFX_OK;
         case 20: g_x3_vit_f32_attn = value != 0; return OFX_OK;
+        case 21: g_text_shared_first = value != 0; return OFX_OK;
         default: ofx_set_error("ofx_tune: unknown knob %d", knob); return OFX_EINVAL;
     }
 }
diff --git a/outfitx_amd/csrc/attention.hip b/outfitx_amd/csrc/attention.hip
--- a/outfitx_amd/csrc/attention.hip
+++ b/outfitx_amd/csrc/attention.hip
@@ -91,6 +91,7 @@
     DropArgs drop;
     int fixed_S, causal, mask_ld;
     const int64_t* key_mask;
+    int shared_first;
     int splits; size_t plane; const float* bias;
 };
 
@@ -105,10 +106,14 @@
     __shared__ __attribute__((aligned(16))) float sc[SMAX * (SMAX + 4)];
     const int lane = threadIdx.x;
     const int b = blockIdx.x / a.n_head, h = blockIdx.x % a.n_head;
-    const int r0 = a.cu ? a.cu[b] : b * a.fixed_S;
-    int S = a.cu ? a.cu[b + 1] - r0 : a.fixed_S;
+    const bool sh = a.shared_first != 0, sh_q0 = sh && b == a.nseq;
+    const int r0 = a.cu ? a.cu[b] : (sh ? (sh_q0 ? 0 : b * (a.fixed_S - 1)) : b * a.fixed_S);
+    int S = a.cu ? a.cu[b + 1] - r0 : (sh_q0 ? 1 : a.fixed_S);
     S = S < SMAX ? S : SMAX;
     const int nq = a.only_row0 ? 1 : S;
+    const int q0 = sh && !sh_q0 ? 1 : 0;
+    const int mb = sh_q0 ? 0 : b;
+    auto row_of = [&](int j) { return sh && j == 0 ? 0 : r0 + j; };
     const int D = a.D;
     const bool two = WIDE && lane < HD - 64;
     float vreg[SMAX];
@@ -149,8 +154,8 @@
         }
     } else if (sizeof(TI) == 4) {
         auto f32_row = [&](int j, int c4) {
-            const float* rp = (const float*)a.qkv + (size_t)(r0 + j) * 3 * D + h * HD + c4;
-            if (j < nq) *(f32x4*)(qs + j * STR + c4) = *(const f32x4*)rp;
+            const float* rp = (const float*)a.qkv + (size_t)row_of(j) * 3 * D + h * HD + c4;
+            if (j >= q0 && j < nq) *(f32x4*)(qs + j * STR + c4) = *(const f32x4*)rp;
             *(f32x4*)(ks + j * STR + c4) = *(const f32x4*)(rp + D);
         };
         if constexpr (!WIDE) {
@@ -163,10 +168,10 @@
             for (int f = lane; f < S * C4; f += 64) f32_row(f / C4, (f % C4) * 4);
         }
 #pragma unroll
-        for (int j = 0; j < SMAX; ++j) vreg[j] = j < S ? ((const float*)a.qkv)[(size_t)(r0 + j) * 3 * D + 2 * D + h * HD + lane] : 0.f;
+        for (int j = 0; j < SMAX; ++j) vreg[j] = j < S ? ((const float*)a.qkv)[(size_t)row_of(j) * 3 * D + 2 * D + h * HD + lane] : 0.f;
         if constexpr (WIDE) {
 #pragma unroll
-            for (int j = 0; j < SMAX; ++j) vreg2[j] = (j < S && two) ? ((const float*)a.qkv)[(size_t)(r0 + j) * 3 * D + 2 * D + h * HD + 64 + lane] : 0.f;
+            for (int j = 0; j < SMAX; ++j) vreg2[j] = (j < S && two) ? ((const float*)a.qkv)[(size_t)row_of(j) * 3 * D + 2 * D + h * HD + 64 + lane] : 0.f;
         }
     } else {
 #pragma unroll
@@ -189,8 +194,8 @@
         }
     }
     __syncthreads();
-    for (int p = lane; p < nq * S; p += 64) {
-        const int i = p / S, j = p % S;
+    for (int p = lane; p < (nq - q0) * S; p += 64) {
+        const int i = q0 + p / S, j = p % S;
         const f32x4* qp = (const f32x4*)(qs + i * STR);
         const f32x4* kp = (const f32x4*)(ks + j * STR);
         float d = 0.f;
@@ -200,11 +205,11 @@
             d += x[0] * y[0] + x[1] * y[1] + x[2] * y[2] + x[3] * y[3];
         }
         bool dead = a.causal && j > i;
-        if (!dead && a.key_mask) dead = a.key_mask[(size_t)b * a.mask_ld + j] == 0;
+        if (!dead && a.key_mask) dead = a.key_mask[(size_t)mb * a.mask_ld + j] == 0;
         sc[i * (SMAX + 4) + j] = dead ? -INFINITY : d * a.scale;
     }
     __syncthreads();
-    if (lane < nq) {
+    if (lane >= q0 && lane < nq) {
         float* row = sc + lane * (SMAX + 4);
         float m = -INFINITY;
         for (int j = 0; j < S; ++j) m = fmaxf(m, row[j]);
@@ -217,22 +222,22 @@
     }
     __syncthreads();
     if (a.out_kind == 0) {
-        for (int i = 0; i < nq; ++i) {
+        for (int i = q0; i < nq; ++i) {
             const float* row = sc + i * (SMAX + 4);
             float acc = 0.f;
 #pragma unroll
             for (int j = 0; j < SMAX; ++j) acc += (j < S ? row[j] : 0.f) * vreg[j];
-            ((float*)a.out)[(size_t)(r0 + i) * a.ldo + h * HD + lane] = acc;
+            ((float*)a.out)[(size_t)row_of(i) * a.ldo + h * HD + lane] = acc;
             if constexpr (WIDE) {
                 float acc2 = 0.f;
 #pragma unroll
                 for (int j = 0; j < SMAX; ++j) acc2 += (j < S ? row[j] : 0.f) * vreg2[j];
-                if (two) ((float*)a.out)[(size_t)(r0 + i) * a.ldo + h * HD + 64 + lane] = acc2;
+                if (two) ((float*)a.out)[(size_t)row_of(i) * a.ldo + h * HD + 64 + lane] = acc2;
             }
         }
         return;
     }
-    for (int i = 0; i < nq; ++i) {
+    for (int i = q0; i < nq; ++i) {
         const float* row = sc + i * (SMAX + 4);
         float acc = 0.f;
 #pragma unroll
@@ -248,16 +253,16 @@
     __syncthreads();
     auto store_row = [&](int i, int c8) {
         const f32x4 x0 = *(const f32x4*)(qs + i * STR + c8), x1 = *(const f32x4*)(qs + i * STR + c8 + 4);
-        store8<T>(a.out, (size_t)(r0 + i) * a.ldo + h * HD + c8, x0, x1, a.out_kind, D);
+        store8<T>(a.out, (size_t)row_of(i) * a.ldo + h * HD + c8, x0, x1, a.out_kind, D);
     };
     if constexpr (!WIDE) {
         const int c8 = (lane & 7) * 8, r8 = lane >> 3;
         for (int i0 = 0; i0 < nq; i0 += 8) {
             const int i = i0 + r8;
-            if (i < nq) store_row(i, c8);
+            if (i >= q0 && i < nq) store_row(i, c8);
         }
     } else {
-        for (int f = lane; f < nq * C8; f += 64) store_row(f / C8, (f % C8) * 8);
+        for (int f = lane + q0 * C8; f < nq * C8; f += 64) store_row(f / C8, (f % C8) * 8);
     }
 }
 
@@ -499,9 +504,12 @@
     k.qkv = g.qkv; k.out = (char*)g.out; k.cu = g.cu_seqlens; k.nseq = g.nseq; k.n_head = g.n_head; k.D = g.D; k.ldo = g.ldo;
     k.out_kind = g.out_kind; k.only_row0 = g.only_row0; k.scale = g.scale; k.drop = g.drop;
     k.fixed_S = g.fixed_len; k.causal = g.causal; k.mask_ld = g.mask_ld; k.key_mask = g.key_mask;
+    OFX_REQUIRE(!g.shared_first || (!g.cu_seqlens && g.causal && g.fixed_len >= 2 && !g.only_row0 && !g.qkv_op && g.splits <= 1 && !g.drop.thresh), OFX_EINVAL,
+                "set_attention: a shared first row needs the fixed-length causal mode on fp32 q|k|v, >= 2 rows per sequence, all queries, no slabs, no dropout");
+    k.shared_first = g.shared_first ? 1 : 0;
     OFX_REQUIRE(g.splits <= 1 || (!g.qkv_op && g.bias && g.plane > 0 && g.max_len <= 32), OFX_EINVAL, "set_attention: slab input needs fp32 q|k|v, the bias, the slab stride and sets of <= 32 rows");
     k.splits = g.splits > 1 ? g.splits : 1; k.plane = g.plane; k.bias = g.bias;
-    const int grid = g.nseq * g.n_head;
+    const int grid = (g.nseq + (g.shared_first ? 1 : 0)) * g.n_head;
     ProfScope prof(PROF_ATTN, s);
 #define SA(T, N) do { if (wide) { if (g.qkv_op) hipLaunchKernelGGL((set_attention_kernel<T, N, T, 96>), dim3(grid), dim3(64), 0, s, k); \
                                       else hipLaunchKernelGGL((set_attention_kernel<T, N, float, 96>), dim3(grid), dim3(64), 0, s, k); } \
diff --git a/outfitx_amd/csrc/norm_act.hip b/outfitx_amd/csrc/norm_act.hip
--- a/outfitx_amd/csrc/norm_act.hip
+++ b/outfitx_amd/csrc/norm_act.hip
@@ -228,12 +228,18 @@
     }
 }
 
+__device__ __forceinline__ int text_row(int i, int t, int Tc, int shared_first) {
+    if (!shared_first) return i * Tc + t;
+    return t == 0 ? 0 : 1 + i * (Tc - 1) + (t - 1);
+}
+
 __global__ __launch_bounds__(256) void text_embed_kernel(const int64_t* ids, const float* tok, const float* pos, float* x,
-                                                        int N, int T, int Tc, int D, int vocab) {
-    const int lane = threadIdx.x & 63, w = threadIdx.x >> 6;
-    const int rows = N * Tc;
+                                                        int N, int T, int Tc, int D, int vocab, int shared_first) {
+    const int lane = threadIdx.x & 63, w = threadIdx.x >> 6;
+    const int rows = shared_first ? 1 + N * (Tc - 1) : N * Tc;
     for (int r = blockIdx.x * 4 + w; r < rows; r += gridDim.x * 4) {
-        const int i = r / Tc, t = r % Tc;
+        int i = r / Tc, t = r % Tc;
+        if (shared_first) { i = r ? (r - 1) / (Tc - 1) : 0; t = r ? 1 + (r - 1) % (Tc - 1) : 0; }
         long long id = ids[(size_t)i * T + t];
         id = id < 0 ? 0 : (id >= vocab ? vocab - 1 : id);
         const f32x4* tp = (const f32x4*)(tok + (size_t)id * D);
@@ -242,7 +248,7 @@
     }
 }
 
-__global__ void text_eos_index_kernel(const int64_t* ids, int* row_idx, int N, int T, int Tc, int eos_id) {
+__global__ void text_eos_index_kernel(const int64_t* ids, int* row_idx, int N, int T, int Tc, int eos_id, int shared_first) {
     const int i = blockIdx.x * blockDim.x + threadIdx.x;
     if (i >= N) return;
     const int64_t* p = ids + (size_t)i * T;
@@ -253,7 +259,7 @@
     } else {
         for (int t = 0; t < T; ++t) if (p[t] == eos_id) { pos = t; break; }
     }
-    row_idx[i] = i * Tc + (pos < Tc ? pos : Tc - 1);
+    row_idx[i] = text_row(i, pos < Tc ? pos : Tc - 1, Tc, shared_first);
 }
 
 __global__ void iota_rows_kernel(int* idx, int n, int stride) {
@@ -484,13 +490,16 @@
     return OFX_OK;
 }
 int ofx_launch_text_embed(const int64_t* ids, const float* tok, const float* pos, float* x, int N, int T, int Tc, int D,
-                          int vocab, hipStream_t s) {
-    hipLaunchKernelGGL(text_embed_kernel, dim3(rows_grid(N * Tc)), dim3(256), 0, s, ids, tok, pos, x, N, T, Tc, D, vocab);
-    OFX_LAUNCH_CHECK();
-    return OFX_OK;
-}
-int ofx_launch_text_eos_index(const int64_t* ids, int* row_idx, int N, int T, int Tc, int eos_id, hipStream_t s) {
-    hipLaunchKernelGGL(text_eos_index_kernel, dim3((N + 255) / 256), dim3(256), 0, s, ids, row_idx, N, T, Tc, eos_id);
+                          int vocab, int shared_first, hipStream_t s) {
+    OFX_REQUIRE(!shared_first || Tc >= 2, OFX_ESHAPE, "text_embed: a shared first row needs Tc >= 2 (Tc=%d)", Tc);
+    hipLaunchKernelGGL(text_embed_kernel, dim3(rows_grid(shared_first ? 1 + N * (Tc - 1) : N * Tc)), dim3(256), 0, s, ids, tok, pos, x, N, T, Tc, D, vocab,
+                       shared_first);
+    OFX_LAUNCH_CHECK();
+    return OFX_OK;
+}
+int ofx_launch_text_eos_index(const int64_t* ids, int* row_idx, int N, int T, int Tc, int eos_id, int shared_first, hipStream_t s) {
+    OFX_REQUIRE(!shared_first || Tc >= 2, OFX_ESHAPE, "text_eos_index: a shared first row needs Tc >= 2 (Tc=%d)", Tc);
+    hipLaunchKernelGGL(text_eos_index_kernel, dim3((N + 255) / 256), dim3(256), 0, s, ids, row_idx, N, T, Tc, eos_id, shared_first);
     OFX_LAUNCH_CHECK();
     return OFX_OK;
 }
diff --git a/outfitx_amd/csrc/ofx_common.h b/outfitx_amd/csrc/ofx_common.h
--- a/outfitx_amd/csrc/ofx_common.h
+++ b/outfitx_amd/csrc/ofx_common.h
@@ -308,8 +308,8 @@
 int ofx_launch_vit_embed_ln(const float* patch_out, const float* cls, const float* pos, const float* g, const float* b,
                             float* x, int N, int S, int D, float eps, hipStream_t s, void* xb, float* stat, int op_dtype, void* xlo);
 int ofx_launch_text_embed(const int64_t* ids, const float* tok, const float* pos, float* x, int N, int T, int Tc, int D,
-                          int vocab, hipStream_t s);
-int ofx_launch_text_eos_index(const int64_t* ids, int* row_idx, int N, int T, int Tc, int eos_id, hipStream_t s);
+                          int vocab, int shared_first, hipStream_t s);
+int ofx_launch_text_eos_index(const int64_t* ids, int* row_idx, int N, int T, int Tc, int eos_id, int shared_first, hipStream_t s);
 int ofx_launch_iota_rows(int* idx, int n, int stride, hipStream_t s);
 int ofx_launch_l2norm_store(const float* src, float* dst, int rows, int D, int ld, int col, int normalize, hipStream_t s);
 int ofx_launch_set_build(const float* x, const uint8_t* mask, const float* prefix, int prefix_stride, int* cu, float* X,
@@ -361,6 +361,7 @@
     int qkv_op = 0;
     int fixed_len = 0, causal = 0, mask_ld = 0;
     const int64_t* key_mask = nullptr;
+    int shared_first = 0;
     int splits = 1; size_t plane = 0; const float* bias = nullptr;
 };
 int ofx_launch_set_attention(const SetAttnArgs& a, int op_dtype, hipStream_t s);
diff --git a/outfitx_amd/encoders.py b/outfitx_amd/encoders.py
--- a/outfitx_amd/encoders.py
+++ b/outfitx_amd/encoders.py
@@ -13,7 +13,7 @@
 
 from . import _lib as L
 from .configs import ItemEncoderConfig
-from .engine import Engine
+from .engine import Engine, TextLengths, shared_first_row
 
 CLIP_MEAN = (0.48145466, 0.4578275, 0.40821073)
 CLIP_STD = (0.26862954, 0.26130258, 0.27577711)
@@ -359,12 +359,12 @@
         ids, att = self._tokenize(flatten_seq_to_one_dim(texts), tokenizer_kargs)
         return ids, att, len(texts)
 
-    def _lengths(self, ids: torch.Tensor):
+    def _lengths(self, ids: torch.Tensor, att=False):
         if ids.device.type != "cpu":
             return None
         eos = self.model.config.eos_token_id
         pos = ids.argmax(-1) if eos == 2 else (ids == eos).int().argmax(-1)
-        return (pos + 1).tolist()
+        return TextLengths((pos + 1).tolist(), att is not False and shared_first_row(ids, att))
 
     def _dedup(self, ids: torch.Tensor, att: Optional[torch.Tensor]):
         if not self.dedup_texts or ids.device.type != "cpu" or ids.shape[0] < 2:
@@ -416,14 +416,14 @@
                 sel = torch.as_tensor(miss, dtype=torch.long)
                 m_ids = ids.index_select(0, sel).contiguous()
                 m_att = None if att is None else att.index_select(0, sel).contiguous()
-                plan["lengths"] = self._lengths(m_ids)
+                plan["lengths"] = self._lengths(m_ids, m_att)
                 plan["ids"], plan["att"] = self._engine("text").stage_tokens(m_ids, m_att)
             return None, None, None, b, plan
         dd = self._dedup(ids, att)
         if dd is not None:
             ids, att, inverse = dd
             inverse = inverse.to(self.device, non_blocking=True)
-        lengths = self._lengths(ids)
+        lengths = self._lengths(ids, att)
         ids_d, att_d = self._engine("text").stage_tokens(ids, att)
         return ids_d, att_d, lengths, b, inverse
 
diff --git a/outfitx_amd/engine.py b/outfitx_amd/engine.py
--- a/outfitx_amd/engine.py
+++ b/outfitx_amd/engine.py
@@ -20,6 +20,23 @@
     if t.device != device or t.dtype != torch.float32 or not t.is_contiguous():
         t = t.to(device=device, dtype=torch.float32).contiguous()
     return t
+
+
+def shared_first_row(ids: torch.Tensor, att: Optional[torch.Tensor]) -> bool:
+    if ids.device.type != "cpu" or ids.dim() != 2 or ids.shape[0] < 1 or ids.shape[1] < 2:
+        return False
+    if not bool((ids[:, 0] == ids[0, 0]).all()):
+        return False
+    if att is not None and (att.device.type != "cpu" or att.shape != ids.shape or not bool((att[:, 0] != 0).all())):
+        return False
+    return True
+
+
+class TextLengths(list):
+
+    def __init__(self, lengths, shared_first: bool = False):
+        super().__init__(lengths)
+        self.shared_first = bool(shared_first)
 
 
 class SetInput(NamedTuple):
@@ -309,15 +326,17 @@
 
     def text(self, ids: torch.Tensor, att: Optional[torch.Tensor], out: torch.Tensor, col: int, normalize: bool,
              lengths: Optional[Sequence[int]] = None) -> None:
+        shared = lengths.shared_first if isinstance(lengths, TextLengths) else shared_first_row(ids, att)
         ids_d, att_d = self.stage_tokens(ids, att)
         N, T = ids_d.shape
         Tc = T if lengths is None else max(1, min(T, max(int(v) for v in lengths)))
         arr = None if lengths is None else (C.c_int * N)(*[int(v) for v in lengths])
         nb = self.ws_bytes(L.OP_TEXT, N, Tc)
         ws = self.workspace(nb)
-        with torch.cuda.device(self.device):
-            L.check(self.lib.ofx_clip_text_fwd(self.h, _ptr(ids_d), _ptr(att_d), arr, N, T, _ptr(out), out.stride(0), col,
-                                               int(normalize), _ptr(ws), ws.numel(), _stream(self.device)), "ofx_clip_text_fwd")
+        shared = bool(shared) and Tc >= 2 and bool(self.desc.txt_x3)
+        with torch.cuda.device(self.device):
+            L.check(self.lib.ofx_clip_text_fwd_shared(self.h, _ptr(ids_d), _ptr(att_d), arr, N, T, _ptr(out), out.stride(0), col,
+                                                      int(normalize), int(shared), _ptr(ws), ws.numel(), _stream(self.device)), "ofx_clip_text_fwd_shared")
         self._keep_ids = (ids_d, att_d)
 
     def l2_topk(self, Q: torch.Tensor, P: torch.Tensor, k: int, index_base: int = 0):
diff --git a/outfitx_amd/graphs.py b/outfitx_amd/graphs.py
--- a/outfitx_amd/graphs.py
+++ b/outfitx_amd/graphs.py
@@ -3,6 +3,8 @@
 from typing import Any, Callable, Optional
 
 import torch
+
+from .engine import TextLengths, shared_first_row
 
 
 class CapturedCall:
@@ -62,11 +64,16 @@
     if ids.device.type == "cpu":
         flat = ids.reshape(-1, ids.shape[-1])
         cc.captured_tokens = max(1, min(flat.shape[1], max(enc._lengths(flat))))
+        att = texts.get("attention_mask")
+        flat_att = None if att is None else att.reshape(-1, att.shape[-1])
+        cc.captured_shared_first = shared_first_row(flat, flat_att)
 
         def check():
             now = max(enc._lengths(flat))
             if now > cc.captured_tokens:
                 raise ValueError(f"replay: a token row of {now} positions, but the graph was captured for {cc.captured_tokens}: capture again (a longer row would be silently truncated)")
+            if cc.captured_shared_first and not shared_first_row(flat, flat_att):
+                raise ValueError("replay: the graph was captured for texts that share their first position (one first token, unmasked), and the token tensors no longer do: capture again")
         cc.check = check
     return cc
 
@@ -116,7 +123,8 @@
         tokens = T
         if ids.device.type == "cpu":
             tokens = max(1, min(T, max(enc.text_enc._lengths(ids.reshape(-1, T)))))
-        key = (images.data_ptr(), tuple(images.shape), images.dtype, tuple(ids.shape), att is not None, tokens, tuple(outfit_mask.shape),
+        shared = shared_first_row(ids.reshape(-1, T), None if att is None else att.reshape(-1, T))
+        key = (images.data_ptr(), tuple(images.shape), images.dtype, tuple(ids.shape), att is not None, tokens, shared, tuple(outfit_mask.shape),
                model.precision, model.tower_fed_precision, enc.image_enc.tower_precision, enc.text_enc.tower_precision, enc.overlap_towers, enc.side_stream_priority,
                enc.image_enc.vit_streams, lib.ofx_config_generation(), torch.cuda.current_stream(images.device).cuda_stream)
         sig = tuple((p.data_ptr(), p._version) for p in model.parameters())
@@ -137,7 +145,7 @@
                 return eager()
             out = eager()
             self.stats["eager"] += 1
-            e = self._capture(model, outfit_mask, images, ids, att, tokens, sig)
+            e = self._capture(model, outfit_mask, images, ids, att, tokens, shared, sig)
             if e is None:
                 if len(self.failed) < 256:
                     self.failed.add(key)
@@ -155,7 +163,7 @@
         self.stats["replays"] += 1
         return e["out"].clone()
 
-    def _capture(self, model, outfit_mask, images, ids, att, tokens, sig):
+    def _capture(self, model, outfit_mask, images, ids, att, tokens, shared, sig):
         dev = images.device
         n_rows, T = ids.numel() // ids.shape[-1], ids.shape[-1]
         ids_d = torch.empty(n_rows, T, dtype=torch.int64, device=dev); ids_d.copy_(ids.reshape(n_rows, T))
@@ -163,7 +171,7 @@
         if att is not None:
             att_d = torch.empty(n_rows, T, dtype=torch.int64, device=dev); att_d.copy_(att.reshape(n_rows, T))
         mask_d = outfit_mask.to(dev).clone()
-        lengths = None if ids.device.type != "cpu" else [tokens] * n_rows
+        lengths = None if ids.device.type != "cpu" else TextLengths([tokens] * n_rows, shared)
         prepared = (ids_d, att_d, lengths, ids.shape[0], None)
 
         def fn():
```
